# seemadhungana/ViT-Project

Measured on AMD Instinct MI355X. Metric: images/sec ViT-B/16 224 train step bs=256 (whole job), higher is better.
Workload: dtype bf16; 1 GPU; ViT-B/16 224 train step (fwd+CE+bwd+SGD), BASELINE configs[1]; model=vit_base_patch16_224, global_batch=256, per_gpu_batch=256, seq_len=197, parallelism=dp1, launch=eager

## Files before the change

include/vit_hip.h:

```cpp
#ifndef VIT_HIP_H
#define VIT_HIP_H
#include <stdint.h>

#ifdef __cplusplus
extern "C" {
#endif

enum { VIT_DTYPE_F32 = 0, VIT_DTYPE_BF16 = 1 };
enum { VIT_LAYOUT_RC = 0, VIT_LAYOUT_CR = 1 };
enum {
  VIT_EPI_STORE = 0,
  VIT_EPI_BIAS_GELU = 1,
  VIT_EPI_RESID = 2,
  VIT_EPI_GELU_BWD = 3,
  VIT_EPI_PATCH = 4,
  VIT_EPI_BIAS_QGELU = 5,
  VIT_EPI_QGELU_BWD = 6,
  VIT_EPI_BIAS_GELU_FWD = 8,
  VIT_EPI_BIAS_QGELU_FWD = 9
};

int vit_abi_version(void);

int vit_gemm(int dtype, int out_dtype, int p_layout, int q_layout, int epi, int M, int N, int R,
             const void* P, int64_t ldp, const void* Q, int64_t ldq, void* C, int64_t ldc,
             const float* bias, const void* aux, int64_t ld_aux, void* aux_out, int allow_fast, void* stream);

int vit_gemm_variant(int v);

int vit_gemm_group(int fwd, int dgrad);

int vit_gemm_g4_config(int fwd_mode, int dgrad_mode, int wgs, int tpw);

int vit_gemm_g4_count(int reset);

int vit_gemm_g4_gelu(int on);

int vit_gemm_streamk_workspace(void* stream, float* part, int64_t part_bytes, int* counters, int ncounters);

int vit_gemm_rc_chunk_rows(int M, int64_t ld);

int vit_linear_fwd(int dtype, int out_dtype, int epi, int M, int N, int K, const void* X, int64_t ldx,
                   const void* W, const float* bias, void* Y, int64_t ldy, const void* resid,
                   void* act_out, void* stream);

int vit_linear_dgrad(int dtype, int out_dtype, int epi, int M, int N, int K, const void* dY, int64_t lddy,
                     const void* W, void* dX, int64_t lddx, const void* pre, float* dbias, float* partial,
                     int64_t partial_floats, int defer_reduce, void* stream);
int vit_linear_dgrad_partial_floats(int M, int K);

int vit_linear_wgrad(int dtype, int M, int N, int K, const void* dY, int64_t lddy, const void* X,
                     int64_t ldx, float* dW, int split, void* workspace, int64_t ws_bytes, void* stream);
int vit_linear_wgrad_nslabs(int dtype, int M, int N, int K, int split);
int vit_linear_wgrad_partials(int dtype, int M, int N, int K, const void* dY, int64_t lddy, const void* X,
                              int64_t ldx, int split, float* slabs, int64_t slab_bytes, void* stream);
int vit_linear_wgrad_partials2(int M, int split, int Na, int Ka, const void* dYa, int64_t lddya, const void* Xa,
                               int64_t ldxa, float* slabs_a, int64_t bytes_a, int Nb, int Kb, const void* dYb,
                               int64_t lddyb, const void* Xb, int64_t ldxb, float* slabs_b, int64_t bytes_b,
                               void* stream);

int vit_colsum(int dtype, int M, int N, const void* X, int64_t ld, float* out, float* partial,
               int64_t partial_floats, int accumulate, void* stream);
int vit_colreduce(const float* part, int S, int N, float* out, int accumulate, float* scratch, void* stream);
int vit_colreduce_multi(const float* part, int nq, int S, int N, float* out0, float* out1, float* out2,
                        int accumulate, float* scratch, void* stream);

int vit_colreduce_batch_sizes(const int64_t* jobs, int njobs, int64_t* scratch_floats, int* counters);
int vit_colreduce_batch(const int64_t* jobs, int njobs, float* scratch, int64_t scratch_floats, int* counters,
                        int ncounters, void* stream);

int vit_patch_embed_fwd(int dtype, int B, int np, int D, int K, const void* U, const void* W,
                        const float* bias, const float* pos, float* x, void* stream);
int vit_patch_unfold(int dtype, int B, int C, int Hi, int Wi, int ps, const float* img, void* U, void* stream);
int vit_patch_unfold_ld(int dtype, int B, int C, int Hi, int Wi, int ps, int ldu, const float* img, void* U,
                        void* stream);
int vit_patch_embed_fwd_ld(int dtype, int B, int np, int D, int K, const void* U, int64_t ldu, const void* W,
                           int64_t ldw, const float* bias, const float* pos, float* x, void* stream);
int vit_copy_rows_padded(int dtype, int rows, int cols, const void* src, int64_t ld_src, void* dst, int64_t ld_dst,
                         void* stream);
int vit_cls_pos_fill(int B, int S, int D, float* x, const float* cls, const float* pos, void* stream);
int vit_pos_grad(int B, int S, int D, const float* dx, float* dpos, float* dcls, void* stream);

int vit_layer_norm_bwd_variant(int v);

int vit_layer_norm_fwd(int dtype_x, int dtype_y, int rows, int D, const void* x, int64_t ldx, void* y,
                       int64_t ldy, const float* w, const float* b, float* mean, float* rstd, float eps,
                       void* stream);
int vit_add_layer_norm_fwd(int dtype_r, int dtype_y, int rows, int D, const float* x, int64_t ldx, const void* r,
                           int64_t ldr, float* xs, int64_t ldxs, void* y, int64_t ldy, const float* w, const float* b,
                           float* mean, float* rstd, float eps, void* stream);
int vit_layer_norm_bwd(int dtype_x, int dtype_dy, int rows, int D, const void* x, int64_t ldx,
                       const void* dy, int64_t lddy, const float* w, const float* mean, const float* rstd,
                       const float* dres, int64_t ldres, float* dx, int64_t lddx, void* dx_copy, int64_t ld_copy,
                       int dtype_copy, int compact_np, float* dgamma, float* dbeta, float* dsum, float* partial,
                       int64_t partial_floats, int defer_reduce, void* stream);
int vit_layer_norm_bwd_partial_floats(int rows, int D);
int vit_layer_norm_bwd_blocks(int rows);

int vit_sdpa_fwd(int dtype, int B, int H, int N, int head_dim, const void* qkv, int64_t ld_qkv, void* o,
                 int64_t ld_o, float* lse, float scale, int causal, void* stream);
int vit_sdpa_fwd_fp8(int dtype, int B, int H, int N, int head_dim, const void* qkv, int64_t ld_qkv, void* o,
                     int64_t ld_o, float* lse, float scale, int causal, void* stream);
int vit_sdpa_bwd(int dtype, int B, int H, int N, int head_dim, const void* qkv, int64_t ld_qkv, const void* o,
                 int64_t ld_o, const void* dout, int64_t ld_do, const float* lse, void* dqkv, int64_t ld_dqkv,
                 float* delta_ws, float scale, int causal, float* dbias, float* partial, int64_t partial_floats,
                 void* stream);
int vit_sdpa_bwd_partial_floats(int B, int N, int D);
int vit_sdpa_long_config(int mode);
int vit_sdpa_long_count(int reset);
int vit_sdpa_long_f32_count(int reset);
int vit_sdpa_bwd_variant(int v);

int vit_cross_entropy_fwd(int B, int C, const float* logits, int64_t ld, const int64_t* target, float* row_lse,
                          float* row_loss, float* loss, void* stream);
int vit_cross_entropy_bwd(int dtype_out, int B, int C, const float* logits, int64_t ld, const int64_t* target,
                          const float* row_lse, const float* grad_loss, void* dlogits, int64_t ldd, void* stream);

int vit_eval_metrics(int B, int C, const float* logits, int64_t ld, const int64_t* target, int topk, float* row_ws,
                     double* acc, void* stream);

int vit_sgd_step(const void* tensors, const void* chunks, int nchunks, const float* lr, float momentum,
                 float weight_decay, void* stream);
int vit_sgd_chunk_size(void);
int vit_sgd_tensor_bytes(void);
int vit_sgd_chunk_bytes(void);

int vit_dora_weight_fwd(int in, int out, int r, const float* m, const float* A, const float* B, const float* D,
                        float scaling, const float* noise, float* W, float* nu, float* DnT_ws, float* colsq_ws,
                        void* stream);
int vit_dora_weight_bwd(int in, int out, int r, const float* m, const float* A, const float* B, const float* gW,
                        const float* DnT, float scaling, const float* nu, float* dm, float* dA, float* dB,
                        float* sdDnT_ws, const float* noise, void* stream);
int vit_dora_weight_bwd_ws(int in, int out, int r, const float* m, const float* A, const float* B, const float* gW,
                           const float* DnT, float scaling, const float* nu, float* dm, float* dA, float* dB,
                           float* sdDnT_ws, float* slabs, int64_t slab_floats, const float* noise, void* stream);
int vit_gemm_splitk(int p_layout, int q_layout, int M, int N, int R, const float* P, int64_t ldp, const float* Q,
                    int64_t ldq, float* C, float* slabs, int64_t slab_floats, void* stream);
int vit_adamw_step(const void* tensors, const void* chunks, int nchunks, float beta1, float beta2, float eps,
                   void* stream);
int vit_adamw_tensor_bytes(void);

int vit_token_embed(int rows, int L, int D, int vocab, const int64_t* tokens, const float* table, const float* pos,
                    float* x, void* stream);
int vit_gather_rows(int n, int D, const float* src, int64_t ld_src, const int64_t* idx, float* dst, int64_t ld_dst,
                    void* stream);
int vit_scatter_rows(int n, int D, const float* src, int64_t ld_src, const int64_t* idx, float* dst, int64_t ld_dst,
                     void* stream);
int vit_rownorm_fwd(int n, int D, const float* x, const float* log_scale, float* y, float* rnorm, void* stream);
int vit_rownorm_bwd(int n, int D, const float* x, const float* dy, const float* rnorm, const float* log_scale,
                    float* dx, void* stream);
int vit_mse_fwd(int n, const float* pred, const float* target, float* loss, void* stream);
int vit_mse_bwd(int n, const float* pred, const float* target, const float* grad_loss, float* dpred, void* stream);

int vit_image_coeff_bytes(int B, int S, int kmax);
int vit_image_transform(int B, int S, const uint8_t* src, const int64_t* params, int kmax, int max_rows,
                        int* coeff_ws, uint8_t* tmp_ws, float* out, const float* norm6, void* stream);

int vit_cast_f32_bf16(const float* x, void* y, int64_t n, void* stream);
int vit_zero(void* p, int64_t bytes, void* stream);

#ifdef __cplusplus
}
#endif
#endif
```

vit-project_amd/csrc/attention.hip:

```cpp
#include "common.hpp"
#include "reduce.hpp"

extern "C" int vit_colsum(int dtype, int M, int N, const void* X, int64_t ld, float* out, float* partial,
                          int64_t partial_floats, int accumulate, void* stream);

__device__ __forceinline__ int at_off(int row, int c) { return row * 128 + ((c ^ (row & 6)) << 4); }

template <int ROWS, int NTHR, int NM>
__device__ __forceinline__ void at_load(char* const (&img)[NM], const bf16* const (&src)[NM],
                                        const int64_t (&ld)[NM], int N) {
  constexpr int TOTAL = ROWS * 8, PER = (TOTAL + NTHR - 1) / NTHR;
  bf16x8 v[NM][PER];
#pragma unroll
  for (int mtx = 0; mtx < NM; ++mtx)
#pragma unroll
    for (int u = 0; u < PER; ++u) {
      const int idx = threadIdx.x + u * NTHR;
      const int row = min(idx >> 3, N - 1), c = idx & 7;
      if (idx < TOTAL) v[mtx][u] = *reinterpret_cast<const bf16x8*>(src[mtx] + (int64_t)row * ld[mtx] + c * 8);
    }
#pragma unroll
  for (int mtx = 0; mtx < NM; ++mtx)
#pragma unroll
    for (int u = 0; u < PER; ++u) {
      const int idx = threadIdx.x + u * NTHR;
      const int row = idx >> 3, c = idx & 7;
      if (idx < TOTAL) {
        bf16x8 w = v[mtx][u];
        if (row >= N) {
#pragma unroll
          for (int t = 0; t < 8; ++t) w[t] = (bf16)0.f;
        }
        *reinterpret_cast<bf16x8*>(img[mtx] + at_off(row, c)) = w;
      }
    }
}

constexpr int AT_THREADS = 512;
constexpr int AT_WAVES = AT_THREADS / 64;

__device__ __forceinline__ bf16x8 pack8(const f32x4& a, const f32x4& b) {
  return bf16x8{(bf16)a[0], (bf16)a[1], (bf16)a[2], (bf16)a[3], (bf16)b[0], (bf16)b[1], (bf16)b[2], (bf16)b[3]};
}

constexpr float LOG2E = 1.4426950408889634f;
constexpr float LN2 = 0.6931471805599453f;

struct AtOffsets {
  int row[2];
  int tr[4];
  __device__ __forceinline__ AtOffsets(int lane) {
    const int l15 = lane & 15, g = lane >> 4, q = l15 >> 2, p = l15 & 3;
#pragma unroll
    for (int kk = 0; kk < 2; ++kk) row[kk] = l15 * 128 + (((kk * 4 + g) ^ (l15 & 6)) << 4);
    const int ra = 4 * g + q;
#pragma unroll
    for (int dt = 0; dt < 4; ++dt) tr[dt] = ra * 128 + (((2 * dt + (p >> 1)) ^ (ra & 6)) << 4) + (p & 1) * 8;
  }
};
__device__ __forceinline__ bf16x8 rowf(const char* img, int row0, int off) {
  return *reinterpret_cast<const bf16x8*>(img + row0 * 128 + off);
}
__device__ __forceinline__ bf16x8 trf(const char* img, int row0, int off) {
  const char* b = img + row0 * 128 + off;
  return cat4(lds_read_tr(b), lds_read_tr(b + 16 * 128));
}
__device__ __forceinline__ float fexp2(float x) { return __builtin_amdgcn_exp2f(x); }

static unsigned long long* g_attn_stamps = nullptr;
#define AT_STAMP(i)                                                   \
  if constexpr (STAMP) { if (threadIdx.x == 0) st[i] = __builtin_amdgcn_s_memtime(); }
#define AT_STAMP_BEGIN()                                                                          \
  unsigned long long st[8] = {0, 0, 0, 0, 0, 0, 0, 0};                                            \
  if constexpr (STAMP) { if (threadIdx.x == 0) st[5] = __builtin_amdgcn_s_memrealtime(); }        \
  AT_STAMP(0)
#define AT_STAMP_FLUSH()                                                                         \
  if constexpr (STAMP) if (threadIdx.x == 0) {                                                   \
    asm volatile("s_waitcnt vmcnt(0)" ::: "memory");                                             \
    st[6] = __builtin_amdgcn_s_memtime();                                                        \
    st[7] = __builtin_amdgcn_s_memrealtime();                                                    \
    unsigned long long* d = stamps + (int64_t)blockIdx.x * 8;                                    \
    for (int i_ = 0; i_ < 8; ++i_) d[i_] = st[i_];                                               \
  }

template <int NT, bool STAMP = false, bool CAUSAL = false>
__global__ __launch_bounds__(AT_THREADS, NT <= 14 ? 4 : 2) void attn_fwd_mfma(const bf16* __restrict__ qkv, int64_t ld_qkv, int D,
                                                     int H, int N, float scale, bf16* __restrict__ o,
                                                     int64_t ld_o, float* __restrict__ lse, int causal,
                                                     unsigned long long* __restrict__ stamps) {
  AT_STAMP_BEGIN()
  constexpr int NT2 = (NT + 1) / 2, ROWS = NT2 * 32;
  __shared__ __attribute__((aligned(16))) char smem[2 * ROWS * 128];
  char* Kimg = smem;
  char* Vimg = smem + ROWS * 128;
  const int bh = blockIdx.x, b = bh / H, h = bh - b * H;
  const int lane = threadIdx.x & 63, wave = threadIdx.x >> 6, g = lane >> 4;
  const bf16* base = qkv + (int64_t)b * N * ld_qkv + h * 64;
  {
    char* const imgs[2] = {Kimg, Vimg};
    const bf16* const srcs[2] = {base + D, base + 2 * D};
    const int64_t lds_[2] = {ld_qkv, ld_qkv};
    at_load<ROWS, AT_THREADS, 2>(imgs, srcs, lds_, N);
  }
  const AtOffsets off(lane);
  __syncthreads();
  AT_STAMP(1)
  const float c2 = scale * LOG2E;
  for (int qt = wave; qt < NT; qt += AT_WAVES) {
    const int q = qt * 16 + (lane & 15);
    bf16x8 qf[2];
    {
      const int qq = min(q, N - 1);
#pragma unroll
      for (int kk = 0; kk < 2; ++kk) qf[kk] = *reinterpret_cast<const bf16x8*>(base + (int64_t)qq * ld_qkv + kk * 32 + g * 8);
    }
    f32x4 s[NT];
#pragma unroll
    for (int kt = 0; kt < NT; ++kt) {
      s[kt] = f32x4{0.f, 0.f, 0.f, 0.f};
#pragma unroll
      for (int kk = 0; kk < 2; ++kk) s[kt] = mfma16(rowf(Kimg, kt * 16, off.row[kk]), qf[kk], s[kt]);
      if (kt % 4 == 3) __builtin_amdgcn_sched_barrier(0);
    }
#pragma unroll
    for (int r = 0; r < 4; ++r)
      if ((NT - 1) * 16 + 4 * g + r >= N) s[NT - 1][r] = -INFINITY;
    if constexpr (CAUSAL) {
#pragma unroll
      for (int kt = 0; kt < NT; ++kt)
#pragma unroll
        for (int r = 0; r < 4; ++r)
          if (kt * 16 + 4 * g + r > q) s[kt][r] = -INFINITY;
    }
    float mr[4] = {-INFINITY, -INFINITY, -INFINITY, -INFINITY};
#pragma unroll
    for (int kt = 0; kt < NT; ++kt)
#pragma unroll
      for (int r = 0; r < 4; ++r) mr[r] = fmaxf(mr[r], s[kt][r]);
    float m = fmaxf(fmaxf(mr[0], mr[1]), fmaxf(mr[2], mr[3]));
    m = fmaxf(m, __shfl_xor(m, 16, 64));
    m = fmaxf(m, __shfl_xor(m, 32, 64));
    const float mc = m * c2;
    float lr[4] = {0.f, 0.f, 0.f, 0.f};
#pragma unroll
    for (int kt = 0; kt < NT; ++kt)
#pragma unroll
      for (int r = 0; r < 4; ++r) { float p = fexp2(fmaf(s[kt][r], c2, -mc)); s[kt][r] = p; lr[r] += p; }
    float l = (lr[0] + lr[1]) + (lr[2] + lr[3]);
    l += __shfl_xor(l, 16, 64);
    l += __shfl_xor(l, 32, 64);
    f32x4 oacc[4];
#pragma unroll
    for (int dt = 0; dt < 4; ++dt) oacc[dt] = f32x4{0.f, 0.f, 0.f, 0.f};
#pragma unroll
    for (int ks = 0; ks < NT2; ++ks) {
      f32x4 hi = (2 * ks + 1 < NT) ? s[2 * ks + 1 < NT ? 2 * ks + 1 : 0] : f32x4{0.f, 0.f, 0.f, 0.f};
      bf16x8 pf = pack8(s[2 * ks], hi);
#pragma unroll
      for (int dt = 0; dt < 4; ++dt) oacc[dt] = mfma16(trf(Vimg, ks * 32, off.tr[dt]), pf, oacc[dt]);
      if (ks % 2 == 1) __builtin_amdgcn_sched_barrier(0);
    }
    if (q < N) {
      const float inv = 1.0f / l;
      bf16* orow = o + ((int64_t)b * N + q) * ld_o + h * 64;
#pragma unroll
      for (int dt = 0; dt < 4; ++dt) {
        bf16x4 ov = {(bf16)(oacc[dt][0] * inv), (bf16)(oacc[dt][1] * inv), (bf16)(oacc[dt][2] * inv),
                     (bf16)(oacc[dt][3] * inv)};
        *reinterpret_cast<bf16x4*>(orow + dt * 16 + 4 * g) = ov;
      }
      if (g == 0) lse[(int64_t)bh * N + q] = (mc + __log2f(l)) * LN2;
    }
  }
  AT_STAMP(2)
  AT_STAMP_FLUSH()
}


__device__ __forceinline__ int e8m0_exp(float amax) {
  const uint32_t bits = __float_as_uint(amax);
  const int E = (int)((bits >> 23) & 255) - 127;
  if (((bits >> 23) & 255) == 0) return -127;
  const int e = (bits & 0x7fffff) <= 0x600000 ? E - 8 : E - 7;
  return e < -127 ? -127 : (e > 127 ? 127 : e);
}
__device__ __forceinline__ float inv_exp2i(int e) {
  return e >= 127 ? 0.f : __uint_as_float((uint32_t)(e == -127 ? 254 : 127 - e) << 23);
}
__device__ __forceinline__ int pack_fp8x4(float a, float b, float c, float d) {
  int w = __builtin_amdgcn_cvt_pk_fp8_f32(a, b, 0, false);
  return __builtin_amdgcn_cvt_pk_fp8_f32(c, d, w, true);
}
typedef int i32x8 __attribute__((ext_vector_type(8)));
typedef float f32x16 __attribute__((ext_vector_type(16)));

constexpr int F8_THREADS = 512, F8_WAVES = 8;
__device__ __forceinline__ int f8_koff(int key, int c) { return key * 64 + ((c ^ ((key >> 2) & 1)) << 4); }

template <typename T> __device__ __forceinline__ void load8f(const T* p, float* x);
template <> __device__ __forceinline__ void load8f<bf16>(const bf16* p, float* x) {
  const bf16x8 v = *reinterpret_cast<const bf16x8*>(p);
#pragma unroll
  for (int u = 0; u < 8; ++u) x[u] = (float)v[u];
}
template <> __device__ __forceinline__ void load8f<float>(const float* p, float* x) {
  const f32x4 a = *reinterpret_cast<const f32x4*>(p), b = *reinterpret_cast<const f32x4*>(p + 4);
#pragma unroll
  for (int u = 0; u < 4; ++u) { x[u] = a[u]; x[4 + u] = b[u]; }
}

template <int NKT, typename T>
__global__ __launch_bounds__(F8_THREADS, 2) void attn_fwd_fp8(const T* __restrict__ qkv, int64_t ld_qkv, int D,
                                                             int H, int N, float scale, T* __restrict__ o,
                                                             int64_t ld_o, float* __restrict__ lse, int causal) {
  constexpr int KEYS = NKT * 64, VROW = KEYS + 4;
  __shared__ __attribute__((aligned(16))) unsigned char Kimg[KEYS * 64];
  __shared__ __attribute__((aligned(16))) unsigned char Vt[64 * VROW];
  __shared__ unsigned char Ksc[KEYS * 2];
  __shared__ unsigned char Vsc[64 * NKT];
  const int bh = blockIdx.x, b = bh / H, hh = bh - b * H;
  const int lane = threadIdx.x & 63, wave = threadIdx.x >> 6;
  const T* base = qkv + (int64_t)b * N * ld_qkv + hh * 64;

  for (int t = threadIdx.x; t < KEYS * 2; t += F8_THREADS) {
    const int key = t >> 1, half = t & 1;
    float x[32];
    if (key < N) {
      const T* src = base + (int64_t)key * ld_qkv + D + half * 32;
#pragma unroll
      for (int c = 0; c < 4; ++c) load8f<T>(src + c * 8, x + c * 8);
    } else {
#pragma unroll
      for (int u = 0; u < 32; ++u) x[u] = 0.f;
    }
    float amax = 0.f;
#pragma unroll
    for (int u = 0; u < 32; ++u) amax = fmaxf(amax, fabsf(x[u]));
    amax = fmaxf(amax, __shfl_xor(amax, 1, 64));
    const int e = e8m0_exp(amax);
    const float inv = inv_exp2i(e);
    int w[8];
#pragma unroll
    for (int u = 0; u < 8; ++u) w[u] = pack_fp8x4(x[4 * u] * inv, x[4 * u + 1] * inv, x[4 * u + 2] * inv, x[4 * u + 3] * inv);
    typedef int i32x4_ __attribute__((ext_vector_type(4)));
    *reinterpret_cast<i32x4_*>(Kimg + f8_koff(key, 2 * half)) = i32x4_{w[0], w[1], w[2], w[3]};
    *reinterpret_cast<i32x4_*>(Kimg + f8_koff(key, 2 * half + 1)) = i32x4_{w[4], w[5], w[6], w[7]};
    Ksc[key * 2 + half] = (unsigned char)(e + 127);
  }
  for (int kt = wave; kt < NKT; kt += F8_WAVES) {
    float x[64];
    const T* src = base + 2 * D + lane;
#pragma unroll
    for (int u = 0; u < 64; ++u) {
      const int key = kt * 64 + u;
      x[u] = key < N ? (float)src[(int64_t)key * ld_qkv] : 0.f;
    }
    float amax = 0.f;
#pragma unroll
    for (int u = 0; u < 64; ++u) amax = fmaxf(amax, fabsf(x[u]));
    const int e = e8m0_exp(amax);
    const float inv = inv_exp2i(e);
#pragma unroll
    for (int u = 0; u < 16; ++u)
      *reinterpret_cast<int*>(Vt + lane * VROW + kt * 64 + 4 * u) =
          pack_fp8x4(x[4 * u] * inv, x[4 * u + 1] * inv, x[4 * u + 2] * inv, x[4 * u + 3] * inv);
    Vsc[lane * NKT + kt] = (unsigned char)(e + 127);
  }
  __syncthreads();

  const float c2 = scale * LOG2E;
  const int h = lane >> 5, l31 = lane & 31;
  const int nqt = (N + 31) / 32;
  for (int qt = wave; qt < nqt; qt += F8_WAVES) {
    const int q = qt * 32 + l31;
    i32x8 qf;
    int qsc;
    {
      const T* src = base + (int64_t)min(q, N - 1) * ld_qkv + h * 32;
      float x[32];
#pragma unroll
      for (int c = 0; c < 4; ++c) load8f<T>(src + c * 8, x + c * 8);
      float amax = 0.f;
#pragma unroll
      for (int u = 0; u < 32; ++u) amax = fmaxf(amax, fabsf(x[u]));
      amax = fmaxf(amax, __shfl_xor(amax, 32, 64));
      const int e = e8m0_exp(amax);
      const float inv = inv_exp2i(e);
#pragma unroll
      for (int u = 0; u < 8; ++u) qf[u] = pack_fp8x4(x[4 * u] * inv, x[4 * u + 1] * inv, x[4 * u + 2] * inv, x[4 * u + 3] * inv);
      qsc = e + 127;
    }
    float m = -INFINITY, l = 0.f;
    f32x16 oacc[2] = {};
#pragma unroll 1
    for (int kt = 0; kt < NKT; ++kt) {
      f32x16 s[2];
#pragma unroll
      for (int u = 0; u < 2; ++u) {
        const int key = (2 * kt + u) * 32 + l31;
        typedef int i32x4_ __attribute__((ext_vector_type(4)));
        const i32x4_ lo = *reinterpret_cast<const i32x4_*>(Kimg + f8_koff(key, 2 * h));
        const i32x4_ hi = *reinterpret_cast<const i32x4_*>(Kimg + f8_koff(key, 2 * h + 1));
        const i32x8 kf = {lo[0], lo[1], lo[2], lo[3], hi[0], hi[1], hi[2], hi[3]};
        f32x16 z = {};
        s[u] = __builtin_amdgcn_mfma_scale_f32_32x32x64_f8f6f4(kf, qf, z, 0, 0, 0, Ksc[key * 2 + h], 0, qsc);
      }
      float mt = -INFINITY;
#pragma unroll
      for (int u = 0; u < 2; ++u)
#pragma unroll
        for (int r = 0; r < 16; ++r) {
          const int key = (2 * kt + u) * 32 + 4 * h + (r & 3) + 8 * (r >> 2);
          if (key >= N || (causal && key > q)) s[u][r] = -INFINITY;
          mt = fmaxf(mt, s[u][r]);
        }
      mt = fmaxf(mt, __shfl_xor(mt, 32, 64));
      const float mn = fmaxf(m, mt);
      const float alpha = fexp2((m - mn) * c2);
      m = mn;
      const float mc = m * c2;
      l *= alpha;
#pragma unroll
      for (int dt = 0; dt < 2; ++dt) oacc[dt] *= alpha;
#pragma unroll
      for (int u = 0; u < 2; ++u)
#pragma unroll
        for (int r = 0; r < 16; ++r) {
          const float p = fexp2(fmaf(s[u][r], c2, -mc));
          s[u][r] = p;
          l += p;
        }
      i32x8 pf;
#pragma unroll
      for (int w = 0; w < 8; ++w) {
        const f32x16& t = s[w >> 2];
        const int r = 4 * (w & 3);
        pf[w] = pack_fp8x4(t[r] * 256.f, t[r + 1] * 256.f, t[r + 2] * 256.f, t[r + 3] * 256.f);
      }
#pragma unroll
      for (int dt = 0; dt < 2; ++dt) {
        const int d = dt * 32 + l31;
        const unsigned char* row = Vt + d * VROW + kt * 64 + 4 * h;
        i32x8 vf;
#pragma unroll
        for (int w = 0; w < 8; ++w) vf[w] = *reinterpret_cast<const int*>(row + (w >> 2) * 32 + 8 * (w & 3));
        oacc[dt] = __builtin_amdgcn_mfma_scale_f32_32x32x64_f8f6f4(vf, pf, oacc[dt], 0, 0, 0, Vsc[d * NKT + kt], 0,
                                                                   127 - 8);
      }
    }
    l += __shfl_xor(l, 32, 64);
    const float mc = m * c2;
    if (q < N) {
      const float inv = 1.0f / l;
      T* orow = o + ((int64_t)b * N + q) * ld_o + hh * 64;
#pragma unroll
      for (int dt = 0; dt < 2; ++dt)
#pragma unroll
        for (int mq = 0; mq < 4; ++mq) {
          const int d = dt * 32 + 4 * h + 8 * mq;
          const f32x4 ov = {oacc[dt][4 * mq] * inv, oacc[dt][4 * mq + 1] * inv, oacc[dt][4 * mq + 2] * inv,
                            oacc[dt][4 * mq + 3] * inv};
          if constexpr (sizeof(T) == 2) *reinterpret_cast<bf16x4*>(orow + d) = bf16x4{(bf16)ov[0], (bf16)ov[1], (bf16)ov[2], (bf16)ov[3]};
          else *reinterpret_cast<f32x4*>(orow + d) = ov;
        }
      if (h == 0 && lse) lse[(int64_t)bh * N + q] = (mc + __log2f(l)) * LN2;
    }
  }
}

template <int NOUT>
__device__ __forceinline__ void bias_flush(f32x4 (&c0)[4], f32x4 (*c1)[4], char* smem, float* out, int D) {
  const int lane = threadIdx.x & 63, wave = threadIdx.x >> 6, g = lane >> 4;
  float* red = reinterpret_cast<float*>(smem);
  __syncthreads();
#pragma unroll
  for (int o = 0; o < NOUT; ++o) {
    f32x4 (&c)[4] = o == 0 ? c0 : *c1;
#pragma unroll
    for (int dt = 0; dt < 4; ++dt)
#pragma unroll
      for (int t = 0; t < 4; ++t) {
        float v = c[dt][t];
        v += __shfl_xor(v, 1, 64);
        v += __shfl_xor(v, 2, 64);
        v += __shfl_xor(v, 4, 64);
        v += __shfl_xor(v, 8, 64);
        if ((lane & 15) == 0) red[(o * AT_WAVES + wave) * 64 + dt * 16 + 4 * g + t] = v;
      }
  }
  __syncthreads();
  if (threadIdx.x < 64 * NOUT) {
    const int o = threadIdx.x >> 6, d = threadIdx.x & 63;
    float sum = 0.f;
#pragma unroll
    for (int w = 0; w < AT_WAVES; ++w) sum += red[(o * AT_WAVES + w) * 64 + d];
    out[(NOUT == 1 ? 0 : (o + 1) * D) + d] = sum;
  }
}

__device__ __forceinline__ float colsum16(const f32x4 (&c)[4], int lane) {
  const int l15 = lane & 15;
  float own = 0.f;
#pragma unroll
  for (int dt = 0; dt < 4; ++dt)
#pragma unroll
    for (int t = 0; t < 4; ++t) {
      float v = c[dt][t];
      v += __shfl_xor(v, 1, 64);
      v += __shfl_xor(v, 2, 64);
      v += __shfl_xor(v, 4, 64);
      v += __shfl_xor(v, 8, 64);
// ... 1279 lines not shown
}

__global__ __launch_bounds__(AT_THREADS, 4) void attn_bwd_dq_stream_f32(
    const float* __restrict__ qkv, int64_t ld_qkv, int D, int H, int N, float scale, const float* __restrict__ o,
    int64_t ld_o, const float* __restrict__ dout, int64_t ld_do, const float* __restrict__ lse,
    float* __restrict__ delta_out, float* __restrict__ dqkv, int64_t ld_dqkv) {
  extern __shared__ __attribute__((aligned(16))) char smem[];
  float* ring = reinterpret_cast<float*>(smem);
  const int bh = blockIdx.x, b = bh / H, h = bh - b * H;
  const int lane = threadIdx.x & 63, wave = threadIdx.x >> 6, g = lane >> 4, l15 = lane & 15;
  const float* base = qkv + (int64_t)b * N * ld_qkv + h * 64;
  const int q = blockIdx.y * ST_QB + wave * 16 + l15, qc = min(q, N - 1);
  float qf[16], df[16];
  float dl = 0.f;
  {
    float of[16];
    f32_glob16(base + (int64_t)qc * ld_qkv + 16 * g, qf);
    f32_glob16(dout + ((int64_t)b * N + qc) * ld_do + h * 64 + 16 * g, df);
    f32_glob16(o + ((int64_t)b * N + qc) * ld_o + h * 64 + 16 * g, of);
#pragma unroll
    for (int j = 0; j < 16; ++j) dl = fmaf(df[j], of[j], dl);
  }
  dl += __shfl_xor(dl, 16, 64);
  dl += __shfl_xor(dl, 32, 64);
  if (q < N && g == 0) delta_out[(int64_t)bh * N + q] = dl;
  const float l2 = lse[(int64_t)bh * N + qc] * LOG2E;
  const int nc = (N + ST_CH - 1) / ST_CH;
  SfPiece pc = sf_fetch(base + D, ld_qkv, base + 2 * D, ld_qkv, 0, N);
  sf_commit(ring, pc, 0, N);
  __syncthreads();
  const float c2 = scale * LOG2E;
  f32x4 dq[4];
#pragma unroll
  for (int dt = 0; dt < 4; ++dt) dq[dt] = f32x4{0.f, 0.f, 0.f, 0.f};
#pragma unroll 1
  for (int c = 0; c < nc; ++c) {
    const float* Kc = ring + (c & 1) * 2 * SF_IMG;
    const float* Vc = Kc + SF_IMG;
    const int j0 = c * ST_CH;
    const bool more = c + 1 < nc;
    if (more) pc = sf_fetch(base + D, ld_qkv, base + 2 * D, ld_qkv, j0 + ST_CH, N);
#pragma unroll 1
    for (int kt = 0; kt < 4; ++kt) {
      float kf[16], vf[16];
      f32_row16(Kc, kt * 16 + l15, g, kf);
      f32_row16(Vc, kt * 16 + l15, g, vf);
      f32x4 st = {0.f, 0.f, 0.f, 0.f}, dpt = st;
#pragma unroll
      for (int ks = 0; ks < 16; ++ks) {
        st = mfma4(kf[ks], qf[ks], st);
        dpt = mfma4(vf[ks], df[ks], dpt);
      }
      f32x4 ds;
#pragma unroll
      for (int r = 0; r < 4; ++r) {
        const float p = j0 + kt * 16 + 4 * g + r < N ? fexp2(fmaf(st[r], c2, -l2)) : 0.f;
        ds[r] = p * (dpt[r] - dl);
      }
#pragma unroll
      for (int r = 0; r < 4; ++r) {
        const f32x4 a = f32_chunk(Kc, kt * 16 + 4 * g + r, l15);
#pragma unroll
        for (int dt = 0; dt < 4; ++dt) dq[dt] = mfma4(a[dt], ds[r], dq[dt]);
      }
    }
    if (more) sf_commit(ring + ((c + 1) & 1) * 2 * SF_IMG, pc, j0 + ST_CH, N);
    __syncthreads();
  }
  if (q < N) {
    float* row = dqkv + ((int64_t)b * N + q) * ld_dqkv + h * 64 + 16 * g;
#pragma unroll
    for (int rr = 0; rr < 4; ++rr)
      *reinterpret_cast<f32x4*>(row + 4 * rr) =
          f32x4{dq[0][rr] * scale, dq[1][rr] * scale, dq[2][rr] * scale, dq[3][rr] * scale};
  }
}

__global__ __launch_bounds__(AT_THREADS, 2) void attn_bwd_dkv_stream_f32(
    const float* __restrict__ qkv, int64_t ld_qkv, int D, int H, int N, float scale, const float* __restrict__ dout,
    int64_t ld_do, const float* __restrict__ lse, const float* __restrict__ delta_in, float* __restrict__ dqkv,
    int64_t ld_dqkv) {
  extern __shared__ __attribute__((aligned(16))) char smem[];
  float* ring = reinterpret_cast<float*>(smem);
  const int bh = blockIdx.x, b = bh / H, h = bh - b * H;
  const int tid = threadIdx.x, lane = tid & 63, wave = tid >> 6, g = lane >> 4, l15 = lane & 15;
  const float* base = qkv + (int64_t)b * N * ld_qkv + h * 64;
  const float* dob = dout + (int64_t)b * N * ld_do + h * 64;
  const int key = blockIdx.y * ST_QB + wave * 16 + l15, kc = min(key, N - 1);
  const bool kvalid = key < N;
  float kf[16], vf[16];
  f32_glob16(base + (int64_t)kc * ld_qkv + D + 16 * g, kf);
  f32_glob16(base + (int64_t)kc * ld_qkv + 2 * D + 16 * g, vf);
  auto stat_fetch = [&](int j0) -> float {
    if (tid >= 2 * ST_CH) return 0.f;
    const int i = j0 + (tid & (ST_CH - 1));
    if (tid < ST_CH) return i < N ? lse[(int64_t)bh * N + i] * LOG2E : INFINITY;
    return i < N ? delta_in[(int64_t)bh * N + i] : 0.f;
  };
  auto stat_commit = [&](float* buf, float v) {
    if (tid < 2 * ST_CH) buf[2 * SF_IMG + tid] = v;
  };
  const int nc = (N + ST_CH - 1) / ST_CH;
  SfPiece pc = sf_fetch(base, ld_qkv, dob, ld_do, 0, N);
  float sv = stat_fetch(0);
  sf_commit(ring, pc, 0, N);
  stat_commit(ring, sv);
  __syncthreads();
  const float c2 = scale * LOG2E;
  f32x4 dk[4], dv[4];
#pragma unroll
  for (int dt = 0; dt < 4; ++dt) { dk[dt] = f32x4{0.f, 0.f, 0.f, 0.f}; dv[dt] = dk[dt]; }
#pragma unroll 1
  for (int c = 0; c < nc; ++c) {
    const float* Qc = ring + (c & 1) * SF_BUF_DKV;
    const float* Oc = Qc + SF_IMG;
    const float* l2s = Qc + 2 * SF_IMG;
    const float* dls = l2s + ST_CH;
    const int j0 = c * ST_CH;
    const bool more = c + 1 < nc;
    if (more) {
      pc = sf_fetch(base, ld_qkv, dob, ld_do, j0 + ST_CH, N);
      sv = stat_fetch(j0 + ST_CH);
    }
#pragma unroll 1
    for (int qt = 0; qt < 4; ++qt) {
      float qf[16], df[16];
      f32_row16(Qc, qt * 16 + l15, g, qf);
      f32_row16(Oc, qt * 16 + l15, g, df);
      f32x4 sc = {0.f, 0.f, 0.f, 0.f}, dpc = sc;
#pragma unroll
      for (int ks = 0; ks < 16; ++ks) {
        sc = mfma4(qf[ks], kf[ks], sc);
        dpc = mfma4(df[ks], vf[ks], dpc);
      }
      const f32x4 l2 = *reinterpret_cast<const f32x4*>(l2s + qt * 16 + 4 * g);
      const f32x4 dl = *reinterpret_cast<const f32x4*>(dls + qt * 16 + 4 * g);
      f32x4 p, ds;
#pragma unroll
      for (int r = 0; r < 4; ++r) {
        const float pv = kvalid ? fexp2(fmaf(sc[r], c2, -l2[r])) : 0.f;
        p[r] = pv;
        ds[r] = pv * (dpc[r] - dl[r]);
      }
#pragma unroll
      for (int r = 0; r < 4; ++r) {
        const f32x4 ao = f32_chunk(Oc, qt * 16 + 4 * g + r, l15), aq = f32_chunk(Qc, qt * 16 + 4 * g + r, l15);
#pragma unroll
        for (int dt = 0; dt < 4; ++dt) {
          dv[dt] = mfma4(ao[dt], p[r], dv[dt]);
          dk[dt] = mfma4(aq[dt], ds[r], dk[dt]);
        }
      }
    }
    if (more) {
      float* nb = ring + ((c + 1) & 1) * SF_BUF_DKV;
      sf_commit(nb, pc, j0 + ST_CH, N);
      stat_commit(nb, sv);
    }
    __syncthreads();
  }
  if (kvalid) {
    float* row = dqkv + ((int64_t)b * N + key) * ld_dqkv + h * 64 + 16 * g;
#pragma unroll
    for (int rr = 0; rr < 4; ++rr) {
      *reinterpret_cast<f32x4*>(row + D + 4 * rr) =
          f32x4{dk[0][rr] * scale, dk[1][rr] * scale, dk[2][rr] * scale, dk[3][rr] * scale};
      *reinterpret_cast<f32x4*>(row + 2 * D + 4 * rr) = f32x4{dv[0][rr], dv[1][rr], dv[2][rr], dv[3][rr]};
    }
  }
}

__global__ __launch_bounds__(256) void attn_bias_image(const bf16* __restrict__ dqkv, int64_t ld, int N, int C,
                                                       float* __restrict__ part) {
  const int b = blockIdx.x, c = blockIdx.y * 256 + threadIdx.x;
  if (c >= C) return;
  const bf16* p = dqkv + (int64_t)b * N * ld + c;
  float a[8] = {0.f, 0.f, 0.f, 0.f, 0.f, 0.f, 0.f, 0.f};
  int n = 0;
  for (; n + 8 <= N; n += 8)
#pragma unroll
    for (int u = 0; u < 8; ++u) a[u] += (float)p[(int64_t)(n + u) * ld];
  for (; n < N; ++n) a[0] += (float)p[(int64_t)n * ld];
  part[(int64_t)b * C + c] = ((a[0] + a[1]) + (a[2] + a[3])) + ((a[4] + a[5]) + (a[6] + a[7]));
}

static int g_long_mode = -1;
static int g_long_count = 0;
static int g_long_f32_count = 0;
static bool attn_long_stream() {
  if (g_long_mode >= 0) return g_long_mode != 0;
  static const int v = [] { const char* e = getenv("VIT_ATTN_LONG"); return e && *e == '0' ? 0 : 1; }();
  return v != 0;
}
constexpr int AT_RESIDENT_MAX = 288;

static void stream_f32_attrs() {
  static bool attr = false;
  if (attr) return;
  (void)hipFuncSetAttribute((const void*)attn_fwd_stream_f32, hipFuncAttributeMaxDynamicSharedMemorySize, SF_LDS);
  (void)hipFuncSetAttribute((const void*)attn_bwd_dq_stream_f32, hipFuncAttributeMaxDynamicSharedMemorySize, SF_LDS);
  (void)hipFuncSetAttribute((const void*)attn_bwd_dkv_stream_f32, hipFuncAttributeMaxDynamicSharedMemorySize, SF_LDS_DKV);
  attr = true;
}

template <int NT>
static int fwd_mfma(const void* qkv, int64_t ld_qkv, int D, int B, int H, int N, float scale, int causal, void* o,
                    int64_t ld_o, float* lse, hipStream_t s) {
  if (causal)
    hipLaunchKernelGGL((attn_fwd_mfma<NT, false, true>), dim3(B * H), dim3(AT_THREADS), 0, s, (const bf16*)qkv, ld_qkv,
                       D, H, N, scale, (bf16*)o, ld_o, lse, causal, nullptr);
  else if (g_attn_stamps)
    hipLaunchKernelGGL((attn_fwd_mfma<NT, true>), dim3(B * H), dim3(AT_THREADS), 0, s, (const bf16*)qkv, ld_qkv, D, H,
                       N, scale, (bf16*)o, ld_o, lse, causal, g_attn_stamps);
  else
    hipLaunchKernelGGL((attn_fwd_mfma<NT>), dim3(B * H), dim3(AT_THREADS), 0, s, (const bf16*)qkv, ld_qkv, D, H, N,
                       scale, (bf16*)o, ld_o, lse, causal, nullptr);
  VIT_CHECK_LAUNCH();
  return 0;
}
static bool attn_f32_generic() {
  static const int v = [] { const char* e = getenv("VIT_ATTN_F32_GENERIC"); return e && *e == '1' ? 1 : 0; }();
  return v != 0;
}
template <int NT>
static int fwd_f32mfma(const void* qkv, int64_t ld_qkv, int D, int B, int H, int N, float scale, int causal, void* o,
                       int64_t ld_o, float* lse, hipStream_t s) {
  constexpr int lds = 2 * NT * 16 * 64 * 4;
  static bool attr = false;
  if (!attr) {
    (void)hipFuncSetAttribute((const void*)attn_fwd_f32mfma<NT>, hipFuncAttributeMaxDynamicSharedMemorySize, lds);
    attr = true;
  }
  hipLaunchKernelGGL((attn_fwd_f32mfma<NT>), dim3(B * H), dim3(512), lds, s, (const float*)qkv, ld_qkv, D, H, N, scale,
                     (float*)o, ld_o, lse, causal);
  VIT_CHECK_LAUNCH();
  return 0;
}
template <int NT>
static int bwd_f32mfma(const void* qkv, int64_t ld_qkv, int D, int B, int H, int N, float scale, int causal,
                       const void* o, int64_t ld_o, const void* dout, int64_t ld_do, const float* lse, float* delta,
                       void* dqkv, int64_t ld_dqkv, hipStream_t s) {
  constexpr int img = NT * 16 * 64 * 4, lds_dq = 2 * img, lds_dkv = 2 * img + 2 * NT * 16 * 4;
  static bool attr = false;
  if (!attr) {
    (void)hipFuncSetAttribute((const void*)attn_bwd_dq_f32mfma<NT>, hipFuncAttributeMaxDynamicSharedMemorySize, lds_dq);
    (void)hipFuncSetAttribute((const void*)attn_bwd_dkv_f32mfma<NT>, hipFuncAttributeMaxDynamicSharedMemorySize, lds_dkv);
    attr = true;
  }
  hipLaunchKernelGGL((attn_bwd_dq_f32mfma<NT>), dim3(B * H), dim3(512), lds_dq, s, (const float*)qkv, ld_qkv, D, H, N,
                     scale, (const float*)o, ld_o, (const float*)dout, ld_do, lse, delta, (float*)dqkv, ld_dqkv, causal);
  VIT_CHECK_LAUNCH();
  hipLaunchKernelGGL((attn_bwd_dkv_f32mfma<NT>), dim3(B * H), dim3(512), lds_dkv, s, (const float*)qkv, ld_qkv, D, H,
                     N, scale, (const float*)dout, ld_do, lse, (const float*)delta, (float*)dqkv, ld_dqkv, causal);
  VIT_CHECK_LAUNCH();
  return 0;
}
static int g_bwd_variant = -1;
static bool attn_bwd_split() {
  if (g_bwd_variant == 2) return true;
  static const int v = [] { const char* e = getenv("VIT_ATTN_BWD_SPLIT"); return e && *e == '1' ? 1 : 0; }();
  return v != 0;
}

template <int NT>
static int bwd_mfma(const void* qkv, int64_t ld_qkv, int D, int B, int H, int N, float scale, int causal, const void* o,
                    int64_t ld_o, const void* dout, int64_t ld_do, const float* lse, float* delta,
                    void* dqkv, int64_t ld_dqkv, float* bias_part, hipStream_t s) {
  if constexpr (NT <= 14) {
    if (!attn_bwd_split()) {
      static bool attr = false;
      if (!attr) {
        (void)hipFuncSetAttribute((const void*)attn_bwd_fused<NT>, hipFuncAttributeMaxDynamicSharedMemorySize,
                                  BwdF<NT>::LDS);
        (void)hipFuncSetAttribute((const void*)attn_bwd_fused<NT, true>, hipFuncAttributeMaxDynamicSharedMemorySize,
                                  BwdF<NT>::LDS);
        (void)hipFuncSetAttribute((const void*)attn_bwd_fused<NT, false, true>,
                                  hipFuncAttributeMaxDynamicSharedMemorySize, BwdF<NT>::LDS);
        attr = true;
      }
#define BWD_FUSED(C, S, ST)                                                                                    \
  hipLaunchKernelGGL((attn_bwd_fused<NT, C, S>), dim3(B * H), dim3(BwdF<NT>::THREADS), BwdF<NT>::LDS, s,         \
                     (const bf16*)qkv, ld_qkv, D, H, N, scale, (const bf16*)o, ld_o, (const bf16*)dout, ld_do, lse, \
                     delta, (bf16*)dqkv, ld_dqkv, bias_part, ST)
      if (causal)
        BWD_FUSED(true, false, nullptr);
      else if (g_attn_stamps)
        BWD_FUSED(false, true, g_attn_stamps);
      else
        BWD_FUSED(false, false, nullptr);
#undef BWD_FUSED
      VIT_CHECK_LAUNCH();
      return 0;
    }
  }
  hipLaunchKernelGGL((attn_bwd_dq<NT>), dim3(B * H), dim3(AT_THREADS), 0, s, (const bf16*)qkv, ld_qkv, D, H, N, scale,
                     (const bf16*)o, ld_o, (const bf16*)dout, ld_do, lse, delta, (bf16*)dqkv, ld_dqkv, bias_part, causal);
  VIT_CHECK_LAUNCH();
  hipLaunchKernelGGL((attn_bwd_dkv<NT>), dim3(B * H), dim3(AT_THREADS), 0, s, (const bf16*)qkv, ld_qkv, D, H, N, scale,
                     (const bf16*)dout, ld_do, lse, (const float*)delta, (bf16*)dqkv, ld_dqkv, bias_part, causal);
  VIT_CHECK_LAUNCH();
  return 0;
}

#define NT_CASES(X) X(1) X(2) X(3) X(4) X(5) X(6) X(7) X(8) X(9) X(10) X(11) X(12) X(13) X(14) X(15) X(16) X(17) X(18)

extern "C" {

int vit_debug_attn_stamps(void* buf) {
  g_attn_stamps = (unsigned long long*)buf;
  return 0;
}

int vit_sdpa_bwd_variant(int v) {
  if (v == 0 || v > 2) return (int)hipErrorInvalidValue;
  g_bwd_variant = v < 0 ? -1 : v;
  return 0;
}

int vit_sdpa_long_config(int mode) {
  const int prev = g_long_mode;
  g_long_mode = mode < 0 ? -1 : (mode != 0);
  return prev;
}
int vit_sdpa_long_count(int reset) {
  const int c = g_long_count;
  if (reset) g_long_count = 0;
  return c;
}
int vit_sdpa_long_f32_count(int reset) {
  const int c = g_long_f32_count;
  if (reset) g_long_f32_count = 0;
  return c;
}

int vit_sdpa_fwd(int dtype, int B, int H, int N, int head_dim, const void* qkv, int64_t ld_qkv, void* o,
                 int64_t ld_o, float* lse, float scale, int causal, void* stream) {
  hipStream_t s = (hipStream_t)stream;
  if (head_dim != 64 || N <= 0) return (int)hipErrorInvalidValue;
  const int D = H * 64;
  const bool resident = N <= AT_RESIDENT_MAX;
  if (!resident && dtype == VIT_BF16 && !causal && (ld_qkv % 8 == 0) && (ld_o % 4 == 0) && attn_long_stream()) {
    hipLaunchKernelGGL(attn_fwd_stream, dim3(B * H, (N + ST_QB - 1) / ST_QB), dim3(AT_THREADS), 0, s,
                       (const bf16*)qkv, ld_qkv, D, H, N, scale, (bf16*)o, ld_o, lse);
    VIT_CHECK_LAUNCH();
    ++g_long_count;
    return 0;
  }
  if (!resident && dtype == VIT_F32 && !causal && (ld_qkv % 4 == 0) && (ld_o % 4 == 0) && attn_long_stream() &&
      !attn_f32_generic()) {
    stream_f32_attrs();
    hipLaunchKernelGGL(attn_fwd_stream_f32, dim3(B * H, (N + ST_QB - 1) / ST_QB), dim3(AT_THREADS), SF_LDS, s,
                       (const float*)qkv, ld_qkv, D, H, N, scale, (float*)o, ld_o, lse);
    VIT_CHECK_LAUNCH();
    ++g_long_f32_count;
    return 0;
  }
  if (resident && dtype == VIT_BF16 && (ld_qkv % 8 == 0) && (ld_o % 4 == 0)) {
    int nt = (N + 15) / 16;
    switch (nt) {
#define CASE(n) case n: return fwd_mfma<n>(qkv, ld_qkv, D, B, H, N, scale, causal, o, ld_o, lse, s);
      NT_CASES(CASE)
#undef CASE
    }
  }
  if (resident && dtype == VIT_F32 && (ld_qkv % 4 == 0) && (ld_o % 4 == 0) && !attn_f32_generic()) {
    int nt = (N + 15) / 16;
    switch (nt) {
#define CASE(n) case n: return fwd_f32mfma<n>(qkv, ld_qkv, D, B, H, N, scale, causal, o, ld_o, lse, s);
      NT_CASES(CASE)
#undef CASE
    }
  }
  if ((int64_t)B * H > 65535) return (int)hipErrorInvalidValue;
  dim3 grid((N + 63) / 64, B * H);
  if (dtype == VIT_BF16)
    hipLaunchKernelGGL(attn_fwd_generic<bf16>, grid, dim3(256), 0, s, (const bf16*)qkv, ld_qkv, D, H, N, scale, (bf16*)o, ld_o, lse, causal);
  else
    hipLaunchKernelGGL(attn_fwd_generic<float>, grid, dim3(256), 0, s, (const float*)qkv, ld_qkv, D, H, N, scale, (float*)o, ld_o, lse, causal);
  VIT_CHECK_LAUNCH();
  return 0;
}

int vit_sdpa_fwd_fp8(int dtype, int B, int H, int N, int head_dim, const void* qkv, int64_t ld_qkv, void* o,
                     int64_t ld_o, float* lse, float scale, int causal, void* stream) {
  hipStream_t s = (hipStream_t)stream;
  if (head_dim != 64 || N <= 0 || N > 320 || (ld_qkv % 8) || (ld_o % 4)) return (int)hipErrorInvalidValue;
  const int D = H * 64;
  switch ((N + 63) / 64) {
#define F8(n)                                                                                                   \
  case n:                                                                                                       \
    if (dtype == VIT_BF16)                                                                                      \
      hipLaunchKernelGGL((attn_fwd_fp8<n, bf16>), dim3(B * H), dim3(F8_THREADS), 0, s, (const bf16*)qkv, ld_qkv, \
                         D, H, N, scale, (bf16*)o, ld_o, lse, causal);                                          \
    else                                                                                                        \
      hipLaunchKernelGGL((attn_fwd_fp8<n, float>), dim3(B * H), dim3(F8_THREADS), 0, s, (const float*)qkv,      \
                         ld_qkv, D, H, N, scale, (float*)o, ld_o, lse, causal);                                 \
    break;
    F8(1) F8(2) F8(3) F8(4) F8(5)
#undef F8
  }
  VIT_CHECK_LAUNCH();
  return 0;
}

int vit_sdpa_bwd_partial_floats(int B, int N, int D) {
  const int64_t C = 3 * (int64_t)D;
  const int64_t mfma = B * C + (B > 64 ? (int64_t)((B + 63) / 64) * C : 0);
  const int64_t gen = 256 * C + 4 * C;
  return (int)(mfma > gen ? mfma : gen);
}

int vit_sdpa_bwd(int dtype, int B, int H, int N, int head_dim, const void* qkv, int64_t ld_qkv, const void* o,
                 int64_t ld_o, const void* dout, int64_t ld_do, const float* lse, void* dqkv, int64_t ld_dqkv,
                 float* delta_ws, float scale, int causal, float* dbias, float* partial, int64_t partial_floats,
                 void* stream) {
  hipStream_t s = (hipStream_t)stream;
  if (head_dim != 64 || N <= 0) return (int)hipErrorInvalidValue;
  const int D = H * 64;
  const bool resident = N <= AT_RESIDENT_MAX;
  if (!delta_ws) return (int)hipErrorInvalidValue;
  const bool part_only = !dbias && partial;
  if ((dbias || part_only) && (partial == nullptr || partial_floats < vit_sdpa_bwd_partial_floats(B, N, D)))
    return (int)hipErrorInvalidValue;
  const bool mfma_ok = dtype == VIT_BF16 && (ld_qkv % 8 == 0) && (ld_do % 8 == 0) && (ld_dqkv % 4 == 0) && (ld_o % 4 == 0);
  if (!resident && dtype == VIT_BF16) {
    if (mfma_ok && !causal && attn_long_stream()) {
      const dim3 grid(B * H, (N + ST_QB - 1) / ST_QB);
      hipLaunchKernelGGL(attn_bwd_dq_stream, grid, dim3(AT_THREADS), 0, s, (const bf16*)qkv, ld_qkv, D, H, N, scale,
                         (const bf16*)o, ld_o, (const bf16*)dout, ld_do, lse, delta_ws, (bf16*)dqkv, ld_dqkv);
      VIT_CHECK_LAUNCH();
      hipLaunchKernelGGL(attn_bwd_dkv_stream, grid, dim3(AT_THREADS), 0, s, (const bf16*)qkv, ld_qkv, D, H, N, scale,
                         (const bf16*)dout, ld_do, lse, (const float*)delta_ws, (bf16*)dqkv, ld_dqkv);
      VIT_CHECK_LAUNCH();
      ++g_long_count;
    } else {
      if ((int64_t)B * H > 65535) return (int)hipErrorInvalidValue;
      const dim3 grid((N + 63) / 64, B * H);
      hipLaunchKernelGGL(attn_bwd_dq_generic<bf16>, grid, dim3(256), 0, s, (const bf16*)qkv, ld_qkv, D, H, N, scale,
                         (const bf16*)o, ld_o, (const bf16*)dout, ld_do, lse, delta_ws, (bf16*)dqkv, ld_dqkv, causal);
      VIT_CHECK_LAUNCH();
      hipLaunchKernelGGL(attn_bwd_dkv_generic<bf16>, grid, dim3(256), 0, s, (const bf16*)qkv, ld_qkv, D, H, N, scale,
                         (const bf16*)dout, ld_do, lse, delta_ws, (bf16*)dqkv, ld_dqkv, causal);
      VIT_CHECK_LAUNCH();
    }
    if (!dbias && !part_only) return 0;
    hipLaunchKernelGGL(attn_bias_image, dim3(B, (3 * D + 255) / 256), dim3(256), 0, s, (const bf16*)dqkv, ld_dqkv, N,
                       3 * D, partial);
    VIT_CHECK_LAUNCH();
    if (dbias) {
      launch_colreduce(partial, B, 3 * D, dbias, 0, s, partial + (int64_t)B * 3 * D);
      VIT_CHECK_LAUNCH();
    }
    return 0;
  }
  if (part_only && !mfma_ok) return (int)hipErrorInvalidValue;
  if (resident && mfma_ok) {
    int nt = (N + 15) / 16;
    int rc = (int)hipErrorInvalidValue;
    switch (nt) {
#define CASE(n) case n: rc = bwd_mfma<n>(qkv, ld_qkv, D, B, H, N, scale, causal, o, ld_o, dout, ld_do, lse, delta_ws, dqkv, ld_dqkv, (dbias || part_only) ? partial : nullptr, s); break;
      NT_CASES(CASE)
#undef CASE
    }
    if (rc || !dbias) return rc;
    launch_colreduce(partial, B, 3 * D, dbias, 0, s, partial + (int64_t)B * 3 * D);
    VIT_CHECK_LAUNCH();
    return 0;
  }
  if (resident && dtype == VIT_F32 && (ld_qkv % 4 == 0) && (ld_do % 4 == 0) && (ld_dqkv % 4 == 0) && (ld_o % 4 == 0) &&
      !attn_f32_generic()) {
    int nt = (N + 15) / 16, rc = (int)hipErrorInvalidValue;
    switch (nt) {
#define CASE(n) case n: rc = bwd_f32mfma<n>(qkv, ld_qkv, D, B, H, N, scale, causal, o, ld_o, dout, ld_do, lse, delta_ws, dqkv, ld_dqkv, s); break;
      NT_CASES(CASE)
#undef CASE
    }
    if (rc) return rc;
    if (dbias) return vit_colsum(dtype, B * N, 3 * D, dqkv, ld_dqkv, dbias, partial, partial_floats, 0, stream);
    return 0;
  }
  if (!resident && dtype == VIT_F32 && !causal && (ld_qkv % 4 == 0) && (ld_do % 4 == 0) && (ld_dqkv % 4 == 0) &&
      (ld_o % 4 == 0) && attn_long_stream() && !attn_f32_generic()) {
    stream_f32_attrs();
    const dim3 grid(B * H, (N + ST_QB - 1) / ST_QB);
    hipLaunchKernelGGL(attn_bwd_dq_stream_f32, grid, dim3(AT_THREADS), SF_LDS, s, (const float*)qkv, ld_qkv, D, H, N,
                       scale, (const float*)o, ld_o, (const float*)dout, ld_do, lse, delta_ws, (float*)dqkv, ld_dqkv);
    VIT_CHECK_LAUNCH();
    hipLaunchKernelGGL(attn_bwd_dkv_stream_f32, grid, dim3(AT_THREADS), SF_LDS_DKV, s, (const float*)qkv, ld_qkv, D, H,
                       N, scale, (const float*)dout, ld_do, lse, (const float*)delta_ws, (float*)dqkv, ld_dqkv);
    VIT_CHECK_LAUNCH();
    ++g_long_f32_count;
    if (dbias) return vit_colsum(dtype, B * N, 3 * D, dqkv, ld_dqkv, dbias, partial, partial_floats, 0, stream);
    return 0;
  }
  if ((int64_t)B * H > 65535) return (int)hipErrorInvalidValue;
  dim3 grid((N + 63) / 64, B * H);
#define GEN(T)                                                                                               \
  hipLaunchKernelGGL(attn_bwd_dq_generic<T>, grid, dim3(256), 0, s, (const T*)qkv, ld_qkv, D, H, N, scale,    \
                     (const T*)o, ld_o, (const T*)dout, ld_do, lse, delta_ws, (T*)dqkv, ld_dqkv, causal);    \
  VIT_CHECK_LAUNCH();                                                                                        \
  hipLaunchKernelGGL(attn_bwd_dkv_generic<T>, grid, dim3(256), 0, s, (const T*)qkv, ld_qkv, D, H, N, scale,   \
                     (const T*)dout, ld_do, lse, delta_ws, (T*)dqkv, ld_dqkv, causal);
  if (dtype == VIT_BF16) { GEN(bf16) } else { GEN(float) }
#undef GEN
  VIT_CHECK_LAUNCH();
  if (dbias) return vit_colsum(dtype, B * N, 3 * D, dqkv, ld_dqkv, dbias, partial, partial_floats, 0, stream);
  return 0;
}

}
```

vit-project_amd/csrc/norm.hip:

```cpp
#include "common.hpp"
#include "reduce.hpp"
#include <stdlib.h>
#include <type_traits>

constexpr int LN_WAVES = 4;
constexpr int LN_SMAX = 32;
static int ln_bwd_rows() {
  static int r = 0;
  if (r <= 0) {
    const char* s = getenv("VIT_LN_BWD_ROWS");
    r = s ? atoi(s) : 32;
    if (r < 4) r = 32;
  }
  return r;
}

template <typename T> __device__ __forceinline__ f32x4 ld4(const T* p);
template <> __device__ __forceinline__ f32x4 ld4<float>(const float* p) { return *reinterpret_cast<const f32x4*>(p); }
template <> __device__ __forceinline__ f32x4 ld4<bf16>(const bf16* p) {
  bf16x4 x = *reinterpret_cast<const bf16x4*>(p);
  return f32x4{(float)x[0], (float)x[1], (float)x[2], (float)x[3]};
}
template <typename T> __device__ __forceinline__ void st4(T* p, f32x4 v);
template <> __device__ __forceinline__ void st4<float>(float* p, f32x4 v) { *reinterpret_cast<f32x4*>(p) = v; }
template <> __device__ __forceinline__ void st4<bf16>(bf16* p, f32x4 v) {
  *reinterpret_cast<bf16x4*>(p) = bf16x4{(bf16)v[0], (bf16)v[1], (bf16)v[2], (bf16)v[3]};
}

__device__ __forceinline__ int col4(int lane, int k) { return (k * 64 + lane) * 4; }

template <int NV, typename TX, typename TY>
__global__ __launch_bounds__(256) void ln_fwd_kernel(const TX* __restrict__ x, int64_t ldx, TY* __restrict__ y,
                                                     int64_t ldy, const float* __restrict__ w,
                                                     const float* __restrict__ b, float* __restrict__ mean,
                                                     float* __restrict__ rstd, int rows, int D, float eps) {
  const int lane = threadIdx.x & 63;
  const int row = blockIdx.x * LN_WAVES + (threadIdx.x >> 6);
  if (row >= rows) return;
  const TX* xr = x + (int64_t)row * ldx;
  TY* yr = y + (int64_t)row * ldy;
  if constexpr (NV > 0) {
    f32x4 v[NV];
    float s = 0.f;
#pragma unroll
    for (int k = 0; k < NV; ++k) { v[k] = ld4<TX>(xr + col4(lane, k)); s += (v[k][0] + v[k][1]) + (v[k][2] + v[k][3]); }
    const float mu = wave_sum(s) / D;
    float q = 0.f;
#pragma unroll
    for (int k = 0; k < NV; ++k)
#pragma unroll
      for (int t = 0; t < 4; ++t) { float d = v[k][t] - mu; q += d * d; }
    const float rs = rsqrtf(wave_sum(q) / D + eps);
#pragma unroll
    for (int k = 0; k < NV; ++k) {
      int c = col4(lane, k);
      f32x4 g = *reinterpret_cast<const f32x4*>(w + c), bb = *reinterpret_cast<const f32x4*>(b + c), o;
#pragma unroll
      for (int t = 0; t < 4; ++t) o[t] = (v[k][t] - mu) * rs * g[t] + bb[t];
      st4<TY>(yr + c, o);
    }
    if (lane == 0) { if (mean) mean[row] = mu; if (rstd) rstd[row] = rs; }
  } else {
    float s = 0.f;
    for (int c = lane; c < D; c += 64) s += (float)xr[c];
    const float mu = wave_sum(s) / D;
    float q = 0.f;
    for (int c = lane; c < D; c += 64) { float d = (float)xr[c] - mu; q += d * d; }
    const float rs = rsqrtf(wave_sum(q) / D + eps);
    for (int c = lane; c < D; c += 64) yr[c] = (TY)(((float)xr[c] - mu) * rs * w[c] + b[c]);
    if (lane == 0) { if (mean) mean[row] = mu; if (rstd) rstd[row] = rs; }
  }
}

template <int NV, typename TR, typename TY>
__global__ __launch_bounds__(256) void add_ln_fwd_kernel(const float* __restrict__ x, int64_t ldx,
                                                         const TR* __restrict__ r, int64_t ldr,
                                                         float* __restrict__ xs, int64_t ldxs, TY* __restrict__ y,
                                                         int64_t ldy, const float* __restrict__ w,
                                                         const float* __restrict__ b, float* __restrict__ mean,
                                                         float* __restrict__ rstd, int rows, int D, float eps) {
  const int lane = threadIdx.x & 63;
  const int row = blockIdx.x * LN_WAVES + (threadIdx.x >> 6);
  if (row >= rows) return;
  const float* xr = x + (int64_t)row * ldx;
  const TR* rr = r + (int64_t)row * ldr;
  float* sr = xs + (int64_t)row * ldxs;
  f32x4 v[NV];
  float s = 0.f;
#pragma unroll
  for (int k = 0; k < NV; ++k) {
    const int c = col4(lane, k);
    v[k] = ld4<float>(xr + c) + ld4<TR>(rr + c);
    s += (v[k][0] + v[k][1]) + (v[k][2] + v[k][3]);
  }
#pragma unroll
  for (int k = 0; k < NV; ++k) st4<float>(sr + col4(lane, k), v[k]);
  if (y == nullptr) return;
  const float mu = wave_sum(s) / D;
  float q = 0.f;
#pragma unroll
  for (int k = 0; k < NV; ++k)
#pragma unroll
    for (int t = 0; t < 4; ++t) { float d = v[k][t] - mu; q += d * d; }
  const float rs = rsqrtf(wave_sum(q) / D + eps);
  TY* yr = y + (int64_t)row * ldy;
#pragma unroll
  for (int k = 0; k < NV; ++k) {
    const int c = col4(lane, k);
    f32x4 g = *reinterpret_cast<const f32x4*>(w + c), bb = *reinterpret_cast<const f32x4*>(b + c), o;
#pragma unroll
    for (int t = 0; t < 4; ++t) o[t] = (v[k][t] - mu) * rs * g[t] + bb[t];
    st4<TY>(yr + c, o);
  }
  if (lane == 0) { mean[row] = mu; rstd[row] = rs; }
}

__device__ __forceinline__ bool copy_row(int row, int compact_np, int64_t& orow) {
  orow = row;
  if (compact_np > 0) {
    int bb = row / (compact_np + 1), p = row - bb * (compact_np + 1);
    orow = (int64_t)bb * compact_np + p - 1;
    return p != 0;
  }
  return true;
}

template <int NV, typename TX, typename TD, typename TC>
__global__ __launch_bounds__(256) void ln_bwd_kernel(
    const TX* __restrict__ x, int64_t ldx, const TD* __restrict__ dy, int64_t lddy,
    const float* __restrict__ w, const float* __restrict__ mean, const float* __restrict__ rstd,
    const float* __restrict__ dres, int64_t ldres, float* __restrict__ dx, int64_t lddx,
    TC* __restrict__ dxc, int64_t ldc, int compact_np, float* __restrict__ part_g,
    float* __restrict__ part_b, float* __restrict__ part_s, int rows, int D, int rows_per) {
  constexpr int NP = NV > 0 ? NV * 4 : LN_SMAX;
  const int lane = threadIdx.x & 63, wv = threadIdx.x >> 6;
  float pg[NP], pb[NP], ps[NP];
#pragma unroll
  for (int t = 0; t < NP; ++t) { pg[t] = 0.f; pb[t] = 0.f; ps[t] = 0.f; }
  __shared__ float red[LN_WAVES][192];
  const int r0 = blockIdx.x * rows_per, r1 = min(rows, r0 + rows_per);
  for (int row = r0 + wv; row < r1; row += LN_WAVES) {
    const TX* xr = x + (int64_t)row * ldx;
    const TD* dyr = dy + (int64_t)row * lddy;
    const float mu = mean[row], rs = rstd[row];
    float* dxr = dx + (int64_t)row * lddx;
    int64_t orow = row;
    const bool keep = (dxc != nullptr) && copy_row(row, compact_np, orow);
    if constexpr (NV > 0) {
      f32x4 xh[NV], g[NV], rv[NV];
      float s1 = 0.f, s2 = 0.f;
      if (dres) {
#pragma unroll
        for (int k = 0; k < NV; ++k)
          rv[k] = *reinterpret_cast<const f32x4*>(dres + (int64_t)row * ldres + col4(lane, k));
      }
#pragma unroll
      for (int k = 0; k < NV; ++k) {
        int c = col4(lane, k);
        f32x4 xv = ld4<TX>(xr + c), dv = ld4<TD>(dyr + c), wv4 = *reinterpret_cast<const f32x4*>(w + c);
#pragma unroll
        for (int t = 0; t < 4; ++t) {
          xh[k][t] = (xv[t] - mu) * rs;
          g[k][t] = dv[t] * wv4[t];
          s1 += g[k][t];
          s2 += g[k][t] * xh[k][t];
          pg[k * 4 + t] += dv[t] * xh[k][t];
          pb[k * 4 + t] += dv[t];
        }
      }
      s1 = wave_sum(s1) / D;
      s2 = wave_sum(s2) / D;
#pragma unroll
      for (int k = 0; k < NV; ++k) {
        int c = col4(lane, k);
        f32x4 o;
#pragma unroll
        for (int t = 0; t < 4; ++t) o[t] = rs * (g[k][t] - s1 - xh[k][t] * s2);
        if (dres) o += rv[k];
#pragma unroll
        for (int t = 0; t < 4; ++t) ps[k * 4 + t] += o[t];
        *reinterpret_cast<f32x4*>(dxr + c) = o;
        if (keep) st4<TC>(dxc + orow * ldc + c, o);
      }
    } else {
      float s1 = 0.f, s2 = 0.f;
#pragma unroll
      for (int k = 0; k < LN_SMAX; ++k) {
        int c = lane + 64 * k;
        if (c < D) {
          float xh = ((float)xr[c] - mu) * rs, dv = (float)dyr[c], g = dv * w[c];
          s1 += g; s2 += g * xh;
          pg[k] += dv * xh; pb[k] += dv;
        }
      }
      s1 = wave_sum(s1) / D;
      s2 = wave_sum(s2) / D;
#pragma unroll
      for (int k = 0; k < LN_SMAX; ++k) {
        const int c = lane + 64 * k;
        if (c >= D) break;
        float xh = ((float)xr[c] - mu) * rs, g = (float)dyr[c] * w[c];
        float o = rs * (g - s1 - xh * s2);
        if (dres) o += dres[(int64_t)row * ldres + c];
        ps[k] += o;
        dxr[c] = o;
        if (keep) dxc[orow * ldc + c] = (TC)o;
      }
    }
  }
  if (!part_g && !part_s) return;
  if constexpr (NV > 0) {
    __shared__ float redv[LN_WAVES][NP][64];
    auto flush = [&](const float (&p)[NP], float* out) {
#pragma unroll
      for (int k = 0; k < NP; ++k) redv[wv][k][lane] = p[k];
      __syncthreads();
#pragma unroll
      for (int k = wv; k < NP; k += LN_WAVES) {
        const float v = (redv[0][k][lane] + redv[1][k][lane]) + (redv[2][k][lane] + redv[3][k][lane]);
        out[(int64_t)blockIdx.x * D + col4(lane, k >> 2) + (k & 3)] = v;
      }
      __syncthreads();
    };
    if (part_g) {
      flush(pg, part_g);
      flush(pb, part_b);
    }
    if (part_s) flush(ps, part_s);
    return;
  }
#pragma unroll
  for (int k = 0; k < NP; ++k) {
    const int c = NV > 0 ? col4(lane, k >> 2) + (k & 3) : k * 64 + lane;
    if (NV == 0 && k * 64 >= D) break;
    red[wv][lane] = pg[k];
    red[wv][64 + lane] = pb[k];
    red[wv][128 + lane] = ps[k];
    __syncthreads();
    if (wv == 0 && c < D) {
      const int64_t o = (int64_t)blockIdx.x * D + c;
      if (part_g) {
        part_g[o] = (red[0][lane] + red[1][lane]) + (red[2][lane] + red[3][lane]);
        part_b[o] = (red[0][64 + lane] + red[1][64 + lane]) + (red[2][64 + lane] + red[3][64 + lane]);
      }
      if (part_s) part_s[o] = (red[0][128 + lane] + red[1][128 + lane]) + (red[2][128 + lane] + red[3][128 + lane]);
    }
    __syncthreads();
  }
}


template <int NV, typename TX, typename TD> struct LnRow {
  f32x4 x[NV], r[NV];
  typename std::conditional<std::is_same<TD, float>::value, f32x4, bf16x4>::type d[NV];
  float mu, rs;
};

template <int NV, typename TX, typename TD, typename TC>
__global__ __launch_bounds__(256) void ln_bwd_pipe_kernel(
    const TX* __restrict__ x, int64_t ldx, const TD* __restrict__ dy, int64_t lddy,
    const float* __restrict__ w, const float* __restrict__ mean, const float* __restrict__ rstd,
    const float* __restrict__ dres, int64_t ldres, float* __restrict__ dx, int64_t lddx,
    TC* __restrict__ dxc, int64_t ldc, int compact_np, float* __restrict__ part_g,
    float* __restrict__ part_b, float* __restrict__ part_s, int rows, int D, int rows_per) {
  constexpr int NP = NV * 4;
  const int lane = threadIdx.x & 63, wv = __builtin_amdgcn_readfirstlane(threadIdx.x >> 6);
  float pg[NP], pb[NP], ps[NP];
#pragma unroll
  for (int t = 0; t < NP; ++t) { pg[t] = 0.f; pb[t] = 0.f; ps[t] = 0.f; }
  f32x4 wg[NV];
#pragma unroll
  for (int k = 0; k < NV; ++k) wg[k] = *reinterpret_cast<const f32x4*>(w + col4(lane, k));
  const int r0 = blockIdx.x * rows_per, r1 = min(rows, r0 + rows_per);
  using Row = LnRow<NV, TX, TD>;
  auto load = [&](int row, Row& R) {
#pragma unroll
    for (int k = 0; k < NV; ++k) {
      const int c = col4(lane, k);
      R.x[k] = ld4<TX>(x + (int64_t)row * ldx + c);
      if constexpr (std::is_same<TD, float>::value) R.d[k] = *reinterpret_cast<const f32x4*>(dy + (int64_t)row * lddy + c);
      else R.d[k] = *reinterpret_cast<const bf16x4*>(dy + (int64_t)row * lddy + c);
      R.r[k] = dres ? *reinterpret_cast<const f32x4*>(dres + (int64_t)row * ldres + c) : f32x4{0.f, 0.f, 0.f, 0.f};
    }
    R.mu = mean[row];
    R.rs = rstd[row];
  };
  auto process = [&](int row, const Row& R) {
    const float mu = R.mu, rs = R.rs;
    f32x4 xh[NV], g[NV];
    float s1 = 0.f, s2 = 0.f;
#pragma unroll
    for (int k = 0; k < NV; ++k) {
      f32x4 dv;
      if constexpr (std::is_same<TD, float>::value) dv = R.d[k];
      else dv = f32x4{(float)R.d[k][0], (float)R.d[k][1], (float)R.d[k][2], (float)R.d[k][3]};
#pragma unroll
      for (int t = 0; t < 4; ++t) {
        xh[k][t] = (R.x[k][t] - mu) * rs;
        g[k][t] = dv[t] * wg[k][t];
        s1 += g[k][t];
        s2 += g[k][t] * xh[k][t];
        pg[k * 4 + t] += dv[t] * xh[k][t];
        pb[k * 4 + t] += dv[t];
      }
    }
    s1 = wave_sum(s1) / D;
    s2 = wave_sum(s2) / D;
    int64_t orow = row;
    const bool keep = (dxc != nullptr) && copy_row(row, compact_np, orow);
    float* dxr = dx + (int64_t)row * lddx;
#pragma unroll
    for (int k = 0; k < NV; ++k) {
      const int c = col4(lane, k);
      f32x4 o;
#pragma unroll
      for (int t = 0; t < 4; ++t) o[t] = rs * (g[k][t] - s1 - xh[k][t] * s2);
      if (dres) o += R.r[k];
#pragma unroll
      for (int t = 0; t < 4; ++t) ps[k * 4 + t] += o[t];
      *reinterpret_cast<f32x4*>(dxr + c) = o;
      if (keep) st4<TC>(dxc + orow * ldc + c, o);
    }
  };
  Row A, B;
  int row = r0 + wv;
  if (row < r1) load(row, A);
  while (row < r1) {
    if (row + LN_WAVES < r1) load(row + LN_WAVES, B);
    process(row, A);
    row += LN_WAVES;
    if (row >= r1) break;
    if (row + LN_WAVES < r1) load(row + LN_WAVES, A);
    process(row, B);
    row += LN_WAVES;
  }
  if (!part_g && !part_s) return;
  __shared__ float redv[LN_WAVES][NP][64];
  auto flush = [&](const float (&p)[NP], float* out) {
#pragma unroll
    for (int k = 0; k < NP; ++k) redv[wv][k][lane] = p[k];
    __syncthreads();
#pragma unroll
    for (int k = wv; k < NP; k += LN_WAVES) {
      const float v = (redv[0][k][lane] + redv[1][k][lane]) + (redv[2][k][lane] + redv[3][k][lane]);
      out[(int64_t)blockIdx.x * D + col4(lane, k >> 2) + (k & 3)] = v;
    }
    __syncthreads();
  };
  if (part_g) {
    flush(pg, part_g);
    flush(pb, part_b);
  }
  if (part_s) flush(ps, part_s);
}


template <typename TX, typename TY>
static void launch_fwd(int nv, dim3 grid, hipStream_t s, const void* x, int64_t ldx, void* y, int64_t ldy,
                       const float* w, const float* b, float* mean, float* rstd, int rows, int D, float eps) {
#define F(NV) hipLaunchKernelGGL((ln_fwd_kernel<NV, TX, TY>), grid, dim3(64 * LN_WAVES), 0, s, (const TX*)x, ldx, (TY*)y, ldy, w, b, mean, rstd, rows, D, eps)
  switch (nv) {
    case 1: F(1); break;
    case 2: F(2); break;
    case 3: F(3); break;
    case 4: F(4); break;
    case 6: F(6); break;
    case 8: F(8); break;
    default: F(0); break;
  }
#undef F
}

static int g_ln_pipe = -1;

template <typename TX, typename TD, typename TC>
static void launch_bwd(int nv, int nblk, hipStream_t s, const void* x, int64_t ldx, const void* dy, int64_t lddy,
                       const float* w, const float* mean, const float* rstd, const float* dres, int64_t ldres,
                       float* dx, int64_t lddx, void* dxc, int64_t ldc, int compact_np, float* pg, float* pb,
                       float* ps, int rows, int D, int rows_per) {
#define B(K, NV) hipLaunchKernelGGL((K<NV, TX, TD, TC>), dim3(nblk), dim3(64 * LN_WAVES), 0, s, (const TX*)x, ldx, \
                                 (const TD*)dy, lddy, w, mean, rstd, dres, ldres, dx, lddx, (TC*)dxc, ldc, compact_np, pg, pb, ps, rows, D, rows_per)
  if (g_ln_pipe < 0) { const char* v = getenv("VIT_LN_BWD_PIPE"); g_ln_pipe = v ? atoi(v) : 1; }
  const int pipe = g_ln_pipe;
  switch (nv) {
    case 3: if (pipe) B(ln_bwd_pipe_kernel, 3); else B(ln_bwd_kernel, 3); break;
    case 4: if (pipe) B(ln_bwd_pipe_kernel, 4); else B(ln_bwd_kernel, 4); break;
    default: B(ln_bwd_kernel, 0); break;
  }
#undef B
}

extern "C" {

int vit_layer_norm_fwd(int dtype_x, int dtype_y, int rows, int D, const void* x, int64_t ldx, void* y,
                       int64_t ldy, const float* w, const float* b, float* mean, float* rstd, float eps,
                       void* stream) {
  hipStream_t s = (hipStream_t)stream;
  if (rows <= 0) return 0;
  if (D > 64 * LN_SMAX) return (int)hipErrorInvalidValue;
  dim3 grid((rows + LN_WAVES - 1) / LN_WAVES);
  bool vec = (D % 256 == 0) && (ldx % 4 == 0) && (ldy % 4 == 0);
  int nv = vec ? D / 256 : 0;
  if (dtype_x == VIT_F32 && dtype_y == VIT_F32) launch_fwd<float, float>(nv, grid, s, x, ldx, y, ldy, w, b, mean, rstd, rows, D, eps);
  else if (dtype_x == VIT_F32) launch_fwd<float, bf16>(nv, grid, s, x, ldx, y, ldy, w, b, mean, rstd, rows, D, eps);
  else if (dtype_y == VIT_BF16) launch_fwd<bf16, bf16>(nv, grid, s, x, ldx, y, ldy, w, b, mean, rstd, rows, D, eps);
  else launch_fwd<bf16, float>(nv, grid, s, x, ldx, y, ldy, w, b, mean, rstd, rows, D, eps);
  VIT_CHECK_LAUNCH();
  return 0;
}

int vit_add_layer_norm_fwd(int dtype_r, int dtype_y, int rows, int D, const float* x, int64_t ldx, const void* r,
                           int64_t ldr, float* xs, int64_t ldxs, void* y, int64_t ldy, const float* w, const float* b,
                           float* mean, float* rstd, float eps, void* stream) {
  hipStream_t s = (hipStream_t)stream;
  if (rows <= 0) return 0;
  if (D % 256 || D > 2048 || (ldx | ldr | ldxs | ldy) % 4) return (int)hipErrorInvalidValue;
  if (y && (!w || !b || !mean || !rstd)) return (int)hipErrorInvalidValue;
  dim3 grid((rows + LN_WAVES - 1) / LN_WAVES);
  if ((dtype_r != VIT_BF16 && dtype_r != VIT_F32) || (dtype_y != VIT_BF16 && dtype_y != VIT_F32))
    return (int)hipErrorInvalidValue;
#define A(NV, TR, TY)                                                                                          \
  hipLaunchKernelGGL((add_ln_fwd_kernel<NV, TR, TY>), grid, dim3(64 * LN_WAVES), 0, s, x, ldx, (const TR*)r, ldr, xs, \
                     ldxs, (TY*)y, ldy, w, b, mean, rstd, rows, D, eps)
#define AD(NV)                                                         \
  if (dtype_r == VIT_BF16 && dtype_y == VIT_BF16) A(NV, bf16, bf16);   \
  else if (dtype_r == VIT_BF16) A(NV, bf16, float);                    \
  else if (dtype_y == VIT_BF16) A(NV, float, bf16);                    \
  else A(NV, float, float);
  switch (D / 256) {
    case 1: AD(1) break;
    case 2: AD(2) break;
    case 3: AD(3) break;
    case 4: AD(4) break;
    case 5: AD(5) break;
    case 6: AD(6) break;
    case 7: AD(7) break;
    case 8: AD(8) break;
    default: return (int)hipErrorInvalidValue;
  }
#undef AD
#undef A
  VIT_CHECK_LAUNCH();
  return 0;
}

int vit_layer_norm_bwd_variant(int v) { g_ln_pipe = v; return 0; }

int vit_layer_norm_bwd_blocks(int rows) { return (rows + ln_bwd_rows() - 1) / ln_bwd_rows(); }

int vit_layer_norm_bwd_partial_floats(int rows, int D) {
  const int nblk = vit_layer_norm_bwd_blocks(rows);
  return (int)(3 * (int64_t)nblk * D + 3 * colreduce_scratch_floats(nblk, D));
}

int vit_layer_norm_bwd(int dtype_x, int dtype_dy, int rows, int D, const void* x, int64_t ldx,
                       const void* dy, int64_t lddy, const float* w, const float* mean, const float* rstd,
                       const float* dres, int64_t ldres, float* dx, int64_t lddx, void* dx_copy, int64_t ld_copy,
                       int dtype_copy, int compact_np, float* dgamma, float* dbeta, float* dsum, float* partial,
                       int64_t partial_floats, int defer_reduce, void* stream) {
  hipStream_t s = (hipStream_t)stream;
  if (rows <= 0) return 0;
  if (D > 64 * LN_SMAX) return (int)hipErrorInvalidValue;
  const int rows_per = ln_bwd_rows();
  const int nblk = vit_layer_norm_bwd_blocks(rows);
  const bool want = dgamma != nullptr || dsum != nullptr;
  if (want && (partial == nullptr || partial_floats < vit_layer_norm_bwd_partial_floats(rows, D)))
    return (int)hipErrorInvalidValue;
  float* pg = dgamma ? partial : nullptr;
  float* pb = dgamma ? partial + (int64_t)nblk * D : nullptr;
  float* ps = dsum ? partial + 2 * (int64_t)nblk * D : nullptr;
  float* scratch = want ? partial + 3 * (int64_t)nblk * D : nullptr;
  bool vec = (D % 256 == 0) && (ldx % 4 == 0) && (lddy % 4 == 0) && (lddx % 4 == 0) && (ldres % 4 == 0) &&
             (ld_copy % 4 == 0);
  int nv = vec ? D / 256 : 0;
#define LB(TX, TD) \
  if (dtype_copy == VIT_BF16) launch_bwd<TX, TD, bf16>(nv, nblk, s, x, ldx, dy, lddy, w, mean, rstd, dres, ldres, dx, lddx, dx_copy, ld_copy, compact_np, pg, pb, ps, rows, D, rows_per); \
  else launch_bwd<TX, TD, float>(nv, nblk, s, x, ldx, dy, lddy, w, mean, rstd, dres, ldres, dx, lddx, dx_copy, ld_copy, compact_np, pg, pb, ps, rows, D, rows_per);
  if (dtype_x == VIT_F32 && dtype_dy == VIT_F32) { LB(float, float) }
  else if (dtype_x == VIT_F32) { LB(float, bf16) }
  else if (dtype_dy == VIT_BF16) { LB(bf16, bf16) }
  else { LB(bf16, float) }
#undef LB
  VIT_CHECK_LAUNCH();
  if (defer_reduce) return 0;
  {
    float* outs[3] = {dgamma, dbeta, dsum};
    if (dgamma) launch_colreduce_multi(pg, dsum ? 3 : 2, nblk, D, outs, 0, s, scratch);
    else if (dsum) launch_colreduce_multi(ps, 1, nblk, D, outs + 2, 0, s, scratch);
  }
  VIT_CHECK_LAUNCH();
  return 0;
}

}
```

vit-project_amd/vit_amd/__init__.py:

```python
from . import _lib
from .model import (VisionTransformer, create_model, cross_entropy, set_wgrad_overlap, set_forward_only,
                    block_forward_only)
from .pos_embed import resample_abs_pos_embed, adapt_state_dict
from .optim import FusedSGD, FusedAdamW, CosineAnnealingLRWithWarmup
from .dora import DoRALayer, dora_weight
from . import rsa
from . import clip
from . import sweep
from . import data
from . import evaluate
from .evaluate import EvalMeter, validate
from .clip import CLIPHBA, MSELoss, mse_loss, apply_dora_to_ViT, switch_dora_layers, count_trainable_parameters

__all__ = ["VisionTransformer", "create_model", "cross_entropy", "set_wgrad_overlap", "FusedSGD", "FusedAdamW",
           "CosineAnnealingLRWithWarmup", "DoRALayer", "dora_weight", "rsa", "clip", "data", "CLIPHBA", "MSELoss",
           "mse_loss", "apply_dora_to_ViT", "switch_dora_layers", "count_trainable_parameters", "set_forward_only",
           "block_forward_only", "evaluate", "EvalMeter", "validate", "resample_abs_pos_embed", "adapt_state_dict"]


def load_library(path=None):
    return _lib.load(path)
```

vit-project_amd/vit_amd/_lib.py:

```python
from __future__ import annotations

import ctypes as C
import os

import torch

_HERE = os.path.dirname(os.path.abspath(__file__))
LIB_PATH = os.environ.get("VIT_HIP_LIB", os.path.join(_HERE, "lib", "libvit_hip.so"))

F32, BF16 = 0, 1
LAY_RC, LAY_CR = 0, 1
EPI_STORE, EPI_BIAS_GELU, EPI_RESID, EPI_GELU_BWD, EPI_PATCH, EPI_BIAS_QGELU, EPI_QGELU_BWD = range(7)
EPI_BIAS_GELU_FWD, EPI_BIAS_QGELU_FWD = 8, 9

i32, i64, f32, vp = C.c_int, C.c_int64, C.c_float, C.c_void_p

SIGNATURES = {
    "vit_abi_version": [],
    "vit_gemm_variant": [i32],
    "vit_gemm_group": [i32, i32],
    "vit_gemm_g4_config": [i32, i32, i32, i32],
    "vit_gemm_g4_count": [i32],
    "vit_gemm_g4_gelu": [i32],
    "vit_gemm_streamk_workspace": [vp, vp, i64, vp, i32],
    "vit_gemm_rc_chunk_rows": [i32, i64],
    "vit_gemm": [i32, i32, i32, i32, i32, i32, i32, i32, vp, i64, vp, i64, vp, i64, vp, vp, i64, vp, i32, vp],
    "vit_linear_fwd": [i32, i32, i32, i32, i32, i32, vp, i64, vp, vp, vp, i64, vp, vp, vp],
    "vit_linear_dgrad": [i32, i32, i32, i32, i32, i32, vp, i64, vp, vp, i64, vp, vp, vp, i64, i32, vp],
    "vit_linear_dgrad_partial_floats": [i32, i32],
    "vit_colreduce": [vp, i32, i32, vp, i32, vp, vp],
    "vit_colreduce_multi": [vp, i32, i32, i32, vp, vp, vp, i32, vp, vp],
    "vit_colreduce_batch_sizes": [vp, i32, vp, vp],
    "vit_colreduce_batch": [vp, i32, vp, i64, vp, i32, vp],
    "vit_linear_wgrad": [i32, i32, i32, i32, vp, i64, vp, i64, vp, i32, vp, i64, vp],
    "vit_linear_wgrad_nslabs": [i32, i32, i32, i32, i32],
    "vit_linear_wgrad_partials": [i32, i32, i32, i32, vp, i64, vp, i64, i32, vp, i64, vp],
    "vit_linear_wgrad_partials2": [i32, i32, i32, i32, vp, i64, vp, i64, vp, i64, i32, i32, vp, i64, vp, i64, vp,
                                   i64, vp],
    "vit_colsum": [i32, i32, i32, vp, i64, vp, vp, i64, i32, vp],
    "vit_patch_embed_fwd": [i32, i32, i32, i32, i32, vp, vp, vp, vp, vp, vp],
    "vit_patch_embed_fwd_ld": [i32, i32, i32, i32, i32, vp, i64, vp, i64, vp, vp, vp, vp],
    "vit_layer_norm_fwd": [i32, i32, i32, i32, vp, i64, vp, i64, vp, vp, vp, vp, f32, vp],
    "vit_add_layer_norm_fwd": [i32, i32, i32, i32, vp, i64, vp, i64, vp, i64, vp, i64, vp, vp, vp, vp, f32, vp],
    "vit_layer_norm_bwd": [i32, i32, i32, i32, vp, i64, vp, i64, vp, vp, vp, vp, i64, vp, i64, vp, i64, i32,
                           i32, vp, vp, vp, vp, i64, i32, vp],
    "vit_layer_norm_bwd_partial_floats": [i32, i32],
    "vit_layer_norm_bwd_blocks": [i32],
    "vit_layer_norm_bwd_variant": [i32],
    "vit_sdpa_fwd": [i32, i32, i32, i32, i32, vp, i64, vp, i64, vp, f32, i32, vp],
    "vit_sdpa_fwd_fp8": [i32, i32, i32, i32, i32, vp, i64, vp, i64, vp, f32, i32, vp],
    "vit_sdpa_bwd_variant": [i32],
    "vit_sdpa_long_config": [i32],
    "vit_sdpa_long_count": [i32],
    "vit_sdpa_long_f32_count": [i32],
    "vit_sdpa_bwd": [i32, i32, i32, i32, i32, vp, i64, vp, i64, vp, i64, vp, vp, i64, vp, f32, i32, vp, vp, i64, vp],
    "vit_sdpa_bwd_partial_floats": [i32, i32, i32],
    "vit_patch_unfold": [i32, i32, i32, i32, i32, i32, vp, vp, vp],
    "vit_patch_unfold_ld": [i32, i32, i32, i32, i32, i32, i32, vp, vp, vp],
    "vit_copy_rows_padded": [i32, i32, i32, vp, i64, vp, i64, vp],
    "vit_cls_pos_fill": [i32, i32, i32, vp, vp, vp, vp],
    "vit_pos_grad": [i32, i32, i32, vp, vp, vp, vp],
    "vit_cross_entropy_fwd": [i32, i32, vp, i64, vp, vp, vp, vp, vp],
    "vit_cross_entropy_bwd": [i32, i32, i32, vp, i64, vp, vp, vp, vp, i64, vp],
    "vit_eval_metrics": [i32, i32, vp, i64, vp, i32, vp, vp, vp],
    "vit_sgd_step": [vp, vp, i32, vp, f32, f32, vp],
    "vit_sgd_chunk_size": [],
    "vit_sgd_tensor_bytes": [],
    "vit_sgd_chunk_bytes": [],
    "vit_cast_f32_bf16": [vp, vp, i64, vp],
    "vit_zero": [vp, i64, vp],
    "vit_dora_weight_fwd": [i32, i32, i32, vp, vp, vp, vp, f32, vp, vp, vp, vp, vp, vp],
    "vit_dora_weight_bwd": [i32, i32, i32, vp, vp, vp, vp, vp, f32, vp, vp, vp, vp, vp, vp, vp],
    "vit_dora_weight_bwd_ws": [i32, i32, i32, vp, vp, vp, vp, vp, f32, vp, vp, vp, vp, vp, vp, i64, vp, vp],
    "vit_gemm_splitk": [i32, i32, i32, i32, i32, vp, i64, vp, i64, vp, vp, i64, vp],
    "vit_adamw_step": [vp, vp, i32, f32, f32, f32, vp],
    "vit_adamw_tensor_bytes": [],
    "vit_token_embed": [i32, i32, i32, i32, vp, vp, vp, vp, vp],
    "vit_gather_rows": [i32, i32, vp, i64, vp, vp, i64, vp],
    "vit_scatter_rows": [i32, i32, vp, i64, vp, vp, i64, vp],
    "vit_rownorm_fwd": [i32, i32, vp, vp, vp, vp, vp],
    "vit_rownorm_bwd": [i32, i32, vp, vp, vp, vp, vp, vp],
    "vit_mse_fwd": [i32, vp, vp, vp, vp],
    "vit_mse_bwd": [i32, vp, vp, vp, vp, vp],
    "vit_image_coeff_bytes": [i32, i32, i32],
    "vit_image_transform": [i32, i32, vp, vp, i32, i32, vp, vp, vp, vp, vp],
}

_lib = None


class HipError(RuntimeError):
    pass


def load(path: str | None = None):
    global _lib
    if _lib is not None:
        return _lib
    p = path or LIB_PATH
    if not os.path.exists(p):
        raise HipError(f"libvit_hip.so not found at {p}: build it with `python __graft_entry__.py` "
                       f"or `make -C vit-project_amd/csrc` (no CPU fallback exists)")
    lib = C.CDLL(p, mode=C.RTLD_GLOBAL)
    for name, args in SIGNATURES.items():
        fn = getattr(lib, name)
        fn.argtypes = args
        fn.restype = i32
    _lib = lib
    return lib


def lib():
    return _lib if _lib is not None else load()


def check(rc: int, what: str):
    if rc != 0:
        raise HipError(f"{what} failed with hipError {rc}")


def call(name: str, *args):
    check(getattr(lib(), name)(*args), name)


def require_gpu(t: torch.Tensor):
    if not t.is_cuda:
        raise HipError("vit_amd ops run only on a ROCm GPU tensor (no CPU fallback); got device "
                       f"{t.device}")


def stream_ptr(device=None) -> int:
    return torch.cuda.current_stream(device).cuda_stream


def ptr(t):
    return None if t is None else t.data_ptr()


def dt(t: torch.Tensor) -> int:
    if t.dtype == torch.float32:
        return F32
    if t.dtype == torch.bfloat16:
        return BF16
    raise HipError(f"unsupported dtype {t.dtype}")


def exported_symbols():
    return list(SIGNATURES)
```

vit-project_amd/vit_amd/model.py:

```python
from __future__ import annotations

import math
import os
from collections import OrderedDict

import torch
import torch.nn as nn

from . import _lib as L
from . import ops

_GRAD_COPY = {}


def _take_copy(g: torch.Tensor, dtype, want_dsum: bool = False):
    key = (g.data_ptr(), g.numel())
    c = _GRAD_COPY.pop(key, None)
    fresh = c is not None and c[1] == g._version
    dsum = c[2] if fresh else None
    if fresh and c[0] is not None and c[0].dtype == dtype:
        out = c[0]
    elif dtype == torch.float32:
        out = g
    else:
        out = torch.empty(g.shape, dtype=dtype, device=g.device)
        ops.cast_bf16(g.contiguous(), out)
    return (out, dsum) if want_dsum else out


def _put_copy(g: torch.Tensor, copy, dsum=None):
    _GRAD_COPY[(g.data_ptr(), g.numel())] = (copy, g._version, dsum)


_SIDE = {}
_OVERLAP = [True]
_FWD_JOIN = [os.environ.get("VIT_FWD_JOIN", "end")]
_BWD_JOIN = [os.environ.get("VIT_BWD_JOIN", "end")]
_HOLD_REFS = [os.environ.get("VIT_HOLD_REFS", "1") != "0"]
_FWD_HALF_DELTA = [None if os.environ.get("VIT_FWD_HALF_DELTA") is None else int(os.environ["VIT_FWD_HALF_DELTA"])]
_HOLD = {}


_FUSED_RESID_F32 = [os.environ.get("VIT_FUSED_RESID_F32", "0") == "1"]
_FWD_ONLY = [os.environ.get("VIT_FWD_ONLY", "1") != "0"]


def set_wgrad_overlap(enable: bool):
    _OVERLAP[0] = bool(enable)




def fwd_split(B: int) -> int:
    delta = 3 * B // 64 if _FWD_HALF_DELTA[0] is None else _FWD_HALF_DELTA[0]
    return min(B - 1, max(1, B // 2 + delta))


class _Side:
    def __init__(self, dev):
        self.main = torch.cuda.current_stream(dev)
        self.on = _OVERLAP[0] and dev.type == "cuda"
        if self.on:
            if dev not in _SIDE:
                _SIDE[dev] = torch.cuda.Stream(device=dev)
            self.side = _SIDE[dev]

    def run(self, fn):
        if not self.on:
            return fn()
        self.side.wait_stream(self.main)
        with torch.cuda.stream(self.side):
            return fn()

    def join(self):
        if self.on:
            self.main.wait_stream(self.side)
            _HOLD.pop(self.side, None)

    def guard(self, *ts):
        if self.on and _HOLD_REFS[0]:
            _HOLD.setdefault(self.side, []).extend(t for t in ts if t is not None)


class _Shadowed:

    def __init__(self):
        self.pairs = []

    def add(self, p: nn.Parameter, dtype):
        if dtype == torch.float32:
            p._vit_shadow = None
            return
        sh = torch.empty(p.shape, dtype=dtype, device=p.device)
        p._vit_shadow = sh
        p._vit_shadow_version = -1
        self.pairs.append(p)

    def refresh(self):
        for p in self.pairs:
            if p._vit_shadow.device != p.device or p._vit_shadow.shape != p.shape:
                p._vit_shadow = torch.empty(p.shape, dtype=p._vit_shadow.dtype, device=p.device)
                p._vit_shadow_version = -1
            if p._vit_shadow_version != p._version:
                ops.cast_bf16(p.detach(), p._vit_shadow)
                p._vit_shadow_version = p._version


def cfg_defer_bwd(ctx) -> bool:
    return getattr(ctx, "defer_bwd", False)


_JOIN_QUEUED = set()


def _queue_backward_join(dev):
    key = (torch._C._current_graph_task_id(), dev)
    if key in _JOIN_QUEUED:
        return
    _JOIN_QUEUED.clear()
    _JOIN_QUEUED.add(key)

    def _join():
        _JOIN_QUEUED.discard(key)
        _Side(dev).join()

    torch.autograd.Variable._execution_engine.queue_callback(_join)


def _gout(p: nn.Parameter) -> torch.Tensor:
    fb = getattr(p, "_vit_flat_grad", None)
    if fb is not None and (p.grad is None or p.grad.data_ptr() != fb.data_ptr()):
        return fb.view(fb.shape)
    return torch.empty(p.shape, dtype=torch.float32, device=p.device)


def _w(p: nn.Parameter):
    sh = getattr(p, "_vit_shadow", None)
    return p.detach() if sh is None else sh


def _wt(p: torch.Tensor, dtype) -> torch.Tensor:
    sh = getattr(p, "_vit_shadow", None)
    if sh is not None:
        return sh
    w = p.detach()
    if w.dtype == dtype:
        return w.contiguous()
    out = torch.empty(w.shape, dtype=dtype, device=w.device)
    ops.cast_bf16(w.contiguous(), out)
    return out



class _PatchEmbedFn(torch.autograd.Function):
    @staticmethod
    def forward(ctx, img, w, b, cls, pos, cfg):
        ctx.params = (w, b, cls, pos)
        ps, T = cfg["patch"], cfg["dtype"]
        B = img.shape[0]
        U = ops.patch_unfold(img.contiguous(), ps, T)
        npatch = U.shape[0] // B
        D = w.shape[0]
        x = ops.patch_embed_fwd(U, _w(w).reshape(D, -1), b.detach(), pos.detach().reshape(-1, D),
                                cls.detach().reshape(-1), B, npatch)
        ctx.save_for_backward(U)
        ctx.meta = (B, npatch, D, tuple(w.shape), T)
        return x

    @staticmethod
    def backward(ctx, dx):
        _Side(dx.device).join()
        (U,) = ctx.saved_tensors
        B, npatch, D, wshape, T = ctx.meta
        dx = dx.contiguous()
        S = npatch + 1
        key = (dx.data_ptr(), dx.numel())
        c = _GRAD_COPY.pop(key, None)
        if c is not None and c[1] == dx._version and c[0].dtype == T and c[0].shape[0] == B * npatch:
            dxc = c[0]
        else:
            rows = dx.reshape(B, S, D)[:, 1:, :].reshape(B * npatch, D)
            if T == torch.float32:
                dxc = rows.contiguous()
            else:
                dxc = torch.empty(B * npatch, D, dtype=T, device=dx.device)
                ops.cast_bf16(rows.contiguous(), dxc)
        pw, pb, pc, pp = ctx.params
        dw = _gout(pw)
        ops.linear_wgrad(dxc, U, out=dw.view(D, -1), tail=True)
        db = ops.colsum(dxc, out=_gout(pb))
        dpos, dcls = _gout(pp), _gout(pc)
        ops.pos_grad(dx, B, S, D, dpos, dcls)
        return None, dw, db, dcls, dpos, None


def _block_chain(x, params, cfg, fwd_only):
    n1w, n1b, qkvw, qkvb, projw, projb, n2w, n2b, fc1w, fc1b, fc2w, fc2b = params
    B, N, D = x.shape
    H, T, eps = cfg["heads"], cfg["dtype"], cfg["eps"]
    if fwd_only:
        act_epi = L.EPI_BIAS_QGELU_FWD if cfg["quick_gelu"] else L.EPI_BIAS_GELU_FWD
    else:
        act_epi = L.EPI_BIAS_QGELU if cfg["quick_gelu"] else L.EPI_BIAS_GELU
    M = B * N
    dev = x.device
    x2 = x.reshape(M, D)
    F = fc1w.shape[0]
    f32 = torch.float32
    h1, h2 = torch.empty(M, D, dtype=T, device=dev), torch.empty(M, D, dtype=T, device=dev)
    m1, r1, m2, r2 = (torch.empty(M, dtype=f32, device=dev) for _ in range(4))
    qkv = torch.empty(M, 3 * D, dtype=T, device=dev)
    o = torch.empty(M, D, dtype=T, device=dev)
    lse = torch.empty(B * H * N, dtype=f32, device=dev)
    xm, xo = torch.empty(M, D, dtype=f32, device=dev), torch.empty(M, D, dtype=f32, device=dev)
    act = torch.empty(M, F, dtype=T, device=dev)
    dact = None if fwd_only else torch.empty(M, F, dtype=T, device=dev)
    Wqkv, Wproj, W1, W2 = _wt(qkvw, T), _wt(projw, T), _wt(fc1w, T), _wt(fc2w, T)
    causal = bool(cfg.get("causal", False))
    attn_fp8 = bool(cfg.get("attn_fp8", False))
    if attn_fp8:
        ops.check_fp8_tokens(N)

    rs = cfg.get("resid")
    pend = rs.get("pending") if rs is not None else None
    pb = yb = None
    if rs is not None:
        pb, yb = torch.empty(M, D, dtype=T, device=dev), torch.empty(M, D, dtype=T, device=dev)

    def fc1(sl):
        if fwd_only:
            return lambda: ops.linear_fwd(h2[sl], W1, fc1b.detach(), epi=act_epi, out=act[sl])
        return lambda: ops.linear_fwd(h2[sl], W1, fc1b.detach(), epi=act_epi, out=dact[sl], act_out=act[sl])

    def ln1(sl):
        if pend is not None:
            return lambda: ops.add_layer_norm_fwd(pend[0][sl], pend[1][sl], x2[sl], n1w.detach(), n1b.detach(), eps,
                                                  out=h1[sl], mean=m1[sl], rstd=r1[sl])
        return lambda: ops.layer_norm_fwd(x2[sl], n1w.detach(), n1b.detach(), eps, T, out=h1[sl], mean=m1[sl],
                                          rstd=r1[sl])

    def chain_fused(b0, b1):
        sl = slice(b0 * N, b1 * N)
        steps = [
            ln1(sl),
            lambda: ops.linear_fwd(h1[sl], Wqkv, qkvb.detach(), out=qkv[sl]),
            lambda: ops.sdpa_fwd(qkv[sl], b1 - b0, H, N, o=o[sl], lse=lse[b0 * H * N:b1 * H * N], causal=causal,
                                 fp8=attn_fp8),
            lambda: ops.linear_fwd(o[sl], Wproj, projb.detach(), out=pb[sl]),
            lambda: ops.add_layer_norm_fwd(x2[sl], pb[sl], xm[sl], n2w.detach(), n2b.detach(), eps, out=h2[sl],
                                           mean=m2[sl], rstd=r2[sl]),
            fc1(sl),
            lambda: ops.linear_fwd(act[sl], W2, fc2b.detach(), out=yb[sl]),
        ]
        if cfg.get("resid_last"):
            steps.append(lambda: ops.add_layer_norm_fwd(xm[sl], yb[sl], xo[sl]))
        return steps

    def chain(b0, b1):
        if rs is not None:
            return chain_fused(b0, b1)
        r0, r1_ = b0 * N, b1 * N
        sl = slice(r0, r1_)
        return [
            lambda: ops.layer_norm_fwd(x2[sl], n1w.detach(), n1b.detach(), eps, T, out=h1[sl], mean=m1[sl],
                                       rstd=r1[sl]),
            lambda: ops.linear_fwd(h1[sl], Wqkv, qkvb.detach(), out=qkv[sl]),
            lambda: ops.sdpa_fwd(qkv[sl], b1 - b0, H, N, o=o[sl], lse=lse[b0 * H * N:b1 * H * N], causal=causal,
                                 fp8=attn_fp8),
            lambda: ops.linear_fwd(o[sl], Wproj, projb.detach(), epi=L.EPI_RESID, resid=x2[sl], out=xm[sl]),
            lambda: ops.layer_norm_fwd(xm[sl], n2w.detach(), n2b.detach(), eps, T, out=h2[sl], mean=m2[sl],
                                       rstd=r2[sl]),
            fc1(sl),
            lambda: ops.linear_fwd(act[sl], W2, fc2b.detach(), epi=L.EPI_RESID, resid=xm[sl], out=xo[sl]),
        ]

    def run(steps):
        for f in steps:
            f()

    side = _Side(dev)
    if side.on and B >= 2 and T != torch.float32:
        hb = fwd_split(B)
        mine, other = chain(0, hb), chain(hb, B)
        side.run(lambda: run(other))
        side.guard(x2, h1, m1, r1, qkv, o, lse, xm, h2, m2, r2, dact, act, xo,
                   *(t for t in (pb, yb, *(pend or ())) if t is not None))
        run(mine)
        if not cfg.get("defer_join"):
            side.join()
    else:
        run(chain(0, B))
    if rs is not None:
        rs["pending"] = None if cfg.get("resid_last") else (xm, yb)
    return xo.reshape(B, N, D), (x2, h1, m1, r1, qkv, o, lse, xm, h2, m2, r2, dact, act), (Wqkv, Wproj, W1, W2)


def block_forward_only(x, params, cfg):
    with torch.no_grad():
        return _block_chain(x, tuple(params), cfg, True)[0]


def forward_only_enabled() -> bool:
    return _FWD_ONLY[0]


def set_forward_only(enable: bool) -> bool:
    prev = _FWD_ONLY[0]
    _FWD_ONLY[0] = bool(enable)
    return prev


def wants_forward_only(enabled: bool, grad_enabled: bool, input_requires_grad: bool,
                       any_param_requires_grad: bool) -> bool:
    return bool(enabled) and (not grad_enabled or not (input_requires_grad or any_param_requires_grad))


def run_block(x, params, cfg):
    if wants_forward_only(_FWD_ONLY[0], torch.is_grad_enabled(), x.requires_grad,
                          any(p.requires_grad for p in params)):
        return block_forward_only(x, params, cfg)
    return _BlockFn.apply(x, *params, cfg)


class _BlockFn(torch.autograd.Function):

    @staticmethod
    def forward(ctx, x, n1w, n1b, qkvw, qkvb, projw, projb, n2w, n2b, fc1w, fc1b, fc2w, fc2b, cfg):
        params = (n1w, n1b, qkvw, qkvb, projw, projb, n2w, n2b, fc1w, fc1b, fc2w, fc2b)
        xo, saved, wops = _block_chain(x, params, cfg, False)
        B, N, D = x.shape
        H, T = cfg["heads"], cfg["dtype"]
        causal = bool(cfg.get("causal", False))
        attn_fp8 = bool(cfg.get("attn_fp8", False))
        ctx.save_for_backward(*saved)
        ctx.params = params
        ctx.wops = wops
        ctx.meta = (B, N, D, H, T, cfg.get("compact_np", 0), cfg["quick_gelu"], causal)
        ctx.defer_bwd = bool(cfg.get("defer_bwd_join"))
        ctx.attn_fp8 = attn_fp8
        ctx.grad_hook = cfg.get("grad_hook")
        ctx.flat_span = cfg.get("flat_span")
        return xo

    @staticmethod
    def backward(ctx, dxo):
        x2, h1, m1, r1, qkv, o, lse, xm, h2, m2, r2, dact, act = ctx.saved_tensors
        n1w, n1b, qkvw, qkvb, projw, projb, n2w, n2b, fc1w, fc1b, fc2w, fc2b = ctx.params
        Wqkv, Wproj, W1, W2 = ctx.wops
        B, N, D, H, T, compact_np, qg, causal = ctx.meta
        ng = ctx.needs_input_grad
        M = B * N
        dev = dxo.device
        dxo = dxo.contiguous().reshape(M, D)
        dxo_c, dxo_sum = _take_copy(dxo, T, want_dsum=True)
        gelu_bwd = L.EPI_QGELU_BWD if qg else L.EPI_GELU_BWD
        side = _Side(dev)
        need_mlp_in = any(ng[0:11])
        need_attn = any(ng[0:5])
        need_h1 = any(ng[0:3])
        if need_attn and ctx.attn_fp8:
            raise RuntimeError("this block's attention ran in fp8 (forward only); its backward needs the bf16 "
                               "forward: enable fp8 attention only for frozen blocks / no-grad passes")
        g = [None] * 13
        dpre = dxm = dxm_c = do = dqkv = None
        for i, p in ((1, n1w), (2, n1b), (3, qkvw), (4, qkvb), (5, projw), (6, projb), (7, n2w), (8, n2b),
                     (9, fc1w), (10, fc1b), (11, fc2w), (12, fc2b)):
            if ng[i]:
                g[i] = _gout(p)
        rb = rbw = ops.ColBatch()
        if ng[12]:
            if dxo_sum is not None:
                rb.add(dxo_sum.view(1, D), 1, D, g[12])
            else:
                ops.colsum(dxo_c, out=g[12])
        pair_mlp = rbw is not None and ng[11] and ng[9] and need_mlp_in
        if ng[11] and not pair_mlp:
            side.run(lambda: ops.linear_wgrad(dxo_c, act, out=g[11], reduce_on=rbw))
        dx = None
        if need_mlp_in:
            dpre = ops.linear_dgrad(dxo_c, W2, out_dtype=T, epi=gelu_bwd, pre=dact, dbias=g[10], reduce_on=rb)
            if pair_mlp:
                side.run(lambda: ops.linear_wgrad_pair((dxo_c, act, g[11]), (dpre, h2, g[9]), rbw))
            elif ng[9]:
                side.run(lambda: ops.linear_wgrad(dpre, h2, out=g[9], reduce_on=rbw))
        if any(ng[0:9]):
            dh2 = ops.linear_dgrad(dpre, W1, out_dtype=T)
            dxm = torch.empty(M, D, dtype=torch.float32, device=dev)
            dxm_c = dxm if T == torch.float32 else torch.empty(M, D, dtype=T, device=dev)
            ops.layer_norm_bwd(xm, D, dh2, n2w.detach(), m2, r2, dxm, D, M, dres=dxo, ldres=D,
                               dx_copy=None if T == torch.float32 else dxm_c, ld_copy=D, dgamma=g[7], dbeta=g[8],
                               dsum=g[6], reduce_on=rb)
            tail = bool(compact_np)
            pair_attn = rbw is not None and ng[5] and ng[3] and need_attn
            if ng[5] and not pair_attn:
                side.run(lambda: ops.linear_wgrad(dxm_c, o, out=g[5], tail=tail, reduce_on=rbw))
            if need_attn:
                do = ops.linear_dgrad(dxm_c, Wproj, out_dtype=T)
                dqkv = ops.sdpa_bwd(qkv, o, do, lse, B, H, N, dbias=g[4], causal=causal,
                                    reduce_on=rb)
                if pair_attn:
                    side.run(lambda: ops.linear_wgrad_pair((dxm_c, o, g[5]), (dqkv, h1, g[3]), rbw, tail=tail))
                elif ng[3]:
                    side.run(lambda: ops.linear_wgrad(dqkv, h1, out=g[3], tail=tail, reduce_on=rbw))
            if need_h1:
                dh1 = ops.linear_dgrad(dqkv, Wqkv, out_dtype=T)
                dx = torch.empty(M, D, dtype=torch.float32, device=dev)
                if compact_np:
                    dx_c = torch.empty(B * compact_np, D, dtype=T, device=dev)
                else:
                    dx_c = None if T == torch.float32 or not ng[0] else torch.empty(M, D, dtype=T, device=dev)
                dsum = None if (compact_np or not ng[0]) else torch.empty(D, dtype=torch.float32, device=dev)
                ops.layer_norm_bwd(x2, D, dh1, n1w.detach(), m1, r1, dx, D, M, dres=dxm, ldres=D, dx_copy=dx_c,
                                   ld_copy=D, compact_np=compact_np, dgamma=g[1], dbeta=g[2], dsum=dsum,
                                   reduce_on=rb)
                if ng[0] and (dx_c is not None or dsum is not None):
                    _put_copy(dx, dx_c, dsum)
        side.run(rb.launch)
        side.guard(*rb.parts)
        side.guard(dxo, dxo_c, dxo_sum, x2, h1, m1, r1, qkv, o, lse, xm, h2, m2, r2, dact, act,
                   *(v for v in (dpre, dxm, dxm_c, do, dqkv, dx) if v is not None))
        if cfg_defer_bwd(ctx):
            _queue_backward_join(dev)
        if ctx.grad_hook is not None and all(ng[1:13]):
            side.run(lambda: ctx.grad_hook(*ctx.flat_span))
        if not cfg_defer_bwd(ctx):
            side.join()
        return (dx.reshape(B, N, D) if (ng[0] and dx is not None) else None, *g[1:], None)


class _HeadFn(torch.autograd.Function):

    @staticmethod
    def forward(ctx, x, nw, nb, hw, hb, cfg):
        B, N, D = x.shape
        xc, mc, rc = ops.layer_norm_fwd(x, nw.detach(), nb.detach(), cfg["eps"], torch.float32, rows=B, ldx=N * D)
        logits = ops.linear_fwd(xc, hw.detach(), hb.detach(), out_dtype=torch.float32)
        ctx.save_for_backward(x, xc, mc, rc)
        ctx.params = (nw, nb, hw, hb)
        ctx.meta = (B, N, D, cfg["dtype"])
        return logits

    @staticmethod
    def backward(ctx, dlogits):
        x, xc, mc, rc = ctx.saved_tensors
        nw, nb, hw, hb = ctx.params
        B, N, D, T = ctx.meta
        dlogits = dlogits.contiguous().to(torch.float32)
        dxc = ops.linear_dgrad(dlogits, hw.detach(), out_dtype=torch.float32)
        dhw = ops.linear_wgrad(dlogits, xc, out=_gout(hw))
        dhb = ops.colsum(dlogits, out=_gout(hb))
        dx = ops.zero_(torch.empty(B, N, D, dtype=torch.float32, device=x.device))
        dx_c = None
        if T != torch.float32:
            dx_c = ops.zero_(torch.empty(B * N, D, dtype=T, device=x.device))
        dnw, dnb = _gout(nw), _gout(nb)
        dsum = torch.empty(D, dtype=torch.float32, device=x.device)
        ops.layer_norm_bwd(x, N * D, dxc, nw.detach(), mc, rc, dx, N * D, B, dx_copy=dx_c, ld_copy=N * D,
                           dgamma=dnw, dbeta=dnb, dsum=dsum)
        _put_copy(dx, dx_c, dsum)
        return dx, dnw, dnb, dhw, dhb, None


class _CrossEntropyFn(torch.autograd.Function):
    @staticmethod
    def forward(ctx, logits, target):
        logits = logits.contiguous().to(torch.float32)
        loss, row_lse = ops.cross_entropy_fwd(logits, target.contiguous())
        ctx.save_for_backward(logits, target, row_lse)
        return loss

    @staticmethod
    def backward(ctx, g):
        logits, target, row_lse = ctx.saved_tensors
        return ops.cross_entropy_bwd(logits, target, row_lse, g), None


def cross_entropy(logits, target):
    L.require_gpu(logits)
    return _CrossEntropyFn.apply(logits, target)



class PatchEmbed(nn.Module):
    def __init__(self, img_size, patch_size, in_chans, embed_dim):
        super().__init__()
        self.img_size, self.patch_size = img_size, patch_size
        self.num_patches = (img_size // patch_size) ** 2
        self.proj = nn.Conv2d(in_chans, embed_dim, patch_size, patch_size)


class Attention(nn.Module):
    def __init__(self, dim, num_heads):
        super().__init__()
        self.num_heads = num_heads
        self.head_dim = dim // num_heads
        self.scale = self.head_dim ** -0.5
        self.qkv = nn.Linear(dim, 3 * dim)
        self.proj = nn.Linear(dim, dim)


class Mlp(nn.Module):
    def __init__(self, dim, hidden):
        super().__init__()
        self.fc1 = nn.Linear(dim, hidden)
        self.fc2 = nn.Linear(hidden, dim)


class Block(nn.Module):
    def __init__(self, dim, num_heads, mlp_ratio, eps):
        super().__init__()
        self.norm1 = nn.LayerNorm(dim, eps=eps)
        self.attn = Attention(dim, num_heads)
        self.norm2 = nn.LayerNorm(dim, eps=eps)
        self.mlp = Mlp(dim, int(dim * mlp_ratio))

    def block_params(self):
        return (self.norm1.weight, self.norm1.bias, self.attn.qkv.weight, self.attn.qkv.bias,
                self.attn.proj.weight, self.attn.proj.bias, self.norm2.weight, self.norm2.bias,
                self.mlp.fc1.weight, self.mlp.fc1.bias, self.mlp.fc2.weight, self.mlp.fc2.bias)


class VisionTransformer(nn.Module):

    def __init__(self, img_size=224, patch_size=16, in_chans=3, num_classes=1000, embed_dim=768, depth=12,
                 num_heads=12, mlp_ratio=4.0, eps=1e-6, quick_gelu=False, compute_dtype=torch.bfloat16):
        super().__init__()
        if embed_dim // num_heads != 64:
            raise ValueError("the HIP attention kernels require head_dim 64")
        self.num_classes = num_classes
        self.embed_dim = self.num_features = embed_dim
        self.global_pool = "token"
        self.num_prefix_tokens = 1
        self.compute_dtype = compute_dtype
        self._cfg = dict(heads=num_heads, eps=eps, quick_gelu=quick_gelu, dtype=compute_dtype, patch=patch_size)
        self.cls_token = nn.Parameter(torch.zeros(1, 1, embed_dim))
        self.patch_embed = PatchEmbed(img_size, patch_size, in_chans, embed_dim)
        self.pos_embed = nn.Parameter(torch.zeros(1, self.patch_embed.num_patches + 1, embed_dim))
        self.blocks = nn.Sequential(*[Block(embed_dim, num_heads, mlp_ratio, eps) for _ in range(depth)])
        self.norm = nn.LayerNorm(embed_dim, eps=eps)
        self.head = nn.Linear(embed_dim, num_classes)
        self._shadows = None
        self._defer_grad_join = False
        self._attn_fp8 = False
        self.init_weights()

    @torch.no_grad()
    def init_weights(self, seed=None):
        g = torch.Generator().manual_seed(seed) if seed is not None else None
        nn.init.trunc_normal_(self.pos_embed, std=0.02, generator=g)
        nn.init.normal_(self.cls_token, std=1e-6, generator=g)
        for m in self.modules():
            if isinstance(m, nn.Linear):
                nn.init.trunc_normal_(m.weight, std=0.02, generator=g)
                nn.init.zeros_(m.bias)

    def load_oracle_params(self, params: "OrderedDict[str, torch.Tensor]"):
        self.load_state_dict(params, strict=True)

    def _ensure_shadows(self):
        dev = self.cls_token.device
        if self._shadows is None or self._shadows_device != dev:
            self._shadows = _Shadowed()
            self._shadows_device = dev
            ws = [self.patch_embed.proj.weight]
            for blk in self.blocks:
                ws += [blk.attn.qkv.weight, blk.attn.proj.weight, blk.mlp.fc1.weight, blk.mlp.fc2.weight]
            for p in ws:
                self._shadows.add(p, self.compute_dtype)
        self._shadows.refresh()

    def use_flat_grads(self, enable: bool = True):
        params = list(self.parameters())
        if not enable:
            for p in params:
                p._vit_flat_grad = None
            self.flat_grad = None
            return None
        order = [self.norm.weight, self.norm.bias, self.head.weight, self.head.bias]
        for blk in reversed(list(self.blocks)):
            order += list(reversed(blk.block_params()))
        pe = self.patch_embed.proj
        order += [pe.weight, pe.bias, self.cls_token, self.pos_embed]
        assert len(order) == len(params) and {id(p) for p in order} == {id(p) for p in params}
        n = sum(p.numel() for p in order)
        flat = torch.zeros(n, dtype=torch.float32, device=self.cls_token.device)
        off = 0
        self.flat_grad_slices = []
        for p in order:
            p._vit_flat_grad = flat[off:off + p.numel()].view(p.shape)
            self.flat_grad_slices.append((off, p.numel()))
            off += p.numel()
        self.flat_grad = flat
        ends = {}
        off = 0
        for p in order:
            ends[id(p)] = (off, off + p.numel())
            off += p.numel()
        for blk in self.blocks:
            spans = [ends[id(p)] for p in blk.block_params()]
            blk._flat_span = (min(s for s, _ in spans), max(e for _, e in spans))
        return flat

    def set_deferred_grad_join(self, enable: bool = True):
        self._defer_grad_join = bool(enable)

    def set_attention_fp8(self, enable: bool = True):
        self._attn_fp8 = bool(enable)

    def set_grad_ready_hook(self, fn):
        self._grad_hook = fn

    def shadow_params(self):
        self._ensure_shadows()
        return list(self._shadows.pairs)

    def _tokens(self, x):
        L.require_gpu(x)
        self._ensure_shadows()
        cfg = dict(self._cfg)
        pe = self.patch_embed
        x = _PatchEmbedFn.apply(x.to(torch.float32), pe.proj.weight, pe.proj.bias, self.cls_token, self.pos_embed,
                                cfg)
        n = len(self.blocks)
        cfg["defer_join"] = _FWD_JOIN[0] == "end"
        cfg["defer_bwd_join"] = (self._defer_grad_join and _BWD_JOIN[0] == "end"
                                 and getattr(self, "flat_grad", None) is not None
                                 and torch.is_grad_enabled() and pe.proj.weight.requires_grad
                                 and all(p.grad is None for p in self.parameters()))
        hook = getattr(self, "_grad_hook", None) if cfg["defer_bwd_join"] else None
        cfg["attn_fp8"] = self._attn_fp8 and not torch.is_grad_enabled()
        D = self.embed_dim
        if (self.compute_dtype != torch.float32 or _FUSED_RESID_F32[0]) and ops.add_layer_norm_supported(D):
            cfg["resid"] = {"pending": None}
        for i, blk in enumerate(self.blocks):
            bcfg = cfg if i != 0 else dict(cfg, compact_np=pe.num_patches)
            if "resid" in cfg and i == n - 1:
                bcfg = dict(bcfg, resid_last=True)
            if hook is not None:
                bcfg = dict(bcfg, grad_hook=hook, flat_span=blk._flat_span)
            x = run_block(x, blk.block_params(), bcfg)
        if cfg["defer_join"]:
            _Side(x.device).join()
        return x

    def forward_features(self, x):
        x = self._tokens(x)
        B, N, D = x.shape
        y, _, _ = ops.layer_norm_fwd(x.reshape(B * N, D), self.norm.weight.detach(), self.norm.bias.detach(),
                                     self._cfg["eps"], torch.float32, need_stats=False)
        return y.reshape(B, N, D)

    def forward_head(self, feats, pre_logits=False):
        x = feats[:, 0]
        return x if pre_logits else ops.linear_fwd(x.contiguous(), self.head.weight.detach(),
                                                   self.head.bias.detach(), out_dtype=torch.float32)

    def forward(self, x):
        x = self._tokens(x)
        return _HeadFn.apply(x, self.norm.weight, self.norm.bias, self.head.weight, self.head.bias, dict(self._cfg))


_MODEL_CFGS = {
    "vit_base_patch16_224": dict(img_size=224, patch_size=16, embed_dim=768, depth=12, num_heads=12),
    "vit_large_patch16_224": dict(img_size=224, patch_size=16, embed_dim=1024, depth=24, num_heads=16),
    "vit_small_patch16_224": dict(img_size=224, patch_size=16, embed_dim=384, depth=12, num_heads=6),
    "vit_base_patch16_384": dict(img_size=384, patch_size=16, embed_dim=768, depth=12, num_heads=12),
    "vit_large_patch16_384": dict(img_size=384, patch_size=16, embed_dim=1024, depth=24, num_heads=16),
    "vit_base_patch8_224": dict(img_size=224, patch_size=8, embed_dim=768, depth=12, num_heads=12),
}


def create_model(name: str, pretrained: bool = False, num_classes: int = 1000, compute_dtype=torch.bfloat16,
                 **kw):
    if pretrained:
        raise ValueError("pretrained weights are not available offline")
    if name not in _MODEL_CFGS:
        raise KeyError(f"unknown model {name}; known: {sorted(_MODEL_CFGS)}")
    cfg = dict(_MODEL_CFGS[name])
    cfg.update(kw)
    return VisionTransformer(num_classes=num_classes, compute_dtype=compute_dtype, **cfg)
```

vit-project_amd/vit_amd/ops.py:

```python
from __future__ import annotations

import os

import torch

from . import _lib as L
from ._lib import call, ptr

_WS = {}


def workspace(name: str, nbytes: int, device) -> torch.Tensor:
    key = (name, torch.device(device))
    t = _WS.get(key)
    if t is None or t.numel() < nbytes:
        t = torch.empty(max(nbytes, 256), dtype=torch.uint8, device=device)
        _WS[key] = t
    return t


def _s(t: torch.Tensor) -> int:
    return L.stream_ptr(t.device)


def _keep(t: torch.Tensor):
    if t.is_cuda:
        t.record_stream(torch.cuda.current_stream(t.device))



_SK = {}


def _streamk(device, stream=None):
    st = L.stream_ptr(device) if stream is None else stream.cuda_stream
    key = (torch.device(device).index if torch.device(device).index is not None else torch.cuda.current_device(), st)
    if key in _SK or torch.cuda.is_current_stream_capturing():
        return
    g = 2 * torch.cuda.get_device_properties(device).multi_processor_count
    part = torch.empty(g * 2 * 128 * 128, dtype=torch.float32, device=device)
    cnt = torch.zeros(g, dtype=torch.int32, device=device)
    with torch.cuda.device(key[0]):
        call("vit_gemm_streamk_workspace", st, ptr(part), part.numel() * 4, ptr(cnt), g)
    _SK[key] = (part, cnt)


def register_capture_stream(stream, device=None):
    _streamk(stream.device if device is None else device, stream)


def linear_fwd(x2d, w, bias=None, epi=L.EPI_STORE, out=None, out_dtype=None, resid=None, act_out=None):
    L.require_gpu(x2d)
    M, K = x2d.shape
    N = w.shape[0]
    assert w.shape[1] == K and w.is_contiguous() and x2d.stride(1) == 1
    assert w.dtype == x2d.dtype
    if out is None:
        if epi == L.EPI_RESID:
            od = torch.float32
        else:
            od = out_dtype or x2d.dtype
        out = torch.empty(M, N, dtype=od, device=x2d.device)
    if epi in (L.EPI_BIAS_GELU, L.EPI_BIAS_QGELU):
        if act_out is None:
            act_out = torch.empty_like(out)
    if epi == L.EPI_RESID:
        assert resid is not None and resid.dtype == torch.float32 and out.dtype == torch.float32
        assert resid.stride(0) == out.stride(0)
    if x2d.dtype == torch.float32:
        _streamk(x2d.device)
    call("vit_linear_fwd", L.dt(x2d), L.dt(out), epi, M, N, K, ptr(x2d), x2d.stride(0), ptr(w), ptr(bias),
         ptr(out), out.stride(0), ptr(resid), ptr(act_out), _s(x2d))
    return (out, act_out) if epi in (L.EPI_BIAS_GELU, L.EPI_BIAS_QGELU) else out


def linear_dgrad(dy2d, w, out_dtype=torch.float32, epi=L.EPI_STORE, pre=None, out=None, dbias=None, reduce_on=None):
    M, N = dy2d.shape
    K = w.shape[1]
    assert w.shape[0] == N and w.dtype == dy2d.dtype and dy2d.stride(1) == 1
    if out is None:
        out = torch.empty(M, K, dtype=out_dtype, device=dy2d.device)
    if pre is not None:
        assert pre.stride(0) == out.stride(0)
    part, nfl = None, 0
    defer = dbias is not None and reduce_on is not None
    if dbias is not None:
        assert dbias.dtype == torch.float32 and dbias.is_contiguous() and dbias.numel() == K
        nfl = L.lib().vit_linear_dgrad_partial_floats(M, K)
        part = (torch.empty(nfl, dtype=torch.float32, device=dy2d.device) if defer
                else workspace("dgrad_bias", nfl * 4, dy2d.device))
    if dy2d.dtype == torch.float32:
        _streamk(dy2d.device)
    call("vit_linear_dgrad", L.dt(dy2d), L.dt(out), epi, M, N, K, ptr(dy2d), dy2d.stride(0), ptr(w), ptr(out),
         out.stride(0), ptr(pre), ptr(dbias), ptr(part), nfl, int(defer), _s(dy2d))
    if defer:
        rows = (M + 63) // 64
        if isinstance(reduce_on, ColBatch):
            reduce_on.add(part, rows, K, dbias)
            return out

        def finish():
            _keep(part)
            colreduce(part, rows, K, dbias, scratch=part[rows * K:])
        reduce_on.run(finish)
    return out


def colreduce(part, S, N, out, accumulate=False, scratch=None):
    call("vit_colreduce", ptr(part), S, N, ptr(out), int(accumulate), ptr(scratch), _s(out))
    return out


class ColBatch:

    def __init__(self):
        self.jobs = []
        self.parts = []
        self.device = None

    def add(self, part, S, N, out, accumulate=False):
        if out is None or S <= 0:
            return
        assert part.dtype == torch.float32 and out.dtype == torch.float32 and part.is_contiguous()
        self.jobs.append((part.data_ptr(), out.data_ptr(), int(S), int(N), int(accumulate)))
        self.parts.append(part)
        self.device = part.device

    def launch(self):
        if not self.jobs:
            return
        import ctypes
        import numpy as np
        dev = self.device
        arr = np.array(self.jobs, dtype=np.int64).reshape(-1)
        jp = arr.ctypes.data_as(ctypes.c_void_p)
        sf, nc = ctypes.c_int64(0), ctypes.c_int(0)
        L.lib().vit_colreduce_batch_sizes(jp, len(self.jobs), ctypes.byref(sf), ctypes.byref(nc))
        scratch = workspace("colbatch", max(16, sf.value * 4), dev)
        cnt = _counters("colbatch", nc.value, dev)
        call("vit_colreduce_batch", jp, len(self.jobs), ptr(scratch), sf.value, ptr(cnt), nc.value, L.stream_ptr(dev))
        self.jobs = []


_CNT = {}


def _counters(name, n, device):
    key = (name, torch.device(device))
    t = _CNT.get(key)
    if t is None or t.numel() < n:
        t = torch.zeros(max(n, 64), dtype=torch.int32, device=device)
        _CNT[key] = t
    return t


_WGRAD_WGS = [int(os.environ.get("VIT_WGRAD_WGS", "128"))]


_WGRAD_TAIL_WGS = [int(os.environ.get("VIT_WGRAD_TAIL_WGS", "256"))]


def _wgrad_split(M, N, K, wgs=None):
    tiles = max(1, ((N + 255) // 256) * ((K + 255) // 256))
    want = max(1, round((wgs or _WGRAD_WGS[0]) / tiles))
    return max(1, min(want, M // 1024))


def linear_wgrad(dy2d, x2d, out=None, split=None, tail=False, reduce_on=None):
    M, N = dy2d.shape
    K = x2d.shape[1]
    assert x2d.shape[0] == M and x2d.dtype == dy2d.dtype
    if out is None:
        out = torch.empty(N, K, dtype=torch.float32, device=dy2d.device)
    if split is None:
        split = _wgrad_split(M, N, K, _WGRAD_TAIL_WGS[0] if tail else None)
    defer = isinstance(reduce_on, ColBatch) and split > 1 and dy2d.dtype == torch.bfloat16
    probe = WGRAD_PROBE[0]
    if probe is not None:
        e0 = torch.cuda.Event(enable_timing=True)
        e0.record()
    if defer:
        nz = L.lib().vit_linear_wgrad_nslabs(L.dt(dy2d), M, N, K, split)
        slabs = torch.empty(nz * N * K, dtype=torch.float32, device=dy2d.device)
        call("vit_linear_wgrad_partials", L.dt(dy2d), M, N, K, ptr(dy2d), dy2d.stride(0), ptr(x2d), x2d.stride(0),
             split, ptr(slabs), slabs.numel() * 4, _s(dy2d))
        reduce_on.add(slabs.view(nz, N * K), nz, N * K, out)
    else:
        ws = workspace("wgrad", split * N * K * 4, dy2d.device) if split > 1 else None
        call("vit_linear_wgrad", L.dt(dy2d), M, N, K, ptr(dy2d), dy2d.stride(0), ptr(x2d), x2d.stride(0), ptr(out),
             split, ptr(ws), 0 if ws is None else ws.numel(), _s(dy2d))
    if probe is not None:
        e1 = torch.cuda.Event(enable_timing=True)
        e1.record()
        probe.append((e0, e1, 2.0 * M * N * K, L.dt(dy2d) == L.BF16 and M % 32 == 0))
    return out


def linear_wgrad_pair(a, b, reduce_on, tail=False):
    (dya, xa, outa), (dyb, xb, outb) = a, b
    M, Na = dya.shape
    Ka, Nb, Kb = xa.shape[1], dyb.shape[1], xb.shape[1]
    ok = (isinstance(reduce_on, ColBatch) and dya.dtype == torch.bfloat16 and dyb.dtype == torch.bfloat16
          and xa.dtype == dya.dtype and xb.dtype == dyb.dtype and dyb.shape[0] == M and M % 32 == 0)
    if ok:
        tiles = ((Na + 255) // 256) * ((Ka + 255) // 256) + ((Nb + 255) // 256) * ((Kb + 255) // 256)
        wgs = _WGRAD_TAIL_WGS[0] if tail else _WGRAD_WGS[0]
        split = max(1, min(max(1, round(wgs / tiles)), M // 1024))
        nz = L.lib().vit_linear_wgrad_nslabs(L.BF16, M, Na, Ka, split)
        sa = torch.empty(nz * Na * Ka, dtype=torch.float32, device=dya.device)
        sb = torch.empty(nz * Nb * Kb, dtype=torch.float32, device=dya.device)
        probe = WGRAD_PROBE[0]
        if probe is not None:
            e0 = torch.cuda.Event(enable_timing=True)
            e0.record()
        rc = L.lib().vit_linear_wgrad_partials2(M, split, Na, Ka, ptr(dya), dya.stride(0), ptr(xa), xa.stride(0),
                                                ptr(sa), sa.numel() * 4, Nb, Kb, ptr(dyb), dyb.stride(0), ptr(xb),
                                                xb.stride(0), ptr(sb), sb.numel() * 4, _s(dya))
        if rc not in (0, 1):
            L.check(rc, "vit_linear_wgrad_partials2")
        if rc == 0:
            if probe is not None:
                e1 = torch.cuda.Event(enable_timing=True)
                e1.record()
                probe.append((e0, e1, 2.0 * M * (Na * Ka + Nb * Kb), True))
            reduce_on.add(sa.view(nz, Na * Ka), nz, Na * Ka, outa)
            reduce_on.add(sb.view(nz, Nb * Kb), nz, Nb * Kb, outb)
            return outa, outb
    linear_wgrad(dya, xa, out=outa, tail=tail, reduce_on=reduce_on)
    linear_wgrad(dyb, xb, out=outb, tail=tail, reduce_on=reduce_on)
    return outa, outb


WGRAD_PROBE = [None]


def colsum(x2d, out=None, accumulate=False):
    M, N = x2d.shape
    if out is None:
        out = torch.empty(N, dtype=torch.float32, device=x2d.device)
    S = max(1, min(256, M // 64))
    nfl = (S + (S + 63) // 64) * N
    part = workspace("colsum", nfl * 4, x2d.device)
    call("vit_colsum", L.dt(x2d), M, N, ptr(x2d), x2d.stride(0), ptr(out), ptr(part), nfl, int(accumulate),
         _s(x2d))
    return out



def layer_norm_fwd(x2d, w, b, eps, out_dtype, rows=None, ldx=None, out=None, need_stats=True, mean=None, rstd=None):
    rows = x2d.shape[0] if rows is None else rows
    D = w.numel()
    ldx = x2d.stride(0) if ldx is None else ldx
    if out is None:
        out = torch.empty(rows, D, dtype=out_dtype, device=x2d.device)
    if need_stats and mean is None:
        mean = torch.empty(rows, dtype=torch.float32, device=x2d.device)
        rstd = torch.empty(rows, dtype=torch.float32, device=x2d.device)
    call("vit_layer_norm_fwd", L.dt(x2d), L.dt(out), rows, D, ptr(x2d), ldx, ptr(out), out.stride(0), ptr(w),
         ptr(b), ptr(mean), ptr(rstd), float(eps), _s(x2d))
    return out, mean, rstd


def add_layer_norm_supported(D: int) -> bool:
    return D % 256 == 0 and 256 <= D <= 2048


def add_layer_norm_fwd(x2d, r2d, xs, w=None, b=None, eps=1e-6, out=None, mean=None, rstd=None):
    assert x2d.dtype == torch.float32 and xs.dtype == torch.float32
    rows, D = xs.shape
    if out is not None:
        assert mean is not None and rstd is not None
    call("vit_add_layer_norm_fwd", L.dt(r2d), L.dt(out) if out is not None else L.dt(r2d), rows, D, ptr(x2d),
         x2d.stride(0), ptr(r2d), r2d.stride(0), ptr(xs), xs.stride(0),
         ptr(out), out.stride(0) if out is not None else 0, ptr(w), ptr(b), ptr(mean), ptr(rstd), float(eps), _s(xs))
    return xs


def layer_norm_bwd(x, ldx, dy, w, mean, rstd, dx, lddx, rows, dres=None, ldres=0, dx_copy=None, ld_copy=0,
                   compact_np=0, dgamma=None, dbeta=None, dsum=None, ws="ln_partial", reduce_on=None):
    D = w.numel()
    part = None
    nfl = 0
    want = dgamma is not None or dsum is not None
    defer = want and reduce_on is not None
    if want:
        nfl = L.lib().vit_layer_norm_bwd_partial_floats(rows, D)
        part = (torch.empty(nfl, dtype=torch.float32, device=x.device) if defer
                else workspace(ws, nfl * 4, x.device))
    call("vit_layer_norm_bwd", L.dt(x), L.dt(dy), rows, D, ptr(x), ldx, ptr(dy), dy.stride(0), ptr(w), ptr(mean),
         ptr(rstd), ptr(dres), ldres, ptr(dx), lddx, ptr(dx_copy), ld_copy,
         L.dt(dx_copy) if dx_copy is not None else L.BF16, compact_np, ptr(dgamma), ptr(dbeta), ptr(dsum), ptr(part),
         nfl, int(defer), _s(x))
    if defer:
        nb = L.lib().vit_layer_norm_bwd_blocks(rows)
        if isinstance(reduce_on, ColBatch):
            for q, o in enumerate((dgamma, dbeta, dsum)):
                if o is not None:
                    reduce_on.add(part[q * nb * D:(q + 1) * nb * D], nb, D, o)
            return
        sc = part[3 * nb * D:]

        def finish():
            _keep(part)
            if dgamma is not None:
                call("vit_colreduce_multi", ptr(part), 3 if dsum is not None else 2, nb, D, ptr(dgamma),
                     ptr(dbeta), ptr(dsum), 0, ptr(sc), _s(dgamma))
            else:
                call("vit_colreduce_multi", ptr(part[2 * nb * D:]), 1, nb, D, ptr(dsum), None, None, 0,
                     ptr(sc), _s(dsum))
        reduce_on.run(finish)



FP8_ATTN_MAX_TOKENS = 320


def check_fp8_tokens(N):
    if N > FP8_ATTN_MAX_TOKENS:
        raise ValueError(f"fp8 attention (vit_sdpa_fwd_fp8) supports at most {FP8_ATTN_MAX_TOKENS} tokens, got "
                         f"{N}: switch it off (set_attention_fp8(False)) for this model")


def sdpa_fwd(qkv2d, B, H, N, o=None, scale=None, lse=None, causal=False, fp8=False):
    if fp8:
        check_fp8_tokens(N)
    D = H * 64
    if o is None:
        o = torch.empty(B * N, D, dtype=qkv2d.dtype, device=qkv2d.device)
    if lse is None:
        lse = torch.empty(B * H * N, dtype=torch.float32, device=qkv2d.device)
    scale = 64 ** -0.5 if scale is None else scale
    name = "vit_sdpa_fwd_fp8" if fp8 else "vit_sdpa_fwd"
    call(name, L.dt(qkv2d), B, H, N, 64, ptr(qkv2d), qkv2d.stride(0), ptr(o), o.stride(0), ptr(lse),
         float(scale), int(causal), _s(qkv2d))
    return o, lse


def sdpa_bwd(qkv2d, o, do, lse, B, H, N, dqkv=None, scale=None, dbias=None, causal=False, ws="", reduce_on=None):
    if dqkv is None:
        dqkv = torch.empty_like(qkv2d)
    scale = 64 ** -0.5 if scale is None else scale
    delta = workspace("sdpa_delta" + ws, B * H * N * 4, qkv2d.device)
    part, nfl = None, 0
    defer = dbias is not None and isinstance(reduce_on, ColBatch) and qkv2d.dtype == torch.bfloat16
    if dbias is not None:
        nfl = L.lib().vit_sdpa_bwd_partial_floats(B, N, H * 64)
        part = (torch.empty(nfl, dtype=torch.float32, device=qkv2d.device) if defer
                else workspace("sdpa_bias" + ws, nfl * 4, qkv2d.device))
    call("vit_sdpa_bwd", L.dt(qkv2d), B, H, N, 64, ptr(qkv2d), qkv2d.stride(0), ptr(o), o.stride(0), ptr(do),
         do.stride(0), ptr(lse), ptr(dqkv), dqkv.stride(0), ptr(delta), float(scale), int(causal),
         None if defer else ptr(dbias), ptr(part), nfl, _s(qkv2d))
    if defer:
        reduce_on.add(part, B, 3 * H * 64, dbias)
    return dqkv



def patch_unfold(img, ps, dtype, ld=None):
    B, C, Hi, Wi = img.shape
    assert img.dtype == torch.float32 and img.is_contiguous()
    npatch = (Hi // ps) * (Wi // ps)
    K = C * ps * ps
    U = torch.empty(B * npatch, max(K, ld or K), dtype=dtype, device=img.device)
    call("vit_patch_unfold_ld", L.dt(U), B, C, Hi, Wi, ps, U.shape[1], ptr(img), ptr(U), _s(img))
    return U


def pad_cols(w2d, ld):
    rows, cols = w2d.shape
    assert w2d.stride(1) == 1 and ld >= cols
    out = torch.empty(rows, ld, dtype=w2d.dtype, device=w2d.device)
    call("vit_copy_rows_padded", L.dt(w2d), rows, cols, ptr(w2d), w2d.stride(0), ptr(out), ld, _s(w2d))
    return out


def patch_embed_fwd(U, w2d, bias, pos, cls, B, npatch):
    D, K = w2d.shape
    assert U.shape[1] == K and U.stride(1) == 1 and w2d.stride(1) == 1
    x = torch.empty(B, npatch + 1, D, dtype=torch.float32, device=U.device)
    call("vit_patch_embed_fwd_ld", L.dt(U), B, npatch, D, K, ptr(U), U.stride(0), ptr(w2d), w2d.stride(0),
         ptr(bias), ptr(pos), ptr(x), _s(U))
    call("vit_cls_pos_fill", B, npatch + 1, D, ptr(x), ptr(cls), ptr(pos), _s(U))
    return x


def pos_grad(dx, B, S, D, dpos, dcls):
    call("vit_pos_grad", B, S, D, ptr(dx), ptr(dpos), ptr(dcls), _s(dx))


def cross_entropy_fwd(logits, target):
    B, C = logits.shape
    assert logits.dtype == torch.float32 and target.dtype == torch.int64
    row_lse = torch.empty(B, dtype=torch.float32, device=logits.device)
    row_loss = torch.empty(B, dtype=torch.float32, device=logits.device)
    loss = torch.empty((), dtype=torch.float32, device=logits.device)
    call("vit_cross_entropy_fwd", B, C, ptr(logits), logits.stride(0), ptr(target), ptr(row_lse), ptr(row_loss),
         ptr(loss), _s(logits))
    return loss, row_lse


def cross_entropy_bwd(logits, target, row_lse, grad_loss, out_dtype=torch.float32):
    B, C = logits.shape
    d = torch.empty(B, C, dtype=out_dtype, device=logits.device)
    g = grad_loss.to(torch.float32).contiguous() if grad_loss is not None else None
    call("vit_cross_entropy_bwd", L.dt(d), B, C, ptr(logits), logits.stride(0), ptr(target), ptr(row_lse), ptr(g),
         ptr(d), d.stride(0), _s(logits))
    return d


def eval_metrics(logits, target, acc, topk=5, row_ws=None):
    L.require_gpu(logits)
    B, C = logits.shape
    assert logits.dtype == torch.float32 and logits.stride(1) == 1 and target.dtype == torch.int64
    assert target.is_contiguous() and target.numel() == B and target.device == logits.device
    assert acc.dtype == torch.float64 and acc.numel() >= 6 and acc.is_contiguous() and acc.device == logits.device
    if row_ws is None:
        row_ws = torch.empty(2 * B, dtype=torch.float32, device=logits.device)
    assert row_ws.dtype == torch.float32 and row_ws.numel() >= 2 * B
    call("vit_eval_metrics", B, C, ptr(logits), logits.stride(0), ptr(target), int(topk), ptr(row_ws), ptr(acc),
         _s(logits))
    return acc


def cast_bf16(src: torch.Tensor, dst: torch.Tensor):
    assert src.dtype == torch.float32 and dst.dtype == torch.bfloat16 and src.numel() == dst.numel()
    call("vit_cast_f32_bf16", ptr(src), ptr(dst), src.numel(), _s(src))


def zero_(t: torch.Tensor):
    call("vit_zero", ptr(t), t.numel() * t.element_size(), _s(t))
    return t



def token_embed(tokens, table, pos):
    S, Lq = tokens.shape
    D = table.shape[1]
    x = torch.empty(S * Lq, D, dtype=torch.float32, device=table.device)
    call("vit_token_embed", S * Lq, Lq, D, table.shape[0], ptr(tokens.contiguous()), ptr(table), ptr(pos), ptr(x),
         _s(table))
    return x


def gather_rows(src2d, idx, out=None):
    n = idx.numel()
    D = src2d.shape[1]
    if out is None:
        out = torch.empty(n, D, dtype=torch.float32, device=src2d.device)
    call("vit_gather_rows", n, D, ptr(src2d), src2d.stride(0), ptr(idx), ptr(out), out.stride(0), _s(src2d))
    return out


def scatter_rows(src2d, idx, dst2d):
    n = idx.numel()
    call("vit_scatter_rows", n, src2d.shape[1], ptr(src2d), src2d.stride(0), ptr(idx), ptr(dst2d), dst2d.stride(0),
         _s(src2d))
    return dst2d


def rownorm_fwd(x2d, log_scale=None):
    n, D = x2d.shape
    y = torch.empty_like(x2d)
    rn = torch.empty(n, dtype=torch.float32, device=x2d.device)
    call("vit_rownorm_fwd", n, D, ptr(x2d), ptr(log_scale), ptr(y), ptr(rn), _s(x2d))
    return y, rn


def rownorm_bwd(x2d, dy, rn, log_scale=None):
    n, D = x2d.shape
    dx = torch.empty_like(x2d)
    call("vit_rownorm_bwd", n, D, ptr(x2d), ptr(dy.contiguous()), ptr(rn), ptr(log_scale), ptr(dx), _s(x2d))
    return dx


def mse_fwd(pred, target):
    loss = torch.empty((), dtype=torch.float32, device=pred.device)
    call("vit_mse_fwd", pred.numel(), ptr(pred), ptr(target), ptr(loss), _s(pred))
    return loss


def mse_bwd(pred, target, grad_loss=None):
    d = torch.empty_like(pred)
    g = grad_loss.to(torch.float32).contiguous() if grad_loss is not None else None
    call("vit_mse_bwd", pred.numel(), ptr(pred), ptr(target), ptr(g), ptr(d), _s(pred))
    return d




def gemm(P, p_layout, Q, q_layout, M, N, R, out=None, out_dtype=torch.float32, bias=None):
    assert P.dtype == Q.dtype and P.stride(-1) == 1 and Q.stride(-1) == 1
    if (out is None and bias is None and P.dtype == torch.float32 and out_dtype == torch.float32
            and R >= 256 and ((M + 31) // 32) * ((N + 31) // 32) < 128):
        out = torch.empty(M, N, dtype=torch.float32, device=P.device)
        ws = workspace(f"gemm_splitk:{_s(P)}", 2 * 256 * 1024 * 4, P.device).view(torch.float32)
        call("vit_gemm_splitk", p_layout, q_layout, M, N, R, ptr(P), P.stride(0), ptr(Q), Q.stride(0), ptr(out),
             ptr(ws), ws.numel(), _s(P))
        return out
    if out is None:
        out = torch.empty(M, N, dtype=out_dtype, device=P.device)
    if P.dtype == torch.float32:
        _streamk(P.device)
    call("vit_gemm", L.dt(P), L.dt(out), p_layout, q_layout, L.EPI_STORE, M, N, R, ptr(P), P.stride(0), ptr(Q),
         Q.stride(0), ptr(out), out.stride(0), ptr(bias), None, 0, None, 1, _s(P))
    return out
```

Measured before the change: 7625 images/s.

## Compute only CLS token in the last block's attention output and MLP tail

Adds a CLS-only tail path for the final transformer block, on by default via VIT_CLS_TAIL. The attention forward computes only the first query tile and fills the remaining outputs with zeros and the LSE with infinity, while the post-attention LN, MLP and backward run over B rows instead of B*N. A strided-residual layernorm backward variant and partial-sum spreading keep the gradients consistent with the reduced rows. The aim is to skip last-layer work that does not affect the classification loss, at the cost of extra code paths, some scatter overhead, and reliance on only the CLS token feeding the head.

```diff
diff --git a/include/vit_hip.h b/include/vit_hip.h
--- a/include/vit_hip.h
+++ b/include/vit_hip.h
@@ -94,11 +94,19 @@
                        const float* dres, int64_t ldres, float* dx, int64_t lddx, void* dx_copy, int64_t ld_copy,
                        int dtype_copy, int compact_np, float* dgamma, float* dbeta, float* dsum, float* partial,
                        int64_t partial_floats, int defer_reduce, void* stream);
+int vit_layer_norm_bwd_cls(int dtype_x, int dtype_dy, int rows, int D, const void* x, int64_t ldx,
+                           const void* dy, int64_t lddy, const float* w, const float* mean, const float* rstd,
+                           const float* dres, int64_t ldres, int res_every, float* dx, int64_t lddx, void* dx_copy,
+                           int64_t ld_copy, int dtype_copy, int compact_np, float* dgamma, float* dbeta, float* dsum,
+                           float* partial, int64_t partial_floats, int defer_reduce, void* stream);
 int vit_layer_norm_bwd_partial_floats(int rows, int D);
 int vit_layer_norm_bwd_blocks(int rows);
 
 int vit_sdpa_fwd(int dtype, int B, int H, int N, int head_dim, const void* qkv, int64_t ld_qkv, void* o,
                  int64_t ld_o, float* lse, float scale, int causal, void* stream);
+int vit_sdpa_fwd_cls(int dtype, int B, int H, int N, int head_dim, const void* qkv, int64_t ld_qkv, void* o,
+                     int64_t ld_o, float* lse, float scale, void* stream);
+int vit_sdpa_cls_count(int reset);
 int vit_sdpa_fwd_fp8(int dtype, int B, int H, int N, int head_dim, const void* qkv, int64_t ld_qkv, void* o,
                      int64_t ld_o, float* lse, float scale, int causal, void* stream);
 int vit_sdpa_bwd(int dtype, int B, int H, int N, int head_dim, const void* qkv, int64_t ld_qkv, const void* o,
diff --git a/vit-project_amd/csrc/attention.hip b/vit-project_amd/csrc/attention.hip
--- a/vit-project_amd/csrc/attention.hip
+++ b/vit-project_amd/csrc/attention.hip
@@ -83,7 +83,7 @@
     for (int i_ = 0; i_ < 8; ++i_) d[i_] = st[i_];                                               \
   }
 
-template <int NT, bool STAMP = false, bool CAUSAL = false>
+template <int NT, bool STAMP = false, bool CAUSAL = false, bool CLS = false>
 __global__ __launch_bounds__(AT_THREADS, NT <= 14 ? 4 : 2) void attn_fwd_mfma(const bf16* __restrict__ qkv, int64_t ld_qkv, int D,
                                                      int H, int N, float scale, bf16* __restrict__ o,
                                                      int64_t ld_o, float* __restrict__ lse, int causal,
@@ -106,7 +106,13 @@
   __syncthreads();
   AT_STAMP(1)
   const float c2 = scale * LOG2E;
-  for (int qt = wave; qt < NT; qt += AT_WAVES) {
+  if constexpr (CLS) {
+    for (int i = 16 * 16 + threadIdx.x; i < N * 16; i += AT_THREADS)
+      *reinterpret_cast<bf16x4*>(o + ((int64_t)b * N + (i >> 4)) * ld_o + h * 64 + (i & 15) * 4) =
+          bf16x4{(bf16)0.f, (bf16)0.f, (bf16)0.f, (bf16)0.f};
+    for (int r = 16 + threadIdx.x; r < N; r += AT_THREADS) lse[(int64_t)bh * N + r] = INFINITY;
+  }
+  for (int qt = wave; qt < (CLS ? 1 : NT); qt += AT_WAVES) {
     const int q = qt * 16 + (lane & 15);
     bf16x8 qf[2];
     {
@@ -1992,6 +1998,16 @@
   return 0;
 }
 
+template <int NT>
+static int fwd_mfma_cls(const void* qkv, int64_t ld_qkv, int D, int B, int H, int N, float scale, void* o, int64_t ld_o,
+                        float* lse, hipStream_t s) {
+  hipLaunchKernelGGL((attn_fwd_mfma<NT, false, false, true>), dim3(B * H), dim3(AT_THREADS), 0, s, (const bf16*)qkv,
+                     ld_qkv, D, H, N, scale, (bf16*)o, ld_o, lse, 0, nullptr);
+  VIT_CHECK_LAUNCH();
+  return 0;
+}
+static int g_cls_count = 0;
+
 #define NT_CASES(X) X(1) X(2) X(3) X(4) X(5) X(6) X(7) X(8) X(9) X(10) X(11) X(12) X(13) X(14) X(15) X(16) X(17) X(18)
 
 extern "C" {
@@ -2069,6 +2085,26 @@
     hipLaunchKernelGGL(attn_fwd_generic<float>, grid, dim3(256), 0, s, (const float*)qkv, ld_qkv, D, H, N, scale, (float*)o, ld_o, lse, causal);
   VIT_CHECK_LAUNCH();
   return 0;
+}
+
+int vit_sdpa_fwd_cls(int dtype, int B, int H, int N, int head_dim, const void* qkv, int64_t ld_qkv, void* o,
+                     int64_t ld_o, float* lse, float scale, void* stream) {
+  if (head_dim != 64 || N <= 0) return (int)hipErrorInvalidValue;
+  if (N <= AT_RESIDENT_MAX && dtype == VIT_BF16 && (ld_qkv % 8 == 0) && (ld_o % 4 == 0) && lse && !g_attn_stamps) {
+    const int nt = (N + 15) / 16;
+    ++g_cls_count;
+    switch (nt) {
+#define CASE(n) case n: return fwd_mfma_cls<n>(qkv, ld_qkv, H * 64, B, H, N, scale, o, ld_o, lse, (hipStream_t)stream);
+      NT_CASES(CASE)
+#undef CASE
+    }
+  }
+  return vit_sdpa_fwd(dtype, B, H, N, head_dim, qkv, ld_qkv, o, ld_o, lse, scale, 0, stream);
+}
+int vit_sdpa_cls_count(int reset) {
+  const int n = g_cls_count;
+  if (reset) g_cls_count = 0;
+  return n;
 }
 
 int vit_sdpa_fwd_fp8(int dtype, int B, int H, int N, int head_dim, const void* qkv, int64_t ld_qkv, void* o,
diff --git a/vit-project_amd/csrc/norm.hip b/vit-project_amd/csrc/norm.hip
--- a/vit-project_amd/csrc/norm.hip
+++ b/vit-project_amd/csrc/norm.hip
@@ -125,13 +125,20 @@
   return true;
 }
 
+__device__ __forceinline__ const float* res_row(const float* dres, int64_t ldres, int every, int row) {
+  if (!dres) return nullptr;
+  if (every <= 0) return dres + (int64_t)row * ldres;
+  const int q = row / every;
+  return row == q * every ? dres + (int64_t)q * ldres : nullptr;
+}
+
 template <int NV, typename TX, typename TD, typename TC>
 __global__ __launch_bounds__(256) void ln_bwd_kernel(
     const TX* __restrict__ x, int64_t ldx, const TD* __restrict__ dy, int64_t lddy,
     const float* __restrict__ w, const float* __restrict__ mean, const float* __restrict__ rstd,
     const float* __restrict__ dres, int64_t ldres, float* __restrict__ dx, int64_t lddx,
     TC* __restrict__ dxc, int64_t ldc, int compact_np, float* __restrict__ part_g,
-    float* __restrict__ part_b, float* __restrict__ part_s, int rows, int D, int rows_per) {
+    float* __restrict__ part_b, float* __restrict__ part_s, int rows, int D, int rows_per, int res_every) {
   constexpr int NP = NV > 0 ? NV * 4 : LN_SMAX;
   const int lane = threadIdx.x & 63, wv = threadIdx.x >> 6;
   float pg[NP], pb[NP], ps[NP];
@@ -150,9 +157,10 @@
       f32x4 xh[NV], g[NV], rv[NV];
       float s1 = 0.f, s2 = 0.f;
       if (dres) {
+        const float* rr = res_row(dres, ldres, res_every, row);
 #pragma unroll
         for (int k = 0; k < NV; ++k)
-          rv[k] = *reinterpret_cast<const f32x4*>(dres + (int64_t)row * ldres + col4(lane, k));
+          rv[k] = rr ? *reinterpret_cast<const f32x4*>(rr + col4(lane, k)) : f32x4{0.f, 0.f, 0.f, 0.f};
       }
 #pragma unroll
       for (int k = 0; k < NV; ++k) {
@@ -184,6 +192,7 @@
       }
     } else {
       float s1 = 0.f, s2 = 0.f;
+      const float* rr = res_row(dres, ldres, res_every, row);
 #pragma unroll
       for (int k = 0; k < LN_SMAX; ++k) {
         int c = lane + 64 * k;
@@ -201,7 +210,7 @@
         if (c >= D) break;
         float xh = ((float)xr[c] - mu) * rs, g = (float)dyr[c] * w[c];
         float o = rs * (g - s1 - xh * s2);
-        if (dres) o += dres[(int64_t)row * ldres + c];
+        if (dres) o += rr ? rr[c] : 0.f;
         ps[k] += o;
         dxr[c] = o;
         if (keep) dxc[orow * ldc + c] = (TC)o;
@@ -262,7 +271,7 @@
     const float* __restrict__ w, const float* __restrict__ mean, const float* __restrict__ rstd,
     const float* __restrict__ dres, int64_t ldres, float* __restrict__ dx, int64_t lddx,
     TC* __restrict__ dxc, int64_t ldc, int compact_np, float* __restrict__ part_g,
-    float* __restrict__ part_b, float* __restrict__ part_s, int rows, int D, int rows_per) {
+    float* __restrict__ part_b, float* __restrict__ part_s, int rows, int D, int rows_per, int res_every) {
   constexpr int NP = NV * 4;
   const int lane = threadIdx.x & 63, wv = __builtin_amdgcn_readfirstlane(threadIdx.x >> 6);
   float pg[NP], pb[NP], ps[NP];
@@ -274,13 +283,14 @@
   const int r0 = blockIdx.x * rows_per, r1 = min(rows, r0 + rows_per);
   using Row = LnRow<NV, TX, TD>;
   auto load = [&](int row, Row& R) {
+    const float* rr = res_row(dres, ldres, res_every, row);
 #pragma unroll
     for (int k = 0; k < NV; ++k) {
       const int c = col4(lane, k);
       R.x[k] = ld4<TX>(x + (int64_t)row * ldx + c);
       if constexpr (std::is_same<TD, float>::value) R.d[k] = *reinterpret_cast<const f32x4*>(dy + (int64_t)row * lddy + c);
       else R.d[k] = *reinterpret_cast<const bf16x4*>(dy + (int64_t)row * lddy + c);
-      R.r[k] = dres ? *reinterpret_cast<const f32x4*>(dres + (int64_t)row * ldres + c) : f32x4{0.f, 0.f, 0.f, 0.f};
+      R.r[k] = rr ? *reinterpret_cast<const f32x4*>(rr + c) : f32x4{0.f, 0.f, 0.f, 0.f};
     }
     R.mu = mean[row];
     R.rs = rstd[row];
@@ -377,9 +387,9 @@
 static void launch_bwd(int nv, int nblk, hipStream_t s, const void* x, int64_t ldx, const void* dy, int64_t lddy,
                        const float* w, const float* mean, const float* rstd, const float* dres, int64_t ldres,
                        float* dx, int64_t lddx, void* dxc, int64_t ldc, int compact_np, float* pg, float* pb,
-                       float* ps, int rows, int D, int rows_per) {
+                       float* ps, int rows, int D, int rows_per, int res_every) {
 #define B(K, NV) hipLaunchKernelGGL((K<NV, TX, TD, TC>), dim3(nblk), dim3(64 * LN_WAVES), 0, s, (const TX*)x, ldx, \
-                                 (const TD*)dy, lddy, w, mean, rstd, dres, ldres, dx, lddx, (TC*)dxc, ldc, compact_np, pg, pb, ps, rows, D, rows_per)
+                                 (const TD*)dy, lddy, w, mean, rstd, dres, ldres, dx, lddx, (TC*)dxc, ldc, compact_np, pg, pb, ps, rows, D, rows_per, res_every)
   if (g_ln_pipe < 0) { const char* v = getenv("VIT_LN_BWD_PIPE"); g_ln_pipe = v ? atoi(v) : 1; }
   const int pipe = g_ln_pipe;
   switch (nv) {
@@ -453,13 +463,14 @@
   return (int)(3 * (int64_t)nblk * D + 3 * colreduce_scratch_floats(nblk, D));
 }
 
-int vit_layer_norm_bwd(int dtype_x, int dtype_dy, int rows, int D, const void* x, int64_t ldx,
-                       const void* dy, int64_t lddy, const float* w, const float* mean, const float* rstd,
-                       const float* dres, int64_t ldres, float* dx, int64_t lddx, void* dx_copy, int64_t ld_copy,
-                       int dtype_copy, int compact_np, float* dgamma, float* dbeta, float* dsum, float* partial,
-                       int64_t partial_floats, int defer_reduce, void* stream) {
+static int ln_bwd(int dtype_x, int dtype_dy, int rows, int D, const void* x, int64_t ldx,
+                  const void* dy, int64_t lddy, const float* w, const float* mean, const float* rstd,
+                  const float* dres, int64_t ldres, int res_every, float* dx, int64_t lddx, void* dx_copy,
+                  int64_t ld_copy, int dtype_copy, int compact_np, float* dgamma, float* dbeta, float* dsum,
+                  float* partial, int64_t partial_floats, int defer_reduce, void* stream) {
   hipStream_t s = (hipStream_t)stream;
   if (rows <= 0) return 0;
+  if (res_every < 0) return (int)hipErrorInvalidValue;
   if (D > 64 * LN_SMAX) return (int)hipErrorInvalidValue;
   const int rows_per = ln_bwd_rows();
   const int nblk = vit_layer_norm_bwd_blocks(rows);
@@ -474,8 +485,8 @@
              (ld_copy % 4 == 0);
   int nv = vec ? D / 256 : 0;
 #define LB(TX, TD) \
-  if (dtype_copy == VIT_BF16) launch_bwd<TX, TD, bf16>(nv, nblk, s, x, ldx, dy, lddy, w, mean, rstd, dres, ldres, dx, lddx, dx_copy, ld_copy, compact_np, pg, pb, ps, rows, D, rows_per); \
-  else launch_bwd<TX, TD, float>(nv, nblk, s, x, ldx, dy, lddy, w, mean, rstd, dres, ldres, dx, lddx, dx_copy, ld_copy, compact_np, pg, pb, ps, rows, D, rows_per);
+  if (dtype_copy == VIT_BF16) launch_bwd<TX, TD, bf16>(nv, nblk, s, x, ldx, dy, lddy, w, mean, rstd, dres, ldres, dx, lddx, dx_copy, ld_copy, compact_np, pg, pb, ps, rows, D, rows_per, res_every); \
+  else launch_bwd<TX, TD, float>(nv, nblk, s, x, ldx, dy, lddy, w, mean, rstd, dres, ldres, dx, lddx, dx_copy, ld_copy, compact_np, pg, pb, ps, rows, D, rows_per, res_every);
   if (dtype_x == VIT_F32 && dtype_dy == VIT_F32) { LB(float, float) }
   else if (dtype_x == VIT_F32) { LB(float, bf16) }
   else if (dtype_dy == VIT_BF16) { LB(bf16, bf16) }
@@ -492,4 +503,24 @@
   return 0;
 }
 
-}
+int vit_layer_norm_bwd(int dtype_x, int dtype_dy, int rows, int D, const void* x, int64_t ldx,
+                       const void* dy, int64_t lddy, const float* w, const float* mean, const float* rstd,
+                       const float* dres, int64_t ldres, float* dx, int64_t lddx, void* dx_copy, int64_t ld_copy,
+                       int dtype_copy, int compact_np, float* dgamma, float* dbeta, float* dsum, float* partial,
+                       int64_t partial_floats, int defer_reduce, void* stream) {
+  return ln_bwd(dtype_x, dtype_dy, rows, D, x, ldx, dy, lddy, w, mean, rstd, dres, ldres, 0, dx, lddx, dx_copy,
+                ld_copy, dtype_copy, compact_np, dgamma, dbeta, dsum, partial, partial_floats, defer_reduce, stream);
+}
+
+int vit_layer_norm_bwd_cls(int dtype_x, int dtype_dy, int rows, int D, const void* x, int64_t ldx,
+                           const void* dy, int64_t lddy, const float* w, const float* mean, const float* rstd,
+                           const float* dres, int64_t ldres, int res_every, float* dx, int64_t lddx, void* dx_copy,
+                           int64_t ld_copy, int dtype_copy, int compact_np, float* dgamma, float* dbeta, float* dsum,
+                           float* partial, int64_t partial_floats, int defer_reduce, void* stream) {
+  if (res_every < 1 || !dres) return (int)hipErrorInvalidValue;
+  return ln_bwd(dtype_x, dtype_dy, rows, D, x, ldx, dy, lddy, w, mean, rstd, dres, ldres, res_every, dx, lddx,
+                dx_copy, ld_copy, dtype_copy, compact_np, dgamma, dbeta, dsum, partial, partial_floats, defer_reduce,
+                stream);
+}
+
+}
diff --git a/vit-project_amd/vit_amd/__init__.py b/vit-project_amd/vit_amd/__init__.py
--- a/vit-project_amd/vit_amd/__init__.py
+++ b/vit-project_amd/vit_amd/__init__.py
@@ -1,6 +1,6 @@
 from . import _lib
 from .model import (VisionTransformer, create_model, cross_entropy, set_wgrad_overlap, set_forward_only,
-                    block_forward_only)
+                    set_cls_tail, block_forward_only)
 from .pos_embed import resample_abs_pos_embed, adapt_state_dict
 from .optim import FusedSGD, FusedAdamW, CosineAnnealingLRWithWarmup
 from .dora import DoRALayer, dora_weight
@@ -15,7 +15,7 @@
 __all__ = ["VisionTransformer", "create_model", "cross_entropy", "set_wgrad_overlap", "FusedSGD", "FusedAdamW",
            "CosineAnnealingLRWithWarmup", "DoRALayer", "dora_weight", "rsa", "clip", "data", "CLIPHBA", "MSELoss",
            "mse_loss", "apply_dora_to_ViT", "switch_dora_layers", "count_trainable_parameters", "set_forward_only",
-           "block_forward_only", "evaluate", "EvalMeter", "validate", "resample_abs_pos_embed", "adapt_state_dict"]
+           "set_cls_tail", "block_forward_only", "evaluate", "EvalMeter", "validate", "resample_abs_pos_embed", "adapt_state_dict"]
 
 
 def load_library(path=None):
diff --git a/vit-project_amd/vit_amd/_lib.py b/vit-project_amd/vit_amd/_lib.py
--- a/vit-project_amd/vit_amd/_lib.py
+++ b/vit-project_amd/vit_amd/_lib.py
@@ -44,11 +44,15 @@
     "vit_add_layer_norm_fwd": [i32, i32, i32, i32, vp, i64, vp, i64, vp, i64, vp, i64, vp, vp, vp, vp, f32, vp],
     "vit_layer_norm_bwd": [i32, i32, i32, i32, vp, i64, vp, i64, vp, vp, vp, vp, i64, vp, i64, vp, i64, i32,
                            i32, vp, vp, vp, vp, i64, i32, vp],
+    "vit_layer_norm_bwd_cls": [i32, i32, i32, i32, vp, i64, vp, i64, vp, vp, vp, vp, i64, i32, vp, i64, vp, i64, i32,
+                               i32, vp, vp, vp, vp, i64, i32, vp],
     "vit_layer_norm_bwd_partial_floats": [i32, i32],
     "vit_layer_norm_bwd_blocks": [i32],
     "vit_layer_norm_bwd_variant": [i32],
     "vit_sdpa_fwd": [i32, i32, i32, i32, i32, vp, i64, vp, i64, vp, f32, i32, vp],
     "vit_sdpa_fwd_fp8": [i32, i32, i32, i32, i32, vp, i64, vp, i64, vp, f32, i32, vp],
+    "vit_sdpa_fwd_cls": [i32, i32, i32, i32, i32, vp, i64, vp, i64, vp, f32, vp],
+    "vit_sdpa_cls_count": [i32],
     "vit_sdpa_bwd_variant": [i32],
     "vit_sdpa_long_config": [i32],
     "vit_sdpa_long_count": [i32],
diff --git a/vit-project_amd/vit_amd/model.py b/vit-project_amd/vit_amd/model.py
--- a/vit-project_amd/vit_amd/model.py
+++ b/vit-project_amd/vit_amd/model.py
@@ -43,6 +43,7 @@
 
 _FUSED_RESID_F32 = [os.environ.get("VIT_FUSED_RESID_F32", "0") == "1"]
 _FWD_ONLY = [os.environ.get("VIT_FWD_ONLY", "1") != "0"]
+_CLS_TAIL = [os.environ.get("VIT_CLS_TAIL", "1") != "0"]
 
 
 def set_wgrad_overlap(enable: bool):
@@ -207,14 +208,17 @@
     x2 = x.reshape(M, D)
     F = fc1w.shape[0]
     f32 = torch.float32
-    h1, h2 = torch.empty(M, D, dtype=T, device=dev), torch.empty(M, D, dtype=T, device=dev)
-    m1, r1, m2, r2 = (torch.empty(M, dtype=f32, device=dev) for _ in range(4))
+    ct = bool(cfg.get("cls_tail"))
+    Mt = B if ct else M
+    h1, h2 = torch.empty(M, D, dtype=T, device=dev), torch.empty(Mt, D, dtype=T, device=dev)
+    m1, r1 = (torch.empty(M, dtype=f32, device=dev) for _ in range(2))
+    m2, r2 = (torch.empty(Mt, dtype=f32, device=dev) for _ in range(2))
     qkv = torch.empty(M, 3 * D, dtype=T, device=dev)
     o = torch.empty(M, D, dtype=T, device=dev)
     lse = torch.empty(B * H * N, dtype=f32, device=dev)
-    xm, xo = torch.empty(M, D, dtype=f32, device=dev), torch.empty(M, D, dtype=f32, device=dev)
-    act = torch.empty(M, F, dtype=T, device=dev)
-    dact = None if fwd_only else torch.empty(M, F, dtype=T, device=dev)
+    xm, xo = torch.empty(Mt, D, dtype=f32, device=dev), torch.empty(Mt, D, dtype=f32, device=dev)
+    act = torch.empty(Mt, F, dtype=T, device=dev)
+    dact = None if fwd_only else torch.empty(Mt, F, dtype=T, device=dev)
     Wqkv, Wproj, W1, W2 = _wt(qkvw, T), _wt(projw, T), _wt(fc1w, T), _wt(fc2w, T)
     causal = bool(cfg.get("causal", False))
     attn_fp8 = bool(cfg.get("attn_fp8", False))
@@ -225,7 +229,12 @@
     pend = rs.get("pending") if rs is not None else None
     pb = yb = None
     if rs is not None:
-        pb, yb = torch.empty(M, D, dtype=T, device=dev), torch.empty(M, D, dtype=T, device=dev)
+        pb, yb = torch.empty(Mt, D, dtype=T, device=dev), torch.empty(Mt, D, dtype=T, device=dev)
+    x_cls = o_cls = xc = None
+    if ct:
+        x_cls, o_cls = x2.view(B, N * D)[:, :D], o.view(B, N * D)[:, :D]
+        if rs is None:
+            xc = torch.empty(B, D, dtype=f32, device=dev)
 
     def fc1(sl):
         if fwd_only:
@@ -256,7 +265,36 @@
             steps.append(lambda: ops.add_layer_norm_fwd(xm[sl], yb[sl], xo[sl]))
         return steps
 
+    def chain_tail(b0, b1):
+        sl, cs = slice(b0 * N, b1 * N), slice(b0, b1)
+        steps = [
+            ln1(sl),
+            lambda: ops.linear_fwd(h1[sl], Wqkv, qkvb.detach(), out=qkv[sl]),
+            lambda: ops.sdpa_fwd_cls(qkv[sl], b1 - b0, H, N, o=o[sl], lse=lse[b0 * H * N:b1 * H * N]),
+        ]
+        if rs is not None:
+            steps += [
+                lambda: ops.linear_fwd(o_cls[cs], Wproj, projb.detach(), out=pb[cs]),
+                lambda: ops.add_layer_norm_fwd(x_cls[cs], pb[cs], xm[cs], n2w.detach(), n2b.detach(), eps,
+                                               out=h2[cs], mean=m2[cs], rstd=r2[cs]),
+                fc1(cs),
+                lambda: ops.linear_fwd(act[cs], W2, fc2b.detach(), out=yb[cs]),
+                lambda: ops.add_layer_norm_fwd(xm[cs], yb[cs], xo[cs]),
+            ]
+        else:
+            steps += [
+                lambda: ops.pad_cols(x_cls[cs], D, out=xc[cs]),
+                lambda: ops.linear_fwd(o_cls[cs], Wproj, projb.detach(), epi=L.EPI_RESID, resid=xc[cs], out=xm[cs]),
+                lambda: ops.layer_norm_fwd(xm[cs], n2w.detach(), n2b.detach(), eps, T, out=h2[cs], mean=m2[cs],
+                                           rstd=r2[cs]),
+                fc1(cs),
+                lambda: ops.linear_fwd(act[cs], W2, fc2b.detach(), epi=L.EPI_RESID, resid=xm[cs], out=xo[cs]),
+            ]
+        return steps
+
     def chain(b0, b1):
+        if ct:
+            return chain_tail(b0, b1)
         if rs is not None:
             return chain_fused(b0, b1)
         r0, r1_ = b0 * N, b1 * N
@@ -284,15 +322,15 @@
         mine, other = chain(0, hb), chain(hb, B)
         side.run(lambda: run(other))
         side.guard(x2, h1, m1, r1, qkv, o, lse, xm, h2, m2, r2, dact, act, xo,
-                   *(t for t in (pb, yb, *(pend or ())) if t is not None))
+                   *(t for t in (pb, yb, xc, *(pend or ())) if t is not None))
         run(mine)
         if not cfg.get("defer_join"):
             side.join()
     else:
         run(chain(0, B))
     if rs is not None:
-        rs["pending"] = None if cfg.get("resid_last") else (xm, yb)
-    return xo.reshape(B, N, D), (x2, h1, m1, r1, qkv, o, lse, xm, h2, m2, r2, dact, act), (Wqkv, Wproj, W1, W2)
+        rs["pending"] = None if (ct or cfg.get("resid_last")) else (xm, yb)
+    return xo.reshape(B, Mt // B, D), (x2, h1, m1, r1, qkv, o, lse, xm, h2, m2, r2, dact, act), (Wqkv, Wproj, W1, W2)
 
 
 def block_forward_only(x, params, cfg):
@@ -308,6 +346,29 @@
     prev = _FWD_ONLY[0]
     _FWD_ONLY[0] = bool(enable)
     return prev
+
+
+TAIL_PAD = 64
+
+
+def tail_pad(N: int, ln_rows_per: int = 32) -> int:
+    ok = (N > TAIL_PAD and ln_rows_per >= 1 and TAIL_PAD % ln_rows_per == 0
+          and TAIL_PAD % ops.DGRAD_SUM_ROWS == 0 and TAIL_PAD % ops.WGRAD_KTILE_ROWS == 0)
+    return TAIL_PAD if ok else N
+
+
+def cls_tail_enabled() -> bool:
+    return _CLS_TAIL[0]
+
+
+def set_cls_tail(enable: bool) -> bool:
+    prev = _CLS_TAIL[0]
+    _CLS_TAIL[0] = bool(enable)
+    return prev
+
+
+def wants_cls_tail(enabled: bool, cls_only: bool, global_pool: str, attn_fp8: bool = False) -> bool:
+    return bool(enabled) and bool(cls_only) and global_pool == "token" and not attn_fp8
 
 
 def wants_forward_only(enabled: bool, grad_enabled: bool, input_requires_grad: bool,
@@ -338,6 +399,7 @@
         ctx.meta = (B, N, D, H, T, cfg.get("compact_np", 0), cfg["quick_gelu"], causal)
         ctx.defer_bwd = bool(cfg.get("defer_bwd_join"))
         ctx.attn_fp8 = attn_fp8
+        ctx.cls_tail = bool(cfg.get("cls_tail"))
         ctx.grad_hook = cfg.get("grad_hook")
         ctx.flat_span = cfg.get("flat_span")
         return xo
@@ -350,9 +412,33 @@
         B, N, D, H, T, compact_np, qg, causal = ctx.meta
         ng = ctx.needs_input_grad
         M = B * N
+        ct = ctx.cls_tail
+        P = tail_pad(N, ops.ln_bwd_rows_per()) if ct else N
+        Mt = B * P
+        spread_sums = ct and P != N
         dev = dxo.device
-        dxo = dxo.contiguous().reshape(M, D)
+        dxo = dxo.contiguous().reshape(B if ct else M, D)
         dxo_c, dxo_sum = _take_copy(dxo, T, want_dsum=True)
+        pads = []
+
+        def rows_padded(t):
+            w = t.shape[1]
+            pads.append(ops.pad_cols(t, P * w).view(B * P, w))
+            return pads[-1]
+
+        dg_rows = ln_rows = sp_mlp = sp_attn = None
+        if ct:
+            dxo_c = rows_padded(dxo_c)
+            dxo = dxo_c if T == torch.float32 else rows_padded(dxo)
+            xm, h2, dact, act = rows_padded(xm), rows_padded(h2), rows_padded(dact), rows_padded(act)
+            m2, r2 = rows_padded(m2.view(B, 1)).view(-1), rows_padded(r2.view(B, 1)).view(-1)
+        if spread_sums:
+            F = act.shape[1]
+            rp = ops.ln_bwd_rows_per()
+            dg_rows = ops.dense_part_rows(B, N, ops.DGRAD_SUM_ROWS, P // ops.DGRAD_SUM_ROWS, dev)
+            ln_rows = ops.dense_part_rows(B, N, rp, P // rp, dev)
+            sp_mlp = ops.pair_split(M, D, F, F, D)
+            sp_attn = ops.pair_split(M, D, D, 3 * D, D, bool(compact_np))
         gelu_bwd = L.EPI_QGELU_BWD if qg else L.EPI_GELU_BWD
         side = _Side(dev)
         need_mlp_in = any(ng[0:11])
@@ -378,30 +464,33 @@
             side.run(lambda: ops.linear_wgrad(dxo_c, act, out=g[11], reduce_on=rbw))
         dx = None
         if need_mlp_in:
-            dpre = ops.linear_dgrad(dxo_c, W2, out_dtype=T, epi=gelu_bwd, pre=dact, dbias=g[10], reduce_on=rb)
+            dpre = ops.linear_dgrad(dxo_c, W2, out_dtype=T, epi=gelu_bwd, pre=dact, dbias=g[10], reduce_on=rb,
+                                    part_rows=dg_rows)
             if pair_mlp:
-                side.run(lambda: ops.linear_wgrad_pair((dxo_c, act, g[11]), (dpre, h2, g[9]), rbw))
+                side.run(lambda: ops.linear_wgrad_pair((dxo_c, act, g[11]), (dpre, h2, g[9]), rbw, split=sp_mlp))
             elif ng[9]:
                 side.run(lambda: ops.linear_wgrad(dpre, h2, out=g[9], reduce_on=rbw))
         if any(ng[0:9]):
             dh2 = ops.linear_dgrad(dpre, W1, out_dtype=T)
-            dxm = torch.empty(M, D, dtype=torch.float32, device=dev)
-            dxm_c = dxm if T == torch.float32 else torch.empty(M, D, dtype=T, device=dev)
-            ops.layer_norm_bwd(xm, D, dh2, n2w.detach(), m2, r2, dxm, D, M, dres=dxo, ldres=D,
+            dxm = torch.empty(Mt, D, dtype=torch.float32, device=dev)
+            dxm_c = dxm if T == torch.float32 else torch.empty(Mt, D, dtype=T, device=dev)
+            ops.layer_norm_bwd(xm, D, dh2, n2w.detach(), m2, r2, dxm, D, Mt, dres=dxo, ldres=D,
                                dx_copy=None if T == torch.float32 else dxm_c, ld_copy=D, dgamma=g[7], dbeta=g[8],
-                               dsum=g[6], reduce_on=rb)
+                               dsum=g[6], reduce_on=rb, part_rows=ln_rows)
             tail = bool(compact_np)
-            pair_attn = rbw is not None and ng[5] and ng[3] and need_attn
+            pair_attn = rbw is not None and ng[5] and ng[3] and need_attn and not spread_sums
+            o_w = rows_padded(o.view(B, N * D)[:, :D]) if spread_sums else o
             if ng[5] and not pair_attn:
-                side.run(lambda: ops.linear_wgrad(dxm_c, o, out=g[5], tail=tail, reduce_on=rbw))
+                side.run(lambda: ops.linear_wgrad(dxm_c, o_w, out=g[5], split=sp_attn, tail=tail, reduce_on=rbw))
             if need_attn:
                 do = ops.linear_dgrad(dxm_c, Wproj, out_dtype=T)
-                dqkv = ops.sdpa_bwd(qkv, o, do, lse, B, H, N, dbias=g[4], causal=causal,
-                                    reduce_on=rb)
+                if spread_sums:
+                    do = ops.pad_cols(do.view(B, P * D)[:, :D], N * D).view(M, D)
+                dqkv = ops.sdpa_bwd(qkv, o, do, lse, B, H, N, dbias=g[4], causal=causal, reduce_on=rb)
                 if pair_attn:
                     side.run(lambda: ops.linear_wgrad_pair((dxm_c, o, g[5]), (dqkv, h1, g[3]), rbw, tail=tail))
                 elif ng[3]:
-                    side.run(lambda: ops.linear_wgrad(dqkv, h1, out=g[3], tail=tail, reduce_on=rbw))
+                    side.run(lambda: ops.linear_wgrad(dqkv, h1, out=g[3], split=sp_attn, tail=tail, reduce_on=rbw))
             if need_h1:
                 dh1 = ops.linear_dgrad(dqkv, Wqkv, out_dtype=T)
                 dx = torch.empty(M, D, dtype=torch.float32, device=dev)
@@ -410,15 +499,16 @@
                 else:
                     dx_c = None if T == torch.float32 or not ng[0] else torch.empty(M, D, dtype=T, device=dev)
                 dsum = None if (compact_np or not ng[0]) else torch.empty(D, dtype=torch.float32, device=dev)
-                ops.layer_norm_bwd(x2, D, dh1, n1w.detach(), m1, r1, dx, D, M, dres=dxm, ldres=D, dx_copy=dx_c,
-                                   ld_copy=D, compact_np=compact_np, dgamma=g[1], dbeta=g[2], dsum=dsum,
-                                   reduce_on=rb)
+                dres = dxm.view(B, P * D)[:, :D] if spread_sums else dxm
+                ops.layer_norm_bwd(x2, D, dh1, n1w.detach(), m1, r1, dx, D, M, dres=dres, ldres=dres.stride(0),
+                                   dx_copy=dx_c, ld_copy=D, compact_np=compact_np, dgamma=g[1], dbeta=g[2], dsum=dsum,
+                                   reduce_on=rb, res_every=N if spread_sums else 0)
                 if ng[0] and (dx_c is not None or dsum is not None):
                     _put_copy(dx, dx_c, dsum)
         side.run(rb.launch)
         side.guard(*rb.parts)
         side.guard(dxo, dxo_c, dxo_sum, x2, h1, m1, r1, qkv, o, lse, xm, h2, m2, r2, dact, act,
-                   *(v for v in (dpre, dxm, dxm_c, do, dqkv, dx) if v is not None))
+                   *(v for v in (dpre, dxm, dxm_c, do, dqkv, dx) if v is not None), *pads)
         if cfg_defer_bwd(ctx):
             _queue_backward_join(dev)
         if ctx.grad_hook is not None and all(ng[1:13]):
@@ -449,10 +539,14 @@
         dxc = ops.linear_dgrad(dlogits, hw.detach(), out_dtype=torch.float32)
         dhw = ops.linear_wgrad(dlogits, xc, out=_gout(hw))
         dhb = ops.colsum(dlogits, out=_gout(hb))
-        dx = ops.zero_(torch.empty(B, N, D, dtype=torch.float32, device=x.device))
+        dx = torch.empty(B, N, D, dtype=torch.float32, device=x.device)
+        if N > 1:
+            ops.zero_(dx)
         dx_c = None
         if T != torch.float32:
-            dx_c = ops.zero_(torch.empty(B * N, D, dtype=T, device=x.device))
+            dx_c = torch.empty(B * N, D, dtype=T, device=x.device)
+            if N > 1:
+                ops.zero_(dx_c)
         dnw, dnb = _gout(nw), _gout(nb)
         dsum = torch.empty(D, dtype=torch.float32, device=x.device)
         ops.layer_norm_bwd(x, N * D, dxc, nw.detach(), mc, rc, dx, N * D, B, dx_copy=dx_c, ld_copy=N * D,
@@ -614,7 +708,7 @@
         self._ensure_shadows()
         return list(self._shadows.pairs)
 
-    def _tokens(self, x):
+    def _tokens(self, x, cls_only=False):
         L.require_gpu(x)
         self._ensure_shadows()
         cfg = dict(self._cfg)
@@ -636,6 +730,8 @@
             bcfg = cfg if i != 0 else dict(cfg, compact_np=pe.num_patches)
             if "resid" in cfg and i == n - 1:
                 bcfg = dict(bcfg, resid_last=True)
+            if i == n - 1 and wants_cls_tail(_CLS_TAIL[0], cls_only, self.global_pool, cfg["attn_fp8"]):
+                bcfg = dict(bcfg, cls_tail=True)
             if hook is not None:
                 bcfg = dict(bcfg, grad_hook=hook, flat_span=blk._flat_span)
             x = run_block(x, blk.block_params(), bcfg)
@@ -656,7 +752,7 @@
                                                    self.head.bias.detach(), out_dtype=torch.float32)
 
     def forward(self, x):
-        x = self._tokens(x)
+        x = self._tokens(x, cls_only=True)
         return _HeadFn.apply(x, self.norm.weight, self.norm.bias, self.head.weight, self.head.bias, dict(self._cfg))
 
 
diff --git a/vit-project_amd/vit_amd/ops.py b/vit-project_amd/vit_amd/ops.py
--- a/vit-project_amd/vit_amd/ops.py
+++ b/vit-project_amd/vit_amd/ops.py
@@ -74,7 +74,50 @@
     return (out, act_out) if epi in (L.EPI_BIAS_GELU, L.EPI_BIAS_QGELU) else out
 
 
-def linear_dgrad(dy2d, w, out_dtype=torch.float32, epi=L.EPI_STORE, pre=None, out=None, dbias=None, reduce_on=None):
+DGRAD_SUM_ROWS = 64
+WGRAD_KTILE_ROWS = 32
+_LN_ROWS = []
+_PART_ROWS = {}
+
+
+def ln_bwd_rows_per() -> int:
+    if not _LN_ROWS:
+        blocks = L.lib().vit_layer_norm_bwd_blocks
+        r = 1
+        while r < (1 << 16) and blocks(r + 1) == 1:
+            r += 1
+        _LN_ROWS.append(r)
+    return _LN_ROWS[0]
+
+
+class PartRows:
+
+    def __init__(self, rows, S, every, device):
+        rows = [int(r) for r in rows]
+        if not rows or min(rows) < 0 or max(rows) >= S or len(set(rows)) != len(rows) or every < 1:
+            raise ValueError(f"partial rows {rows[:4]}.. do not fit a dense partial matrix of {S} rows one to one")
+        self.n, self.S, self.every = len(rows), int(S), int(every)
+        self.idx = torch.tensor(rows, dtype=torch.int64, device=device)
+
+
+def dense_part_rows(B, N, unit, every, device):
+    key = (B, N, unit, every, torch.device(device))
+    if key not in _PART_ROWS:
+        _PART_ROWS[key] = PartRows([b * N // unit for b in range(B)], (B * N + unit - 1) // unit, every, device)
+    return _PART_ROWS[key]
+
+
+def spread_partials(part2d, pr):
+    rows, N = part2d.shape
+    assert part2d.is_contiguous() and part2d.dtype == torch.float32
+    assert rows == pr.n * pr.every and pr.idx.numel() == pr.n and pr.idx.device == part2d.device, (rows, pr.n, pr.every)
+    out = zero_(torch.empty(pr.S * N, dtype=torch.float32, device=part2d.device))
+    scatter_rows(part2d.view(pr.n, pr.every * N)[:, :N], pr.idx, out.view(pr.S, N))
+    return out
+
+
+def linear_dgrad(dy2d, w, out_dtype=torch.float32, epi=L.EPI_STORE, pre=None, out=None, dbias=None, reduce_on=None,
+                 part_rows=None):
     M, N = dy2d.shape
     K = w.shape[1]
     assert w.shape[0] == N and w.dtype == dy2d.dtype and dy2d.stride(1) == 1
@@ -94,8 +137,10 @@
     call("vit_linear_dgrad", L.dt(dy2d), L.dt(out), epi, M, N, K, ptr(dy2d), dy2d.stride(0), ptr(w), ptr(out),
          out.stride(0), ptr(pre), ptr(dbias), ptr(part), nfl, int(defer), _s(dy2d))
     if defer:
-        rows = (M + 63) // 64
+        rows = (M + DGRAD_SUM_ROWS - 1) // DGRAD_SUM_ROWS
         if isinstance(reduce_on, ColBatch):
+            if part_rows is not None:
+                part, rows = spread_partials(part[:rows * K].view(rows, K), part_rows), part_rows.S
             reduce_on.add(part, rows, K, dbias)
             return out
 
@@ -196,16 +241,27 @@
     return out
 
 
-def linear_wgrad_pair(a, b, reduce_on, tail=False):
+def pair_split(M, Na, Ka, Nb, Kb, tail=False):
+    tiles = ((Na + 255) // 256) * ((Ka + 255) // 256) + ((Nb + 255) // 256) * ((Kb + 255) // 256)
+    wgs = _WGRAD_TAIL_WGS[0] if tail else _WGRAD_WGS[0]
+    return max(1, min(max(1, round(wgs / tiles)), M // 1024))
+
+
+def linear_wgrad_pair(a, b, reduce_on, tail=False, split=None):
+    asked = split
+    """Two weight gradients of a block over the same token rows, a = (dy, x, out), b likewise, as
+    ONE grouped launch of split-K partials whose slab sums become two jobs of ``reduce_on`` (a
+    ColBatch).  The split is chosen for the pair's tiles together (half the slabs of two separate
+    launches).  Falls back to two linear_wgrad calls when the pair does not meet the grouped
+    kernel's rules (bf16, M % 32 == 0, MFMA operand alignment)."""
     (dya, xa, outa), (dyb, xb, outb) = a, b
     M, Na = dya.shape
     Ka, Nb, Kb = xa.shape[1], dyb.shape[1], xb.shape[1]
     ok = (isinstance(reduce_on, ColBatch) and dya.dtype == torch.bfloat16 and dyb.dtype == torch.bfloat16
           and xa.dtype == dya.dtype and xb.dtype == dyb.dtype and dyb.shape[0] == M and M % 32 == 0)
     if ok:
-        tiles = ((Na + 255) // 256) * ((Ka + 255) // 256) + ((Nb + 255) // 256) * ((Kb + 255) // 256)
-        wgs = _WGRAD_TAIL_WGS[0] if tail else _WGRAD_WGS[0]
-        split = max(1, min(max(1, round(wgs / tiles)), M // 1024))
+        if split is None:
+            split = pair_split(M, Na, Ka, Nb, Kb, tail)
         nz = L.lib().vit_linear_wgrad_nslabs(L.BF16, M, Na, Ka, split)
         sa = torch.empty(nz * Na * Ka, dtype=torch.float32, device=dya.device)
         sb = torch.empty(nz * Nb * Kb, dtype=torch.float32, device=dya.device)
@@ -226,8 +282,8 @@
             reduce_on.add(sa.view(nz, Na * Ka), nz, Na * Ka, outa)
             reduce_on.add(sb.view(nz, Nb * Kb), nz, Nb * Kb, outb)
             return outa, outb
-    linear_wgrad(dya, xa, out=outa, tail=tail, reduce_on=reduce_on)
-    linear_wgrad(dyb, xb, out=outb, tail=tail, reduce_on=reduce_on)
+    linear_wgrad(dya, xa, out=outa, split=asked, tail=tail, reduce_on=reduce_on)
+    linear_wgrad(dyb, xb, out=outb, split=asked, tail=tail, reduce_on=reduce_on)
     return outa, outb
 
 
@@ -277,7 +333,8 @@
 
 
 def layer_norm_bwd(x, ldx, dy, w, mean, rstd, dx, lddx, rows, dres=None, ldres=0, dx_copy=None, ld_copy=0,
-                   compact_np=0, dgamma=None, dbeta=None, dsum=None, ws="ln_partial", reduce_on=None):
+                   compact_np=0, dgamma=None, dbeta=None, dsum=None, ws="ln_partial", reduce_on=None, res_every=0,
+                   part_rows=None):
     D = w.numel()
     part = None
     nfl = 0
@@ -287,16 +344,26 @@
         nfl = L.lib().vit_layer_norm_bwd_partial_floats(rows, D)
         part = (torch.empty(nfl, dtype=torch.float32, device=x.device) if defer
                 else workspace(ws, nfl * 4, x.device))
-    call("vit_layer_norm_bwd", L.dt(x), L.dt(dy), rows, D, ptr(x), ldx, ptr(dy), dy.stride(0), ptr(w), ptr(mean),
-         ptr(rstd), ptr(dres), ldres, ptr(dx), lddx, ptr(dx_copy), ld_copy,
-         L.dt(dx_copy) if dx_copy is not None else L.BF16, compact_np, ptr(dgamma), ptr(dbeta), ptr(dsum), ptr(part),
-         nfl, int(defer), _s(x))
+    tail = (ptr(dx), lddx, ptr(dx_copy), ld_copy, L.dt(dx_copy) if dx_copy is not None else L.BF16, compact_np,
+            ptr(dgamma), ptr(dbeta), ptr(dsum), ptr(part), nfl, int(defer), _s(x))
+    head = (L.dt(x), L.dt(dy), rows, D, ptr(x), ldx, ptr(dy), dy.stride(0), ptr(w), ptr(mean), ptr(rstd), ptr(dres),
+            ldres)
+    if res_every:
+        assert dres is not None and dres.dtype == torch.float32 and dres.shape[0] * res_every >= rows
+        call("vit_layer_norm_bwd_cls", *head, int(res_every), *tail)
+    else:
+        call("vit_layer_norm_bwd", *head, *tail)
     if defer:
         nb = L.lib().vit_layer_norm_bwd_blocks(rows)
         if isinstance(reduce_on, ColBatch):
             for q, o in enumerate((dgamma, dbeta, dsum)):
-                if o is not None:
-                    reduce_on.add(part[q * nb * D:(q + 1) * nb * D], nb, D, o)
+                if o is None:
+                    continue
+                pq = part[q * nb * D:(q + 1) * nb * D]
+                if part_rows is not None:
+                    reduce_on.add(spread_partials(pq.view(nb, D), part_rows), part_rows.S, D, o)
+                else:
+                    reduce_on.add(pq, nb, D, o)
             return
         sc = part[3 * nb * D:]
 
@@ -333,6 +400,18 @@
     name = "vit_sdpa_fwd_fp8" if fp8 else "vit_sdpa_fwd"
     call(name, L.dt(qkv2d), B, H, N, 64, ptr(qkv2d), qkv2d.stride(0), ptr(o), o.stride(0), ptr(lse),
          float(scale), int(causal), _s(qkv2d))
+    return o, lse
+
+
+def sdpa_fwd_cls(qkv2d, B, H, N, o=None, scale=None, lse=None):
+    D = H * 64
+    if o is None:
+        o = torch.empty(B * N, D, dtype=qkv2d.dtype, device=qkv2d.device)
+    if lse is None:
+        lse = torch.empty(B * H * N, dtype=torch.float32, device=qkv2d.device)
+    scale = 64 ** -0.5 if scale is None else scale
+    call("vit_sdpa_fwd_cls", L.dt(qkv2d), B, H, N, 64, ptr(qkv2d), qkv2d.stride(0), ptr(o), o.stride(0), ptr(lse),
+         float(scale), _s(qkv2d))
     return o, lse
 
 
@@ -366,10 +445,12 @@
     return U
 
 
-def pad_cols(w2d, ld):
+def pad_cols(w2d, ld, out=None):
     rows, cols = w2d.shape
     assert w2d.stride(1) == 1 and ld >= cols
-    out = torch.empty(rows, ld, dtype=w2d.dtype, device=w2d.device)
+    if out is None:
+        out = torch.empty(rows, ld, dtype=w2d.dtype, device=w2d.device)
+    assert out.shape == (rows, ld) and out.is_contiguous() and out.dtype == w2d.dtype
     call("vit_copy_rows_padded", L.dt(w2d), rows, cols, ptr(w2d), w2d.stride(0), ptr(out), ld, _s(w2d))
     return out
 
```

Result: faster. 7835 images/s (median of 6 runs) (+2.7%).
